# NyanCAD/CedarSim.jl

Measured on AMD Instinct MI355X. Metric: newton_iters_per_sec, higher is better.
Workload: dtype f64

## Files before the change

cedarsim.jl_amd/csrc/ch_engine.hip:

```cpp
#include <hip/hip_runtime.h>
#include <hip/hip_ext.h>

#include <algorithm>
#include <atomic>
#include <chrono>
#include <cmath>
#include <cstdio>
#include <cstring>
#include <map>
#include <memory>
#include <new>
#include <stdexcept>
#include <string>
#include <array>
#include <vector>

#include "../../include/cedarhip.h"
#include "ch_analysis.hpp"
#include "ch_bsim4.hpp"
#include "ch_device_mem.hpp"
#include "ch_env.hpp"
#include "ch_kernels.hpp"
#include "ch_persist.hpp"
#include "ch_sparse.hpp"
#include "ch_stepper_host.hpp"

using namespace chip;
using hclock = std::chrono::steady_clock;

struct ch_ctx {
  int device = 0;
  hipStream_t stream = nullptr;
  std::string err;
};

namespace {

struct Rng {
  uint64_t s;
  explicit Rng(uint64_t seed) : s(seed) {}
  uint64_t next() { uint64_t z = (s += 0x9E3779B97F4A7C15ull); z = (z ^ (z >> 30)) * 0xBF58476D1CE4E5B9ull; z = (z ^ (z >> 27)) * 0x94D049BB133111EBull; return z ^ (z >> 31); }
  double uniform() { return ((next() >> 11) + 0.5) * (1.0 / 9007199254740992.0); }
  double normal() { double u1 = uniform(), u2 = uniform(); return std::sqrt(-2.0 * std::log(u1)) * std::cos(6.283185307179586 * u2); }
};

}

struct ch_result {
  std::vector<double> times, values, final_state;
  std::vector<int32_t> pts;
  const double* dev_values = nullptr; int64_t dev_n = 0;
  ch_stats stats;
  int status = CH_OK;
  int n_obs = 0, S = 1;
};

struct PersistConsts;
struct ch_circuit;

struct Description {
  int n_nodes = 0; double temp = 27, gmin = 1e-12, scale = 1;
  std::vector<HDev> dev; std::vector<HSource> src; std::vector<std::vector<double>> model;
  std::vector<int> slot_kind, slot_a, slot_b, obs_kind, obs_index;
  std::vector<double> va_par;
  Analysis A;
};
struct Structure {
  DevBuf<int> d_comp_class, d_comp_uofs, d_comp_dofs, d_gl_ptr, d_dkind, d_dterm, d_dsrc, d_dhdev, d_obs_unk, d_unk_obs;
  DevBuf<unsigned long long> d_stamps; DevBuf<ClassMeta> d_classes; DevBuf<unsigned char> d_dmask;
  DevBuf<int> d_dvac, d_va_mod, d_va_pofs, d_va_cofs;
  int n_va_inst = 0; size_t vac_total = 0; std::vector<ClassMeta> h_cms;
  std::vector<int> obs_primary;
  std::vector<int> needed_src;
  std::vector<int> dev_src;
  int n_dev_src() const { return std::max<int>(1, (int)dev_src.size()); }
  int block_threads = 64, lu_variant = 16;
  bool wide_split = false; int wide_l = 0, wide_other = 0;
  size_t lds_doubles_fixed = 0, lds_extra_bytes = 0;
 private: friend struct ch_circuit;
  void class_blobs(const Description& D, std::vector<int>& blob) {
    h_cms.clear();
    int max_slots = 0;
    for (size_t ci = 0; ci < D.A.classes.size(); ++ci) {
      const CompClass& c = D.A.classes[ci];
      ClassMeta m; std::memset(&m, 0, sizeof(m));
      m.nc = c.nc; m.ndev = c.ndev; m.nonlinear = c.nonlinear ? 1 : 0;
      m.n_mat_src = (int)c.mat_src.size(); m.n_vec_src = (int)c.vec_src.size();
      while (blob.size() & 3) blob.push_back(0);
      m.blob_ofs = (int)blob.size();
      blob.insert(blob.end(), c.mat_ptr.begin(), c.mat_ptr.end());
      blob.insert(blob.end(), c.vec_ptr.begin(), c.vec_ptr.end());
      int rep = -1;
      for (int k = 0; k < D.A.n_comp; ++k) if (D.A.comp_class[k] == (int)ci) { rep = k; break; }
      int ns = 0;
      {
        std::vector<int> lanes;
        bool big = false;
        for (int d = 0; d < c.ndev; ++d) {
          const EDev& e = D.A.edev[D.A.comp_dofs[rep] + d];
          if (e.kind != K_VA) continue;
          if (va_gen::MODULES[D.dev[e.hdev].ipar[0]].n_params >= 64) big = true;
          bool first = true;
          for (int j = 0; j < e.nt; ++j) if (e.term[j] >= 0) { lanes.push_back((d << 4) | (first ? 8 : 0) | j); first = false; }
        }
        const bool split = big && !env_on(Env::VA_NOSPLIT);
        if (ci == 0) { wide_split = split; wide_l = (int)lanes.size(); wide_other = 0; }
        if (!split) { for (int v : lanes) { blob.push_back(v); ++ns; } }
        else {
          for (int v : lanes) { blob.push_back(v | (1 << 29)); ++ns; }
          while (ns & 63) { blob.push_back(-1); ++ns; }
          for (int v : lanes) { blob.push_back(v | (1 << 29) | (1 << 30)); ++ns; }
        }
      }
      for (int d = 0; d < c.ndev; ++d) if (D.A.edev[D.A.comp_dofs[rep] + d].kind == K_MOS) { blob.push_back(d << 4); ++ns; if (ci == 0) ++wide_other; }
      for (int d = 0; d < c.ndev; ++d) { const int kd = D.A.edev[D.A.comp_dofs[rep] + d].kind; if (kd != K_MOS && kd != K_VA) { blob.push_back(d << 4); ++ns; if (ci == 0) ++wide_other; } }
      m.nslots = ns;
      std::vector<uint16_t> h16(c.mat_src); h16.insert(h16.end(), c.vec_src.begin(), c.vec_src.end());
      if (h16.size() & 1) h16.push_back(0);
      for (size_t i = 0; i < h16.size(); i += 2) blob.push_back((int)((uint32_t)h16[i] | ((uint32_t)h16[i + 1] << 16)));
      if (((int)blob.size() - m.blob_ofs) & 1) blob.push_back(0);
      m.wl_ofs = (int)blob.size() - m.blob_ofs;
      if (c.nc <= 64 && !c.vec_ptr.empty()) {
        std::vector<std::array<int, 3>> items;
        for (int i = 0; i < c.nc; ++i) {
          const int start = c.vec_ptr[i], cnt = c.vec_ptr[i + 1] - start;
          items.push_back({cnt, m.n_mat_src + start, (int)(0x8000u | (uint32_t)i)});
        }
        for (int e = 0; e < c.nc * c.nc; ++e) {
          const int start = c.mat_ptr[e], cnt = c.mat_ptr[e + 1] - start;
          if (cnt == 0 && e / c.nc != e % c.nc) continue;
          items.push_back({cnt, start, e});
        }
        std::stable_sort(items.begin(), items.end(), [](const std::array<int, 3>& x, const std::array<int, 3>& y) { return x[0] > y[0]; });
        for (const auto& it : items) { blob.push_back(it[1]); blob.push_back((int)(((uint32_t)it[0] << 16) | (uint32_t)it[2])); ++m.n_work; }
      }
      while ((blob.size() - m.blob_ofs) & 3) blob.push_back(0);
      m.blob_ints = (int)blob.size() - m.blob_ofs;
      if (env_on(Env::DEBUG_BLOB)) std::fprintf(stderr, "[blob] class %zu: nc %d ndev %d slots %d mat_src %d vec_src %d work %d blob_ints %d\n", ci, m.nc, m.ndev, m.nslots, m.n_mat_src, m.n_vec_src, m.n_work, m.blob_ints);
      max_slots = std::max(max_slots, m.nslots);
      h_cms.push_back(m);
    }
    block_threads = std::min(256, std::max(64, ((max_slots + 63) / 64) * 64));
    lu_variant = D.A.max_nc <= 8 ? 8 : (D.A.max_nc <= 12 ? 12 : (D.A.max_nc <= 16 ? 16 : (D.A.max_nc <= 32 ? 32 : 0)));
    if (D.A.wide) lu_variant = D.A.max_nc <= 16 ? 16 : 0;
  }
  void source_lists(const Description& D, std::vector<int>& dkind, std::vector<int>& dterm, std::vector<int>& dhdev, std::vector<int>& dsrc) {
    dsrc.clear();
    dev_src.clear();
    { std::vector<int> slot_of(D.src.size(), -1);
      for (const EDev& e : D.A.edev) {
        dkind.push_back(e.kind); for (int k = 0; k < NTERM; ++k) dterm.push_back(e.term[k]); dhdev.push_back(e.hdev);
        int si = e.kind == K_VA ? D.dev[e.hdev].ipar[1] : 0;
        if (e.src >= 0) { if (slot_of[e.src] < 0) { slot_of[e.src] = (int)dev_src.size(); dev_src.push_back(e.src); } si = slot_of[e.src]; }
        dsrc.push_back(si);
      }
      std::vector<char> need(D.src.size(), 0);
      for (int si : dev_src) need[si] = 1;
      for (const KnownDef& kd : D.A.known) for (auto& tm : kd.terms) need[tm.first] = 1;
      needed_src.clear();
      for (size_t i = 0; i < D.src.size(); ++i) if (need[i]) needed_src.push_back((int)i); }
  }
  void va_offsets(const Description& D, std::vector<int>& dvac, std::vector<int>& vmod, std::vector<int>& vpofs, std::vector<int>& vcofs) {
    dvac.assign(D.A.edev.size(), 0);
    vac_total = 0;
    for (size_t i = 0; i < D.A.edev.size(); ++i) {
      const EDev& e = D.A.edev[i];
      if (e.kind != K_VA) continue;
      const int mod = D.dev[e.hdev].ipar[0];
      dvac[i] = (int)vac_total; vmod.push_back(mod); vpofs.push_back(D.dev[e.hdev].ipar[1]); vcofs.push_back((int)vac_total);
      vac_total += (size_t)va_gen::N_CACHE[mod];
    }
    n_va_inst = (int)vmod.size();
    if (vmod.empty()) { vmod.push_back(0); vpofs.push_back(0); vcofs.push_back(0); }
  }
  void masks_and_observables(const Description& D, std::vector<unsigned char>& dm, std::vector<int>& obs_unk, std::vector<int>& unk_obs) {
    dm.assign(D.A.n_unk, 0);
    for (int u = 0; u < D.A.n_unk; ++u) dm[u] = (D.A.diff_mask[u] ? 1 : 0) | (D.A.unk_mna[u] >= D.n_nodes ? 2 : 0) | (D.A.replica[u] ? 4 : 0);
    obs_unk.clear(); unk_obs.assign(D.A.n_unk, -1);
    obs_primary.clear();
    for (size_t o = 0; o < D.obs_kind.size(); ++o) {
      int u = -1;
      if (D.obs_kind[o] == 0) u = D.A.node_unknown[D.obs_index[o]];
      else { int b = D.dev[D.obs_index[o]].branch; u = b >= 0 ? D.A.branch_unknown[b] : -1; }
      obs_unk.push_back(u);
      int prim = (int)o;
      if (u >= 0) { if (unk_obs[u] < 0) unk_obs[u] = (int)o; else prim = unk_obs[u]; }
      obs_primary.push_back(prim);
    }
  }
  void size_lds(const Description& D) {
    lds_doubles_fixed = 0; lds_extra_bytes = 0;
    for (size_t ci = 0; ci < D.A.classes.size(); ++ci) {
      const CompClass& c = D.A.classes[ci];
      lds_doubles_fixed = std::max(lds_doubles_fixed, (size_t)c.ndev * D.A.stride() + (size_t)c.nc * (c.nc + 1) + (size_t)c.nc * c.nc + 12 * (size_t)c.nc);
      lds_extra_bytes = std::max(lds_extra_bytes, ((size_t)h_cms[ci].blob_ints + 64) * 4 + 16);
    }
  }
};
struct SampleTables {
  int S = 1; bool dirty = true;
  std::vector<std::vector<double>> slot_val;
  int Spar = 1, Ssrc = 1, Smos = 1, Sgmin = 1, Stemp = 1, Sva = 1;
  std::vector<double> h_src_dc, h_src_par;
  std::vector<int> mos_cls; int n_cls = 0, max_mc = 0; long vac_stride_ = 0;
  DevBuf<double> d_dpar, d_dmult, d_gmin, d_temp, d_mosp, d_vapar, d_vacache;
  DevBuf<int> d_dcls, d_moscls_inst, d_mc_ofs, d_mc_n, d_mc_list, d_dcls_local;
  DevBuf<BlockMeta> d_bmeta;
};
struct NewtonState {
  DevBuf<double> d_X, d_Q, d_rate, d_kv;
  DevBuf<unsigned char> d_perm, d_active;
  DevBuf<BlockOut> d_out; PinnedBuf<BlockOut> h_out;
  PinnedBuf<Summary> h_sum; PinnedBuf<double> h_stage;
  DevEvent ev0, ev1; bool host_reduce = true; size_t lds_bytes = 0;
  int path = 1;
  NewtonArgs base;
  mutable std::vector<double> all_src; std::vector<double> sv_buf, kv_buf;
};
struct SparsePath {
  SparsePlan plan[2];
  struct PlanDev { DevBuf<int> prow, pcol, a2lu, diag_pos, lvl_ptr, lvl_rows, ulvl_ptr, ulvl_rows, lrow_ptr, l_pos, l_k, l_upd_ptr, upd_dst, upd_src, urow_ptr, u_pos, u_col;
                   DevBuf<int> lu2a, la_pos, la_diag, lb_dst, lb_sptr, lb_l, lb_u, lb_d, fl_rows, bl_rows; DevBuf<double> LUv, Lv;
                   DevBuf<int> s3_blob, s3_ptr, s3_topa, s3_topr; DevBuf<double> s3_schur, s3_xT, s3_base, s3_sum; DevBuf<unsigned> s3_cnt; bool s3 = false; } plan_dev[2];
  DevBuf<int> dflag; DevBuf<double> part;
  DevBuf<double> hpart, hrow;
  DevBuf<int> rowptr, colidx, mat_gptr, mat_gsrc, vec_gptr, vec_gsrc, heavy_mat, heavy_vec, heavy_rows; int n_heavy_mat = 0, n_heavy_vec = 0, n_heavy_rows = 0;
  DevBuf<double> stage, Aval, Cval, F, Q, rhs, y, dx, xcur, xpred, hq, w, qn;
  std::vector<int> h_rowptr, h_colidx; PinnedBuf<double> h_red; PinnedBuf<int> h_flag;
  std::vector<double> rate_v; std::vector<int> status_v;
  DevBuf<int> act[3]; DevBuf<double> scale;
  PinnedBuf<int> h_act; PinnedBuf<double> h_scale;
};
struct DeviceStepper {
  DevBuf<int> d_pci; DevBuf<double> d_pcd, d_pbps, d_psave, d_ptimes, d_prows, d_wgrec, d_grprec; DevBuf<unsigned> d_pcnt; DevBuf<TranCtl> d_pctl; DevBuf<int> d_pwgc, d_pwgk; DevBuf<double> d_pdcent, d_ptrans;
  int n_cu = 0, mode = 0; bool aborted = false;
};
struct SmallSignal {
  DevBuf<double> d_dumpA, d_dumpF, d_dumpQ, d_dumpC, d_dumpG, d_dumpF0, d_omega, d_xac, d_psd, d_noise_pwr, d_noise_exp;
  DevBuf<int> d_noise_a, d_noise_b, d_acfail; DevBuf<BlockMeta> d_bmeta_all;
  double scale = 0.0;
};
struct TornCompanion {
  std::unique_ptr<ch_circuit> c; std::string note;
  bool is_torn = false, keep_slot0 = false;
  std::vector<int> dsrc_host;
  std::vector<double> h_dpar0, h_dmult0;
};

struct ch_circuit {
  Arena arena;
  ch_ctx* ctx = nullptr;
  Description desc; Structure stru; SampleTables tab; NewtonState nwt;
  SparsePath sp; DeviceStepper ps; SmallSignal ac; TornCompanion torn; LaunchStats stats;
  const bool host_profile = env_on(Env::HOST_PROFILE);
  const long time_every = std::max(1L, env_long(Env::TIME_EVERY, 8));

  std::string& err() { return ctx->err; }
  void set_err(const std::string& s) { ctx->err = s; }

  ~ch_circuit() {
    if (ctx && ctx->stream) (void)hipStreamSynchronize(ctx->stream);
    if (g_arena == &arena) g_arena = nullptr;
  }

  int upload_structure() {
    g_arena = &arena; hipStream_t st = ctx->stream;
    std::vector<int> blob, dkind, dterm, dhdev, dvac, vmod, vpofs, vcofs, obs_unk, unk_obs; std::vector<unsigned char> dm;
    std::vector<int>& dsrc = torn.dsrc_host;
    stru.class_blobs(desc, blob);
    stru.source_lists(desc, dkind, dterm, dhdev, dsrc);
    stru.va_offsets(desc, dvac, vmod, vpofs, vcofs);
    HIPCHK(stru.d_dvac.upload(dvac, st)); HIPCHK(stru.d_va_mod.upload(vmod, st)); HIPCHK(stru.d_va_pofs.upload(vpofs, st)); HIPCHK(stru.d_va_cofs.upload(vcofs, st));
    stru.masks_and_observables(desc, dm, obs_unk, unk_obs);
    HIPCHK(stru.d_unk_obs.upload(unk_obs, st));
    { std::vector<unsigned long long> z(8, 0ull); HIPCHK(stru.d_stamps.upload(z, st)); }
    HIPCHK(stru.d_classes.upload(stru.h_cms, st)); HIPCHK(stru.d_gl_ptr.upload(blob, st));
    HIPCHK(stru.d_comp_class.upload(desc.A.comp_class, st)); HIPCHK(stru.d_comp_uofs.upload(desc.A.comp_uofs, st)); HIPCHK(stru.d_comp_dofs.upload(desc.A.comp_dofs, st));
    HIPCHK(stru.d_dkind.upload(dkind, st)); HIPCHK(stru.d_dterm.upload(dterm, st)); HIPCHK(stru.d_dsrc.upload(dsrc, st)); HIPCHK(stru.d_dhdev.upload(dhdev, st));
    HIPCHK(stru.d_dmask.upload(dm, st)); HIPCHK(stru.d_obs_unk.upload(obs_unk, st));
    HIPCHK(nwt.h_sum.alloc(1, hipHostMallocMapped)); HIPCHK(nwt.ev0.create()); HIPCHK(nwt.ev1.create());
    stru.size_lds(desc);
    return CH_OK;
  }

  bool slot_set(int i) const { return !tab.slot_val[i].empty(); }

 private:
  int check_capacity() {
    size_t free_b = 0, total_b = 0;
    HIPCHK(hipMemGetInfo(&free_b, &total_b));
    const double need = 2.0 * NSLOT * (double)tab.S * (double)std::max(1, desc.A.n_unk) * sizeof(double) + 64.0 * (double)tab.S * (double)std::max(1, desc.A.n_comp);
    if (need > 0.9 * (double)total_b) { set_err("sample count does not fit the device: " + std::to_string(tab.S) + " samples of " + std::to_string(desc.A.n_unk) + " unknowns need " + std::to_string((long long)(need / 1048576.0)) + " MiB for the state rings"); return CH_ERR_NOMEM; }
    return CH_OK;
  }
  int sample_widths() {
    const int nslot = (int)desc.slot_kind.size();
    bool any_par = false, any_src = false, any_mos = false, any_gmin = false;
    for (int i = 0; i < nslot; ++i) if (slot_set(i)) {
      switch (desc.slot_kind[i]) {
        case CH_SLOT_DEV_PAR: if (desc.dev[desc.slot_a[i]].kind == CH_DEV_MOS) any_mos = true; else any_par = true; break;
        case CH_SLOT_DEV_MULT: any_par = true; break;
        case CH_SLOT_MODEL_PAR: case CH_SLOT_TEMP: any_mos = true; break;
        case CH_SLOT_SRC_DC: case CH_SLOT_SRC_PAR: any_src = true; break;
        case CH_SLOT_GMIN: any_gmin = true; break;
      }
    }
    tab.Spar = any_par ? tab.S : 1; tab.Ssrc = any_src ? tab.S : 1; tab.Smos = any_mos ? tab.S : 1; tab.Sgmin = any_gmin ? tab.S : 1;
    return CH_OK;
  }
  int param_tables() {
    hipStream_t st = ctx->stream; const int nslot = (int)desc.slot_kind.size();
    const int nh = (int)desc.dev.size(), nsrc = (int)desc.src.size();
    std::vector<double> hpar((size_t)nh * tab.Spar), hmult((size_t)nh * tab.Spar);
    for (int d = 0; d < nh; ++d) for (int s = 0; s < tab.Spar; ++s) { hpar[(size_t)d * tab.Spar + s] = desc.dev[d].par[0]; hmult[(size_t)d * tab.Spar + s] = desc.dev[d].mult; }
    tab.h_src_dc.assign((size_t)tab.Ssrc * nsrc, 0.0); tab.h_src_par.assign((size_t)tab.Ssrc * nsrc * CH_SRC_NPAR, 0.0);
    for (int s = 0; s < tab.Ssrc; ++s) for (int i = 0; i < nsrc; ++i) { tab.h_src_dc[(size_t)s * nsrc + i] = desc.src[i].dc; for (int k = 0; k < CH_SRC_NPAR; ++k) tab.h_src_par[((size_t)s * nsrc + i) * CH_SRC_NPAR + k] = desc.src[i].par[k]; }
    std::vector<double> hg(tab.Sgmin, desc.gmin);
    bool any_temp = false;
    for (int i = 0; i < nslot; ++i) if (slot_set(i) && desc.slot_kind[i] == CH_SLOT_TEMP) any_temp = true;
    tab.Stemp = any_temp ? tab.S : 1;
    std::vector<double> htemp(tab.Stemp, desc.temp);
    for (int i = 0; i < nslot; ++i) if (slot_set(i)) {
      const int a = desc.slot_a[i], b = desc.slot_b[i];
      for (int s = 0; s < tab.S; ++s) {
        const double v = tab.slot_val[i][s];
        switch (desc.slot_kind[i]) {
          case CH_SLOT_DEV_PAR: if (desc.dev[a].kind != CH_DEV_MOS && b == 0) hpar[(size_t)a * tab.Spar + s] = v; break;
          case CH_SLOT_DEV_MULT: hmult[(size_t)a * tab.Spar + s] = v; break;
          case CH_SLOT_SRC_DC: tab.h_src_dc[(size_t)s * nsrc + a] = v; if (desc.src[a].kind == CH_SRC_DC) tab.h_src_par[((size_t)s * nsrc + a) * CH_SRC_NPAR] = v; break;
          case CH_SLOT_SRC_PAR: tab.h_src_par[((size_t)s * nsrc + a) * CH_SRC_NPAR + b] = v; break;
          case CH_SLOT_GMIN: hg[s] = v; break;
          case CH_SLOT_TEMP: htemp[s] = v; break;
          default: break;
        }
      }
    }
    torn.h_dpar0.assign(nh, 0.0); torn.h_dmult0.assign(nh, 1.0);
    for (int i = 0; i < nh; ++i) { torn.h_dpar0[i] = hpar[(size_t)i * tab.Spar]; torn.h_dmult0[i] = hmult[(size_t)i * tab.Spar]; }
    HIPCHK(tab.d_dpar.upload(hpar, st)); HIPCHK(tab.d_dmult.upload(hmult, st)); HIPCHK(tab.d_gmin.upload(hg, st)); HIPCHK(tab.d_temp.upload(htemp, st));
    return CH_OK;
  }
  int va_setup() {
    hipStream_t st = ctx->stream; const int nslot = (int)desc.slot_kind.size();
    bool any_va = false;
    for (int i = 0; i < nslot; ++i) if (slot_set(i) && desc.slot_kind[i] == CH_SLOT_VA_PAR) any_va = true;
    tab.Sva = any_va ? tab.S : 1;
    const size_t nvp = std::max<size_t>(1, desc.va_par.size());
    std::vector<double> vp(nvp * tab.Sva, 0.0);
    for (int s = 0; s < tab.Sva; ++s) std::copy(desc.va_par.begin(), desc.va_par.end(), vp.begin() + (size_t)s * nvp);
    for (int i = 0; i < nslot; ++i) if (slot_set(i) && desc.slot_kind[i] == CH_SLOT_VA_PAR) for (int s = 0; s < tab.Sva; ++s) vp[(size_t)s * nvp + desc.slot_a[i]] = tab.slot_val[i][s];
    HIPCHK(tab.d_vapar.upload(vp, st));
    const int Svac = (tab.Sva > 1 || tab.Stemp > 1) ? tab.S : 1;
    HIPCHK(tab.d_vacache.alloc(std::max<size_t>(1, stru.vac_total * (size_t)Svac)));
    if (stru.n_va_inst > 0) {
      const long nthr = (long)stru.n_va_inst * Svac;
      hipLaunchKernelGGL(va_setup_kernel, dim3((unsigned)((nthr + 63) / 64)), dim3(64), 0, st, stru.n_va_inst, Svac, stru.d_va_mod.p, stru.d_va_pofs.p, stru.d_va_cofs.p,
                         tab.d_vapar.p, tab.Sva > 1 ? (long)nvp : 0L, tab.d_temp.p, tab.Stemp, tab.d_vacache.p, Svac > 1 ? (long)stru.vac_total : 0L);
      HIPCHK(hipGetLastError());
    }
    tab.vac_stride_ = Svac > 1 ? (long)stru.vac_total : 0L;
    return CH_OK;
  }
  int mos_classes() {
    hipStream_t st = ctx->stream; const int nslot = (int)desc.slot_kind.size();
    const int nmos = (int)desc.A.mos_hdev.size();
    tab.mos_cls.assign(nmos, 0);
    std::map<std::vector<double>, int> cls_of;
    std::vector<int> cls_rep;
    for (int m = 0; m < nmos; ++m) {
      const HDev& d = desc.dev[desc.A.mos_hdev[m]];
      std::vector<double> key;
      key.push_back(d.ipar[0]);
      for (int k = 0; k < 7; ++k) key.push_back(std::isnan(d.par[k]) ? -1e300 : d.par[k]);
      for (int i = 0; i < nslot; ++i) if (slot_set(i) && desc.slot_kind[i] == CH_SLOT_DEV_PAR && desc.slot_a[i] == desc.A.mos_hdev[m]) {
        key.push_back(1e6 + desc.slot_b[i]);
        key.insert(key.end(), tab.slot_val[i].begin(), tab.slot_val[i].end());
      }
      auto it = cls_of.find(key);
      if (it == cls_of.end()) { it = cls_of.insert({key, (int)cls_rep.size()}).first; cls_rep.push_back(m); }
      tab.mos_cls[m] = it->second;
    }
    tab.n_cls = (int)cls_rep.size();
    const long cols = (long)std::max(1, tab.n_cls) * tab.Smos;
    std::vector<double> table((size_t)B4I_COUNT * cols + 2, 0.0), col(B4I_COUNT);
    for (int c = 0; c < tab.n_cls; ++c) {
      const int hd = desc.A.mos_hdev[cls_rep[c]];
      for (int s = 0; s < tab.Smos; ++s) {
        std::vector<double> card = desc.model[desc.dev[hd].ipar[0]];
        double ip[CH_DEV_NPAR]; for (int k = 0; k < CH_DEV_NPAR; ++k) ip[k] = desc.dev[hd].par[k];
        double tc = desc.temp;
        for (int i = 0; i < nslot; ++i) if (slot_set(i)) {
          const double v = tab.slot_val[i][tab.Smos > 1 ? s : 0];
          if (desc.slot_kind[i] == CH_SLOT_MODEL_PAR && desc.slot_a[i] == desc.dev[hd].ipar[0]) card[desc.slot_b[i]] = v;
          else if (desc.slot_kind[i] == CH_SLOT_DEV_PAR && desc.slot_a[i] == hd) ip[desc.slot_b[i]] = v;
          else if (desc.slot_kind[i] == CH_SLOT_TEMP) tc = v;
        }
        ip[CH_MOS_W] *= desc.scale; ip[CH_MOS_L] *= desc.scale;
        int rc = b4_pack(card.data(), ip, tc, col.data());
        if (rc != CH_OK) { set_err(rc == CH_ERR_UNSUPPORTED ? "BSIM4 card selects a sub-model the engine does not implement (rdsmod/rgatemod/rbodymod/igcmod/igbmod/trnqsmod/geomod != 0, diomod != 1, mobmod > 2, capmod not 0/2)" : "invalid MOS geometry or model card"); return rc; }
        for (int k = 0; k < B4I_COUNT; ++k) table[((size_t)c * tab.Smos + s) * B4I_COUNT + k] = col[k];
      }
    }
    HIPCHK(tab.d_mosp.upload(table, st));
    std::vector<int> dcls;
    for (const EDev& e : desc.A.edev) dcls.push_back(e.mos >= 0 ? tab.mos_cls[e.mos] : 0);
    HIPCHK(tab.d_dcls.upload(dcls, st));
    return CH_OK;
  }
  int block_class_lists() {
    hipStream_t st = ctx->stream;
    std::vector<int> mc_ofs(desc.A.n_comp), mc_n(desc.A.n_comp), mc_list, dloc(desc.A.edev.size(), 0);
    tab.max_mc = 0;
    for (int k = 0; k < desc.A.n_comp; ++k) {
      mc_ofs[k] = (int)mc_list.size();
      std::vector<int> seen;
      for (int d = 0; d < desc.A.comp_ndev[k]; ++d) {
        const EDev& e = desc.A.edev[desc.A.comp_dofs[k] + d];
        if (e.kind == K_VA) { dloc[desc.A.comp_dofs[k] + d] = desc.dev[e.hdev].ipar[0]; continue; }
        if (e.mos < 0) continue;
        const int cl = tab.mos_cls[e.mos];
        int j = (int)(std::find(seen.begin(), seen.end(), cl) - seen.begin());
        if (j == (int)seen.size()) seen.push_back(cl);
        dloc[desc.A.comp_dofs[k] + d] = j;
      }
      mc_n[k] = (int)seen.size();
      mc_list.insert(mc_list.end(), seen.begin(), seen.end());
      tab.max_mc = std::max(tab.max_mc, mc_n[k]);
    }
    std::vector<BlockMeta> bmv(desc.A.n_comp);
    for (int k = 0; k < desc.A.n_comp; ++k) {
      BlockMeta& b = bmv[k]; std::memset(&b, 0, sizeof(b));
      b.uofs = desc.A.comp_uofs[k]; b.dofs = desc.A.comp_dofs[k]; b.mc_n = mc_n[k]; b.mc_ofs = mc_ofs[k]; b.cm = stru.h_cms[desc.A.comp_class[k]];
      for (int j = 0; j < mc_n[k] && j < 8; ++j) b.mc[j] = mc_list[mc_ofs[k] + j];
    }
    HIPCHK(tab.d_bmeta.upload(bmv, st));
    HIPCHK(tab.d_mc_ofs.upload(mc_ofs, st)); HIPCHK(tab.d_mc_n.upload(mc_n, st)); HIPCHK(tab.d_mc_list.upload(mc_list, st)); HIPCHK(tab.d_dcls_local.upload(dloc, st));
    HIPCHK(tab.d_moscls_inst.upload(tab.mos_cls, st));
    return CH_OK;
  }
  int alloc_rings() {
    hipStream_t st = ctx->stream;
    const size_t slot_elems = (size_t)tab.S * desc.A.n_unk;
    HIPCHK(nwt.d_X.alloc(slot_elems * NSLOT)); HIPCHK(nwt.d_Q.alloc(slot_elems * NSLOT));
    HIPCHK(hipMemsetAsync(nwt.d_X.p, 0, slot_elems * NSLOT * sizeof(double), st));
    HIPCHK(hipMemsetAsync(nwt.d_Q.p, 0, slot_elems * NSLOT * sizeof(double), st));
    HIPCHK(nwt.d_out.alloc((size_t)desc.A.n_comp * tab.S));
    { std::vector<double> ones((size_t)desc.A.n_comp * tab.S, 1.0); HIPCHK(nwt.d_rate.upload(ones, st)); }
    HIPCHK(nwt.d_perm.alloc((size_t)desc.A.n_comp * tab.S * 16)); HIPCHK(hipMemsetAsync(nwt.d_perm.p, 0, (size_t)desc.A.n_comp * tab.S * 16, st));
    nwt.host_reduce = (size_t)desc.A.n_comp * tab.S <= 4096 && !env_on(Env::DEVICE_REDUCE);
    if (nwt.host_reduce && nwt.h_out.n < (size_t)desc.A.n_comp * tab.S) {
      HIPCHK(nwt.h_out.alloc((size_t)desc.A.n_comp * tab.S, hipHostMallocMapped));
      std::memset(nwt.h_out, 0, (size_t)desc.A.n_comp * tab.S * sizeof(BlockOut));
    }
    HIPCHK(nwt.d_active.alloc((size_t)desc.A.n_comp * tab.S));
    const size_t need = (size_t)tab.Ssrc * (desc.A.known.size() + stru.n_dev_src());
    HIPCHK(nwt.d_kv.alloc(need));
    if (need > nwt.h_stage.n) HIPCHK(nwt.h_stage.alloc(need));
    return CH_OK;
  }
  int fill_base() {
    const long cols = (long)std::max(1, tab.n_cls) * tab.Smos; const size_t slot_elems = (size_t)tab.S * desc.A.n_unk;
    NewtonArgs& a = nwt.base;
    std::memset(&a, 0, sizeof(a));
    a.comp_class = stru.d_comp_class.p; a.comp_uofs = stru.d_comp_uofs.p; a.comp_dofs = stru.d_comp_dofs.p; a.classes = stru.d_classes.p;
    a.blob = stru.d_gl_ptr.p; a.dkind = stru.d_dkind.p; a.dterm = stru.d_dterm.p; a.dsrc = stru.d_dsrc.p; a.dcls = tab.d_dcls.p; a.dhdev = stru.d_dhdev.p;
    a.dpar = tab.d_dpar.p; a.dmult = tab.d_dmult.p; a.mosp = tab.d_mosp.p; a.mos_cols = cols; a.kv = nwt.d_kv.p; a.srcv = nwt.d_kv.p + (size_t)tab.Ssrc * desc.A.known.size(); a.dmask = stru.d_dmask.p;
    a.active = nullptr; a.gmin_s = tab.d_gmin.p; a.vapar = tab.d_vapar.p; a.va_stride = tab.Sva > 1 ? (long)std::max<size_t>(1, desc.va_par.size()) : 0; a.temp_s = tab.d_temp.p; a.Stemp = tab.Stemp;
    a.vacache = tab.d_vacache.p; a.vac_stride = tab.vac_stride_; a.dvac = stru.d_dvac.p;
    a.n_comp = desc.A.n_comp; a.S = tab.S; a.Spar = tab.Spar; a.Ssrc = tab.Ssrc; a.Smos = tab.Smos; a.Sgmin = tab.Sgmin; a.nk = (int)desc.A.known.size(); a.nsrc = stru.n_dev_src();
    a.n_unk = desc.A.n_unk; a.n_mos_cls = tab.n_cls;
    a.X = nwt.d_X.p; a.Qh = nwt.d_Q.p; a.slot_stride = (long)slot_elems; a.out = nwt.host_reduce ? nwt.h_out.p : nwt.d_out.p;
    a.unk_obs = stru.d_unk_obs.p; a.n_obs = (int)desc.obs_kind.size();
    a.bmeta = tab.d_bmeta.p; a.dcls_local = tab.d_dcls_local.p; a.comp_mc_ofs = tab.d_mc_ofs.p; a.comp_mc_n = tab.d_mc_n.p; a.mc_list = tab.d_mc_list.p; a.max_mc = tab.max_mc;
    a.summary = nwt.h_sum; a.rate = nwt.d_rate.p; a.perm = nwt.d_perm.p;
#ifdef CH_STAMPS
    a.stamps = stru.d_stamps.p;
#endif
    nwt.lds_bytes = (stru.lds_doubles_fixed + desc.A.known.size() + stru.n_dev_src() + (size_t)tab.max_mc * B4L_STRIDE) * sizeof(double) + stru.lds_extra_bytes;
    nwt.lds_bytes = std::max(nwt.lds_bytes, (size_t)9 * stru.block_threads * sizeof(double));
    nwt.path = (nwt.lds_bytes > 150 * 1024 || desc.A.max_nc > 64 || tab.max_mc > 64 || desc.A.force_sparse || env_on(Env::FORCE_SPARSE)) ? 2 : 1;
    return CH_OK;
  }
 public:
  int finalize_params() {
    if (!tab.dirty) return CH_OK;
    g_arena = &arena;
    for (int (ch_circuit::*step)() : {&ch_circuit::check_capacity, &ch_circuit::sample_widths, &ch_circuit::param_tables, &ch_circuit::va_setup,
                                      &ch_circuit::mos_classes, &ch_circuit::block_class_lists, &ch_circuit::alloc_rings, &ch_circuit::fill_base})
      { const int rc = (this->*step)(); if (rc != CH_OK) return rc; }
    if (nwt.path == 2) { const int rcs = build_sparse_structure(); if (rcs != CH_OK) return rcs; nwt.lds_bytes = 0; }
    HIPCHK(hipStreamSynchronize(ctx->stream));
    tab.dirty = false;
    return CH_OK;
  }

  void eval_sources(double t, int mode, std::vector<double>& sv, std::vector<double>& kv) const {
    const int nsrc = (int)desc.src.size(), nk = (int)desc.A.known.size(), nds = stru.n_dev_src();
    sv.assign((size_t)tab.Ssrc * nds, 0.0); kv.assign((size_t)tab.Ssrc * nk, 0.0);
    nwt.all_src.resize(std::max(1, nsrc));
    for (int s = 0; s < tab.Ssrc; ++s) {
      for (int i : stru.needed_src) nwt.all_src[i] = source_value(desc.src[i], &tab.h_src_par[((size_t)s * nsrc + i) * CH_SRC_NPAR], tab.h_src_dc[(size_t)s * nsrc + i], t, mode) + ac.scale * desc.src[i].ac;
      for (size_t j = 0; j < stru.dev_src.size(); ++j) sv[(size_t)s * nds + j] = nwt.all_src[stru.dev_src[j]];
      for (int k = 0; k < nk; ++k) { double v = 0; for (auto& tm : desc.A.known[k].terms) v += tm.second * nwt.all_src[tm.first]; kv[(size_t)s * nk + k] = v; }
    }
  }
  int set_sources(NewtonArgs& a, double t, int mode) {
    std::vector<double>& sv = nwt.sv_buf; std::vector<double>& kv = nwt.kv_buf;
    eval_sources(t, mode, sv, kv);
    if (tab.Ssrc == 1 && kv.size() + sv.size() <= (size_t)KV_INLINE) {
      a.inline_vals = 1;
      for (size_t i = 0; i < kv.size(); ++i) a.vals_inline[i] = kv[i];
      for (size_t i = 0; i < sv.size(); ++i) a.vals_inline[kv.size() + i] = sv[i];
      return CH_OK;
    }
    a.inline_vals = 0;
    std::memcpy(nwt.h_stage, kv.data(), kv.size() * sizeof(double));
    std::memcpy(nwt.h_stage + kv.size(), sv.data(), sv.size() * sizeof(double));
    HIPCHK(hipMemcpyAsync(nwt.d_kv.p, nwt.h_stage, (kv.size() + sv.size()) * sizeof(double), hipMemcpyHostToDevice, ctx->stream));
    return CH_OK;
  }

  int build_sparse_structure();
  SparseDev sparse_dev(int which, int sm = 0);
  int sparse_plan_from_current(int which, int sm = 0);
  void launch_lu_solve(int which, const int* wl, size_t n_work);
  int stage_list(int slot, const std::vector<int>& list);
  int run_sparse(NewtonArgs a, const unsigned char* host_active, Summary& out);
  int ac_ncomp() const { return nwt.path == 2 ? 1 : desc.A.n_comp; }
  int ac_ds() const { return nwt.path == 2 ? desc.A.n_unk : desc.A.max_nc; }
  int ac_comp_of(int u) const { return nwt.path == 2 ? 0 : (int)(std::upper_bound(desc.A.comp_uofs.begin(), desc.A.comp_uofs.end(), u) - desc.A.comp_uofs.begin()) - 1; }
  int ac_uofs(int comp) const { return nwt.path == 2 ? 0 : desc.A.comp_uofs[comp]; }
  int ac_nc(int comp) const { return nwt.path == 2 ? desc.A.n_unk : desc.A.comp_nc[comp]; }
  int ac_dofs(int comp) const { return nwt.path == 2 ? 0 : desc.A.comp_dofs[comp]; }
  int ac_ndev(int comp) const { return nwt.path == 2 ? (int)desc.A.edev.size() : desc.A.comp_ndev[comp]; }
  const BlockMeta* ac_bmeta();

  int poll_stream(const char* what) {
    hipError_t q = hipErrorNotReady;
    for (int spin = 0; spin < 200000 && q == hipErrorNotReady; ++spin) q = hipStreamQuery(ctx->stream);
    if (q == hipErrorNotReady) q = hipStreamSynchronize(ctx->stream);
    if (q != hipSuccess) { set_err(std::string(what) + hipGetErrorString(q)); return CH_ERR_DEVICE; }
    return CH_OK;
  }
  int run_newton(const NewtonArgs& a, const unsigned char* host_active, Summary& out) {
    if (nwt.path == 2) return run_sparse(a, host_active, out);
    hipStream_t st = ctx->stream;
    const int nblk = desc.A.n_comp * tab.S;
    const bool timed = time_every <= 1 || ((uint64_t)(stats.n_launch + 1) * 0x9E3779B97F4A7C15ull >> 33) % (uint64_t)time_every == 0;
    const auto tp0 = host_profile ? hclock::now() : hclock::time_point();
    hipEvent_t e0 = timed ? nwt.ev0.e : nullptr, e1 = timed ? nwt.ev1.e : nullptr;
    const dim3 g(nblk), b(stru.block_threads);
    static void (*const kernels[])(const NewtonArgs) = {newton_block_kernel<16, true>, newton_block_kernel<0, true>, newton_block_kernel<8>, newton_block_kernel<12>,
                                                        newton_block_kernel<16>, newton_block_kernel<32>, newton_block_kernel<0>};
    const int lu = stru.lu_variant, ki = desc.A.wide ? (lu == 16 ? 0 : 1) : lu == 8 ? 2 : lu == 12 ? 3 : lu == 16 ? 4 : lu == 32 ? 5 : 6;
    hipExtLaunchKernelGGL(kernels[ki], g, b, (uint32_t)nwt.lds_bytes, st, e0, e1, 0, a);
    if (!nwt.host_reduce) hipLaunchKernelGGL(reduce_blocks_kernel, dim3(1), dim3(256), 9 * 256 * sizeof(double), st, a);
    const auto tp1 = host_profile ? hclock::now() : hclock::time_point();
    { const int prc = poll_stream("newton kernel: "); if (prc != CH_OK) return prc; }
    HIPCHK(hipGetLastError());
    const auto tp2 = host_profile ? hclock::now() : hclock::time_point();
    if (timed) { float ms = 0; HIPCHK(hipEventElapsedTime(&ms, nwt.ev0, nwt.ev1)); stats.device_ms += ms; stats.n_timed += 1; }
    stats.n_launch += 1;
    if (!nwt.host_reduce) out = *nwt.h_sum;
    else {
      Summary r; std::memset(&r, 0, sizeof(r));
      for (int s = 0; s < tab.S; ++s) {
        double e2[3] = {0, 0, 0}; long nd = 0; int smx = 0;
        for (int k = 0; k < desc.A.n_comp; ++k) {
          const size_t b = (size_t)k * tab.S + s;
          if (host_active && !host_active[b]) continue;
          const BlockOut& o = nwt.h_out[b];
          e2[0] += o.e2k; e2[1] += o.e2km1; e2[2] += o.e2kp1; nd += o.ndiff;
          if (o.status != 0) ++r.n_fail;
          if (o.status == 2) ++r.n_singular;
          smx = std::max(smx, o.iters); r.sum_block_iters += o.iters; r.fnorm = std::max(r.fnorm, o.fnorm);
        }
        r.sum_iters += smx; r.max_iters = std::max(r.max_iters, smx);
        if (nd > 0) { r.errk = std::max(r.errk, a.ck * std::sqrt(e2[0] / nd)); r.errkm1 = std::max(r.errkm1, a.ckm1 * std::sqrt(e2[1] / nd)); r.errkp1 = std::max(r.errkp1, a.ckp1 * std::sqrt(e2[2] / nd)); }
      }
      out = r;
    }
    if (host_profile) {
      const auto tp3 = hclock::now();
      stats.prof_launch += std::chrono::duration<double>(tp1 - tp0).count(); stats.prof_wait += std::chrono::duration<double>(tp2 - tp1).count();
      stats.prof_reduce += std::chrono::duration<double>(tp3 - tp2).count();
    }
    return CH_OK;
  }

  int download_mna(int slot, double t, int mode, double* x_out) {
    std::vector<double> xs((size_t)tab.S * desc.A.n_unk);
    HIPCHK(hipMemcpy(xs.data(), nwt.d_X.p + (size_t)slot * tab.S * desc.A.n_unk, xs.size() * sizeof(double), hipMemcpyDeviceToHost));
    std::vector<double> sv, kv; eval_sources(t, mode, sv, kv);
    const int nk = (int)desc.A.known.size();
    for (int s = 0; s < tab.S; ++s) {
      double* xo = x_out + (size_t)s * desc.A.n_mna;
      for (int n = 1; n <= desc.n_nodes; ++n) xo[n - 1] = desc.A.node_unknown[n] >= 0 ? xs[(size_t)s * desc.A.n_unk + desc.A.node_unknown[n]] : kv[(size_t)(tab.Ssrc > 1 ? s : 0) * nk + desc.A.node_known[n]];
      for (int b = 0; b < desc.A.n_branch; ++b) xo[desc.n_nodes + b] = desc.A.branch_unknown[b] >= 0 ? xs[(size_t)s * desc.A.n_unk + desc.A.branch_unknown[b]] : CH_NAN;
    }
    return CH_OK;
  }
  int upload_from_mna(int slot, const double* x_mna) {
    std::vector<double> xs((size_t)tab.S * desc.A.n_unk);
    for (int s = 0; s < tab.S; ++s) for (int u = 0; u < desc.A.n_unk; ++u) xs[(size_t)s * desc.A.n_unk + u] = x_mna[(size_t)s * desc.A.n_mna + desc.A.unk_mna[u]];
    HIPCHK(hipMemcpy(nwt.d_X.p + (size_t)slot * tab.S * desc.A.n_unk, xs.data(), xs.size() * sizeof(double), hipMemcpyHostToDevice));
    return CH_OK;
  }

  int dc_solve(const ch_dc_opts& o, int slot, std::vector<int>* status_out, ch_stats* stt) {
    const int mode = o.tran_mode ? 2 : 0;
    const int nblk = desc.A.n_comp * tab.S;
    int rc = CH_OK;
    std::vector<unsigned char> active(nblk, 1);
    std::vector<double> xs((size_t)tab.S * desc.A.n_unk), xm(desc.A.n_mna);
    std::vector<BlockOut> bo(nblk);
    NewtonArgs a = nwt.base;
    a.mode = MODE_DC; a.maxit = std::max(1, o.maxiters); a.dc_abstol = o.abstol; a.dv_max = o.dv_max; a.gshunt = 0.0;
    a.abstol = 1e-6; a.reltol = 1e-3; a.newton_tol = 0.1;
    a.hist_slot[0] = slot; a.cand_slot = slot; a.active = nwt.d_active.p;
    rc = set_sources(a, 0.0, mode);
    if (rc != CH_OK) return rc;
    std::vector<Rng> rngs; for (int s = 0; s < tab.S; ++s) rngs.emplace_back(o.seed + (uint64_t)s);
    auto block_of_unknown = [&](int u) { int c = (int)(std::upper_bound(desc.A.comp_uofs.begin(), desc.A.comp_uofs.end(), u) - desc.A.comp_uofs.begin()) - 1; return c; };
    int n_active = nblk;
    std::vector<unsigned char> donor_ok(nblk, 0);
    const int nrest = std::max(1, o.n_restarts);
    for (int r = 0; r < nrest + 1 && n_active > 0; ++r) {
      const bool homotopy = (r == nrest);
      HIPCHK(hipMemcpy(xs.data(), nwt.d_X.p + (size_t)slot * tab.S * desc.A.n_unk, xs.size() * sizeof(double), hipMemcpyDeviceToHost));
      for (int s = 0; s < tab.S; ++s) {
        bool any = false;
        for (int c = 0; c < desc.A.n_comp; ++c) if (active[(size_t)c * tab.S + s]) any = true;
        if (!any) continue;
        if (!homotopy) {
          if (r == 0 && o.x0) for (int i = 0; i < desc.A.n_mna; ++i) xm[i] = o.x0[(size_t)s * desc.A.n_mna + i];
          else for (int i = 0; i < desc.A.n_mna; ++i) xm[i] = 1e-7 * rngs[s].normal();
        } else std::fill(xm.begin(), xm.end(), 0.0);
        for (int u = 0; u < desc.A.n_unk; ++u) if (active[(size_t)block_of_unknown(u) * tab.S + s]) xs[(size_t)s * desc.A.n_unk + u] = xm[desc.A.unk_mna[u]];
      }
      if (r == 1 && tab.S > 1) {
        for (int c = 0; c < desc.A.n_comp; ++c) {
          int donor = -1;
          for (int s = 0; s < tab.S && donor < 0; ++s) if (!active[(size_t)c * tab.S + s] && donor_ok[(size_t)c * tab.S + s]) donor = s;
          if (donor < 0) continue;
          for (int s = 0; s < tab.S; ++s) if (active[(size_t)c * tab.S + s])
            for (int u = desc.A.comp_uofs[c]; u < desc.A.comp_uofs[c] + desc.A.comp_nc[c]; ++u) xs[(size_t)s * desc.A.n_unk + u] = xs[(size_t)donor * desc.A.n_unk + u];
        }
      }
      HIPCHK(hipMemcpy(nwt.d_X.p + (size_t)slot * tab.S * desc.A.n_unk, xs.data(), xs.size() * sizeof(double), hipMemcpyHostToDevice));
      HIPCHK(hipMemcpy(nwt.d_active.p, active.data(), nblk, hipMemcpyHostToDevice));
      Summary sm;
      if (!homotopy) {
        rc = run_newton(a, active.data(), sm);
        if (rc != CH_OK) return rc;
      } else {
        for (double g = 1e-2; g >= 1e-13 * 0.99; g *= 0.1) { a.gshunt = g; rc = run_newton(a, active.data(), sm); if (rc != CH_OK) return rc; }
        a.gshunt = 0.0;
        rc = run_newton(a, active.data(), sm);
        if (rc != CH_OK) return rc;
      }
      if (stt) { stt->n_block_iters += sm.sum_block_iters; stt->nnonliniter += sm.sum_iters; stt->nf += sm.sum_iters; stt->njacs += sm.sum_iters; stt->nfactors += sm.sum_iters; stt->nsolve += sm.sum_iters; }
      if (nwt.path == 2) { for (int b = 0; b < nblk; ++b) bo[b].status = sp.status_v[b % tab.S]; }
      else if (nwt.host_reduce) std::memcpy(bo.data(), nwt.h_out, nblk * sizeof(BlockOut)); else HIPCHK(hipMemcpy(bo.data(), nwt.d_out.p, nblk * sizeof(BlockOut), hipMemcpyDeviceToHost));
      n_active = 0;
      for (int b = 0; b < nblk; ++b) if (active[b]) { if (bo[b].status == 0) { active[b] = 0; donor_ok[b] = 1; } else ++n_active; }
      if (n_active > 0 && stt) { stt->nrestarts++; stt->nnonlinconvfail++; }
    }
    if (status_out) { status_out->assign(tab.S, CH_OK); for (int b = 0; b < nblk; ++b) if (active[b]) (*status_out)[b % tab.S] = bo[b].status == 2 ? CH_ERR_SINGULAR : CH_ERR_MAXITERS; }
    if (n_active > 0) { set_err("DC operating point analysis failed for " + std::to_string(n_active) + " block(s)"); return CH_ERR_MAXITERS; }
    return CH_OK;
  }

  bool persist_eligible(std::string& why, bool own_steps);
  int persist_bpw(long nblk) const;
  bool persist_own_steps(const ch_tran_opts& o) const;
  size_t persist_wave_doubles(bool wg_consts) const;
  bool persist_blob(const std::vector<int>& kn, const std::vector<int>& ds, std::vector<int>& bi, std::vector<double>& bd, std::vector<int>& need) const;
  size_t persist_va_arena(int bpw, size_t& lds) const;
  int persist_collect(ch_result& R, const TranCtl& cs, bool own_steps, bool single_batch, const std::vector<double>& htimes, const std::vector<double>& hpts,
                      const std::vector<double>& hrows, int status, hclock::time_point tstart);
  bool persist_consts(bool wg_consts, int n_wg, int bpw, double t0, double t1, PersistConsts& pc);
  int tran_persistent(double t0, double t1, const ch_tran_opts& o, ch_result& R, const std::vector<double>& bps, int kmax, double dtmin, double dtmax,
                      int max_steps, int nmaxit, hclock::time_point tstart, bool& used, const ch_dc_opts* dcm = nullptr, long long* dc_iters = nullptr,
                      const std::vector<double>* bpc = nullptr);
  int dc_border(const ch_dc_opts& o, long long* iters);
  int tran_torn(double t0, double t1, const ch_tran_opts& o, ch_result& R, bool& used);


  int check_tran_opts(double t0, double t1, const ch_tran_opts& o) {
    if (!std::isfinite(t0) || !std::isfinite(t1) || !(t1 > t0)) { set_err("tspan must be finite and increasing"); return CH_ERR_INVALID; }
    if (!(o.abstol >= 0) || !(o.reltol >= 0) || !std::isfinite(o.abstol) || !std::isfinite(o.reltol) || o.abstol + o.reltol == 0) { set_err("abstol and reltol must be finite, non-negative and not both zero"); return CH_ERR_INVALID; }
    if (!(o.dtmin >= 0) || !(o.dtmax >= 0) || !(o.dt0 >= 0) || !std::isfinite(o.dtmin) || !std::isfinite(o.dtmax) || !std::isfinite(o.dt0)) { set_err("dtmin, dtmax and dt0 must be finite and non-negative (0 = automatic)"); return CH_ERR_INVALID; }
    if (o.n_saveat < 0 || (o.n_saveat > 0 && !o.saveat)) { set_err("saveat: n_saveat points announced, none given"); return CH_ERR_INVALID; }
    for (int i = 0; i < o.n_saveat; ++i)
      if (!std::isfinite(o.saveat[i]) || (i > 0 && o.saveat[i] < o.saveat[i - 1])) { set_err("saveat must be finite and non-decreasing"); return CH_ERR_INVALID; }
    if (o.stepper < CH_STEPPER_AUTO || o.stepper > CH_STEPPER_DEVICE) { set_err("stepper must be CH_STEPPER_AUTO, _HOST or _DEVICE"); return CH_ERR_INVALID; }
    if (o.step_control != CH_STEPS_AUTO && o.step_control != CH_STEPS_SHARED) { set_err("step_control must be CH_STEPS_AUTO or CH_STEPS_SHARED"); return CH_ERR_INVALID; }
    return CH_OK;
  }
  int try_device_stepper(double t0, double t1, const ch_tran_opts& o, ch_result& R, const std::vector<double>& bps, const std::vector<double>& bpc, int kmax,
                         double dtmin, double dtmax, int max_steps, int nmaxit, hclock::time_point tstart, bool& done) {
    done = true;
    const int want = resolve_stepper(o.stepper, env_get(Env::STEPPER));
    if (want != CH_STEPPER_HOST) {
      std::string why;
      if (persist_eligible(why, persist_own_steps(o))) {
        bool used = false;
        ps.aborted = false;
        const int rc = tran_persistent(t0, t1, o, R, bps, kmax, dtmin, dtmax, max_steps, nmaxit, tstart, used, nullptr, nullptr, &bpc);
        if (used && ps.aborted && want != CH_STEPPER_DEVICE) {
          const std::string msg = err();
          ctx->err.clear();
          if (torn.is_torn) { set_err(msg); return CH_ERR_UNSUPPORTED; }
          ch_tran_opts o3 = o; o3.stepper = CH_STEPPER_HOST;
          return tran_solve(t0, t1, o3, R);
        }
        if (used) return rc;
        why = err();
      }
      if (want == CH_STEPPER_DEVICE || torn.is_torn) { set_err("device-resident stepper not available for this circuit: " + why); return CH_ERR_UNSUPPORTED; }
      if (env_on(Env::DEBUG_STEPPER)) std::fprintf(stderr, "[stepper] host stepper because: %s\n", why.c_str());
    }
    if (torn.is_torn) { set_err("the torn form of a circuit runs on the device-resident stepper only"); return CH_ERR_UNSUPPORTED; }
    done = false;
    return CH_OK;
  }

  struct RowStore {
    static constexpr int CH = 512;
    std::vector<double*> chunks; size_t row_doubles = 1;
    ~RowStore() { for (double* p : chunks) (void)hipFree(p); }
    hipError_t row_ptr(long row, double** out) {
      while ((size_t)(row / CH) >= chunks.size()) { double* p = nullptr; const hipError_t e = hipMalloc((void**)&p, std::max<size_t>(1, (size_t)CH * row_doubles) * sizeof(double)); if (e != hipSuccess) return e; chunks.push_back(p); }
      *out = chunks[row / CH] + (size_t)(row % CH) * row_doubles;
      return hipSuccess;
    }
  };
  int save_row(ch_result& R, RowStore& rows, double ts, const int* slots, const double* w, int nw) {
    double* dst = nullptr;
    HIPCHK(rows.row_ptr((long)R.times.size(), &dst));
    const int n_obs = R.n_obs;
    if (n_obs > 0) {
      ObsArgs oa; oa.X = nwt.d_X.p; oa.slot_stride = (long)tab.S * desc.A.n_unk; oa.nw = nw; oa.n_unk = desc.A.n_unk; oa.S = tab.S; oa.n_obs = n_obs; oa.obs_unk = stru.d_obs_unk.p;
      for (int j = 0; j < nw; ++j) { oa.slots[j] = slots[j]; oa.w[j] = w[j]; }
      oa.dst = dst;
      const int n = n_obs * tab.S;
      hipLaunchKernelGGL(save_obs_kernel, dim3((n + 255) / 256), dim3(256), 0, ctx->stream, oa);
    }
    R.times.push_back(ts); R.pts.push_back(0);
    return CH_OK;
  }

  int tran_solve(double t0, double t1, const ch_tran_opts& o, ch_result& R) {
    { const int vrc = check_tran_opts(t0, t1, o); if (vrc != CH_OK) return vrc; }
    if (torn.c && !torn.is_torn && tab.S == 1 && !env_on(Env::NO_TEAR) && resolve_stepper(o.stepper, env_get(Env::STEPPER), false) != CH_STEPPER_HOST) {
      bool used = false;
      const int rc = tran_torn(t0, t1, o, R, used);
      if (used || rc != CH_OK) return rc;
    }
    auto tstart = hclock::now();
    R.times.clear(); R.pts.clear(); R.values.clear(); R.final_state.clear();
    std::memset(&R.stats, 0, sizeof(R.stats));
    R.S = tab.S; R.n_obs = (int)desc.obs_kind.size();
    stats.reset();
    int rc = finalize_params();
    if (rc != CH_OK) return rc;
    hipStream_t st = ctx->stream;
    const int kmax = std::min(5, std::max(1, o.max_order));
    const double span = t1 - t0;
    const double dtmax = o.dtmax > 0 ? o.dtmax : span / 10.0, dtmin = o.dtmin > 0 ? o.dtmin : 1e-15 * span;
    const int max_steps = o.max_steps > 0 ? o.max_steps : 100000 , nmaxit = o.newton_maxiters > 0 ? o.newton_maxiters : 10;
    const int n_obs = R.n_obs;

    if (o.skip_dc) {
      if (o.dc.x0) { rc = upload_from_mna(0, o.dc.x0); if (rc != CH_OK) return rc; }
      else if (!torn.keep_slot0) HIPCHK(hipMemsetAsync(nwt.d_X.p, 0, (size_t)tab.S * desc.A.n_unk * sizeof(double), st));
    } else {
      rc = dc_solve(o.dc, 0, nullptr, &R.stats);
      if (rc != CH_OK) return rc;
    }
    R.stats.dc_seconds = std::chrono::duration<double>(hclock::now() - tstart).count();
    {
      NewtonArgs a = nwt.base; a.mode = MODE_EVAL; a.maxit = 1; a.hist_slot[0] = 0; a.cand_slot = 0; a.abstol = o.abstol; a.reltol = o.reltol;
      rc = set_sources(a, t0, 1); if (rc != CH_OK) return rc;
      Summary sm; rc = run_newton(a, nullptr, sm); if (rc != CH_OK) return rc;
      R.stats.nf += tab.S;
    }
    stats.end_of_dc(R.stats.n_block_iters);

    std::vector<double> bps, bpc;
    {
      const int nsrc = (int)desc.src.size();
      std::vector<std::pair<double, double>> pts;
      for (int s = 0; s < tab.Ssrc; ++s) for (int i = 0; i < nsrc; ++i) source_breakpoint_codes(desc.src[i], &tab.h_src_par[((size_t)s * nsrc + i) * CH_SRC_NPAR], t0, t1, pts);
      merge_breakpoints(pts, t1, bps, bpc);
    }
    if (nwt.d_perm.p) HIPCHK(hipMemsetAsync(nwt.d_perm.p, 0, (size_t)desc.A.n_comp * tab.S * 16, ctx->stream));

    { bool done = false;
      rc = try_device_stepper(t0, t1, o, R, bps, bpc, kmax, dtmin, dtmax, max_steps, nmaxit, tstart, done);
      if (done) return rc; }

    StepControl sc(t0, t1, o.dt0, dtmin, dtmax, kmax, bps, bpc);
    RowStore rows; rows.row_doubles = (size_t)n_obs * tab.S;
    int isave = 0;
    { const double one = 1.0; const int s0 = sc.order[0];
      if (o.n_saveat == 0) { rc = save_row(R, rows, t0, &s0, &one, 1); if (rc) return rc; }
      else while (isave < o.n_saveat && o.saveat[isave] <= t0) { rc = save_row(R, rows, o.saveat[isave], &s0, &one, 1); if (rc) return rc; ++isave; } }

    int status = CH_OK;
    NewtonArgs a = nwt.base;
    a.mode = MODE_TRAN; a.maxit = nmaxit; a.abstol = o.abstol; a.reltol = o.reltol; a.newton_tol = 0.1;
    for (int step = 0; step < max_steps && sc.t < t1;) {
      status = sc.plan();
      if (status != CH_OK) break;
      const StepCoeffs& c = sc.c;
      a.k = c.k; a.npred = c.npred; a.nkm1 = c.nkm1; a.nkp1 = c.nkp1; a.ck = c.ck; a.ckm1 = c.ckm1; a.ckp1 = c.ckp1; a.cand_slot = c.cand_slot;
      std::memcpy(a.alpha, c.alpha, sizeof(a.alpha)); std::memcpy(a.wpred, c.wpred, sizeof(a.wpred)); std::memcpy(a.wkm1, c.wkm1, sizeof(a.wkm1)); std::memcpy(a.wkp1, c.wkp1, sizeof(a.wkp1));
      std::memcpy(a.hist_slot, c.hist_slot, sizeof(a.hist_slot));
      rc = set_sources(a, sc.source_time(), 1); if (rc != CH_OK) { status = rc; break; }
      a.reset_rate = sc.reset_rate ? 1 : 0;
      a.obs_row = nullptr;
      if (o.n_saveat == 0 && n_obs > 0 && rows.row_ptr((long)R.times.size(), &a.obs_row) != hipSuccess) { set_err("host stepper: out of device memory for the saved rows"); status = CH_ERR_DEVICE; break; }
      Summary sm;
      rc = run_newton(a, nullptr, sm); if (rc != CH_OK) { status = rc; break; }
      R.stats.n_step_attempts++;
      R.stats.n_block_iters += sm.sum_block_iters; R.stats.nnonliniter += sm.sum_iters; R.stats.nf += sm.sum_iters; R.stats.njacs += sm.sum_iters; R.stats.nfactors += sm.sum_iters; R.stats.nsolve += sm.sum_iters;
      if (sm.n_fail > 0) { R.stats.nnonlinconvfail++; sc.on_convergence_failure(); continue; }
      const double errk = sc.lte ? sm.errk : 0.0;
      if (errk > 1.0) { R.stats.nreject++; sc.on_error_test_failure(errk); continue; }
      R.stats.naccept++; ++step;
      sc.on_accept();
      if (o.n_saveat > 0) {
        while (isave < o.n_saveat && o.saveat[isave] <= sc.tn * (1 + 1e-15)) {
          double ww[9]; const int m = sc.dense_weights(o.saveat[isave], ww);
          rc = save_row(R, rows, o.saveat[isave], sc.order, ww + 1, m); if (rc) break;
          ++isave;
        }
      } else if (n_obs > 0) { R.times.push_back(sc.tn); R.pts.push_back(sc.dense_points()); }
      else { const double one = 1.0; rc = save_row(R, rows, sc.tn, sc.order, &one, 1); if (rc == CH_OK) R.pts.back() = sc.dense_points(); }
      if (rc != CH_OK) { status = rc; break; }
      sc.select_next(errk, sm.errkm1, sm.errkp1);
    }
    if (status == CH_OK && sc.t < t1) status = CH_ERR_MAXSTEPS;
    (void)hipStreamSynchronize(st);
    const size_t nt = R.times.size();
    R.values.assign((size_t)n_obs * nt * tab.S, 0.0);
    std::vector<double> buf((size_t)RowStore::CH * n_obs * tab.S);
    for (size_t cidx = 0; cidx < rows.chunks.size(); ++cidx) {
      const size_t nr = std::min<size_t>(RowStore::CH, nt - cidx * RowStore::CH);
      if (n_obs == 0 || nr == 0) continue;
      (void)hipMemcpy(buf.data(), rows.chunks[cidx], nr * n_obs * tab.S * sizeof(double), hipMemcpyDeviceToHost);
      rows_to_obs_major(buf.data(), nr, cidx * RowStore::CH, nt, n_obs, tab.S, R.values.data());
    }
    return finish_tran(R, sc.order[0], sc.t, status, tstart);
  }

  int finish_tran(ch_result& R, int newest_slot, double t, int status, hclock::time_point tstart) {
    const int n_obs = R.n_obs;
    const size_t nt = R.times.size();
    {
      for (int ob = 0; ob < n_obs; ++ob) if (stru.obs_primary[ob] != ob)
        std::memcpy(&R.values[(size_t)ob * nt * tab.S], &R.values[(size_t)stru.obs_primary[ob] * nt * tab.S], nt * tab.S * sizeof(double));
      const int nk = (int)desc.A.known.size();
      std::vector<double> sv, kv;
      for (int ob = 0; ob < n_obs; ++ob) {
        if (desc.obs_kind[ob] == 0 && desc.A.node_unknown[desc.obs_index[ob]] < 0) {
          const int kn = desc.A.node_known[desc.obs_index[ob]];
          for (size_t it = 0; it < nt; ++it) { eval_sources(R.times[it], 1, sv, kv); for (int s = 0; s < tab.S; ++s) R.values[((size_t)ob * nt + it) * tab.S + s] = kv[(size_t)(tab.Ssrc > 1 ? s : 0) * nk + kn]; }
        } else if (desc.obs_kind[ob] == 1) {
          const int b = desc.dev[desc.obs_index[ob]].branch;
          if (b < 0 || desc.A.branch_unknown[b] < 0) for (size_t it = 0; it < nt; ++it) for (int s = 0; s < tab.S; ++s) R.values[((size_t)ob * nt + it) * tab.S + s] = CH_NAN;
        }
      }
    }
    R.final_state.assign((size_t)tab.S * desc.A.n_mna, 0.0);
    download_mna(newest_slot, t, 1, R.final_state.data());
#ifdef CH_STAMPS
    { unsigned long long hs[8]; (void)hipMemcpy(hs, stru.d_stamps.p, sizeof(hs), hipMemcpyDeviceToHost);
      std::fprintf(stderr, "[stamps] cycles summed over blocks: prologue %llu eval %llu gather %llu solve %llu epilogue %llu arrival %llu pre-LU %llu LU %llu ; launches %ld blocks %d\n", hs[0], hs[1], hs[2], hs[3], hs[4], hs[5], hs[6], hs[7], stats.n_launch, desc.A.n_comp * tab.S); }
#endif
    R.status = status;
    R.stats.wall_seconds = std::chrono::duration<double>(hclock::now() - tstart).count();
    if (host_profile) { std::fprintf(stderr, "[host profile] wall %.3f ms; in run_newton: launch %.3f ms, wait %.3f ms, events+reduce %.3f ms; launches %ld\n", 1e3 * R.stats.wall_seconds, 1e3 * stats.prof_launch, 1e3 * stats.prof_wait, 1e3 * stats.prof_reduce, stats.n_launch); stats.prof_launch = stats.prof_wait = stats.prof_reduce = 0; }
    stats.fill(R.stats);
    R.stats.n_kernel_launches = stats.n_launch + stats.persist_launches;
    R.stats.n_step_attempts += stats.persist_attempts; R.stats.barrier_seconds = stats.persist_barrier_s;
    R.stats.stepper = stats.persist_launches > 0 ? CH_STEPPER_DEVICE : CH_STEPPER_HOST;
    R.stats.stepper_mode = stats.persist_launches > 0 ? ps.mode : 0;
    R.stats.step_block_iters = R.stats.n_block_iters - stats.dc_block_iters;
    if (status != CH_OK && err().empty()) set_err(status == CH_ERR_DTMIN ? "step size underflow (DtLessThanMin)" : "transient did not reach t1");
    return status;
  }
};
struct CallScope { ArenaScope arena; explicit CallScope(ch_circuit* c) : arena(&c->arena) { c->ctx->err.clear(); (void)hipSetDevice(c->ctx->device); } };

#include "ch_engine_sparse.hpp"
#include "ch_engine_persist.hpp"


static void set_err_nothrow(ch_ctx* ctx, const char* what, const char* detail) noexcept {
  if (!ctx) return;
  try { ctx->err = what; if (detail && *detail) { ctx->err += ": "; ctx->err += detail; } }
  catch (...) { ctx->err.clear(); }
}
template <class F>
static int guard_rc(ch_ctx* ctx, F&& body) noexcept {
  try { return body(); }
  catch (const std::bad_alloc&) { set_err_nothrow(ctx, "out of host memory inside the engine call", ""); return CH_ERR_NOMEM; }
  catch (const std::length_error& e) { set_err_nothrow(ctx, "a host container would exceed its maximum size (sample count x circuit size too large)", e.what()); return CH_ERR_NOMEM; }
  catch (const std::exception& e) { set_err_nothrow(ctx, "internal error (C++ exception caught at the C-ABI)", e.what()); return CH_ERR_INTERNAL; }
  catch (...) { set_err_nothrow(ctx, "internal error (unknown C++ exception caught at the C-ABI)", ""); return CH_ERR_INTERNAL; }
}

extern "C" {

void ch_dc_opts_default(ch_dc_opts* o) { std::memset(o, 0, sizeof(*o)); o->abstol = 1e-10; o->maxiters = 200; o->n_restarts = 10; o->seed = 10; o->tran_mode = 0; o->dv_max = 2.0; o->x0 = nullptr; }
void ch_tran_opts_default(ch_tran_opts* o) { std::memset(o, 0, sizeof(*o)); o->abstol = 1e-6; o->reltol = 1e-3; o->max_order = 5; o->newton_maxiters = 10; ch_dc_opts_default(&o->dc); }

static hipError_t raise_lds_ceilings() {
  const int lds_cu = 160 * 1024;
  const void* fns[] = {(const void*)newton_block_kernel<8>, (const void*)newton_block_kernel<12>, (const void*)newton_block_kernel<16>,
                       (const void*)newton_block_kernel<32>, (const void*)newton_block_kernel<0>, (const void*)newton_block_kernel<16, true>,
                       (const void*)newton_block_kernel<0, true>, (const void*)ac_block_kernel<64>};
  for (const void* f : fns) {
    hipFuncAttributes fa;
    hipError_t e = hipFuncGetAttributes(&fa, f);
    if (e != hipSuccess) return e;
    const int cap = (lds_cu - (int)fa.sharedSizeBytes) & ~255;
    e = hipFuncSetAttribute(f, hipFuncAttributeMaxDynamicSharedMemorySize, cap);
    if (e != hipSuccess) return e;
  }
  return hipSuccess;
}

static ch_ctx* ch_create_impl(int device_id, char* err, size_t errlen) {
  auto fail = [&](const std::string& m) -> ch_ctx* { if (err && errlen) { std::snprintf(err, errlen, "%s", m.c_str()); } return nullptr; };
  int n = 0;
  hipError_t e = hipGetDeviceCount(&n);
  if (e != hipSuccess || n == 0) return fail(std::string("cedarhip needs a HIP device (gfx950); none available: ") + (e != hipSuccess ? hipGetErrorString(e) : "device count 0"));
  if (device_id < 0 || device_id >= n) return fail("invalid device id");
  if ((e = hipSetDevice(device_id)) != hipSuccess) return fail(hipGetErrorString(e));
  if ((e = raise_lds_ceilings()) != hipSuccess) return fail(std::string("hipFuncSetAttribute(MaxDynamicSharedMemorySize): ") + hipGetErrorString(e));
  ch_ctx* c = new ch_ctx();
  c->device = device_id;
  if ((e = hipStreamCreateWithFlags(&c->stream, hipStreamNonBlocking)) != hipSuccess) { delete c; return fail(hipGetErrorString(e)); }
  return c;
}
void ch_destroy(ch_ctx* c) { if (!c) return; if (c->stream) (void)hipStreamDestroy(c->stream); delete c; }
const char* ch_last_error(ch_ctx* c) { return c ? c->err.c_str() : "null context"; }

static ch_circuit* ch_circuit_build_impl(ch_ctx* ctx, const ch_desc* d, bool tear = false) {
  if (!ctx || !d) return nullptr;
  ctx->err.clear();
  (void)hipSetDevice(ctx->device);
  std::unique_ptr<ch_circuit> owner(new ch_circuit());
  ch_circuit* c = owner.get();
  c->ctx = ctx;
  ArenaScope arena_scope(&c->arena);
  c->desc.n_nodes = d->n_nodes; c->desc.temp = d->temp; c->desc.gmin = d->gmin; c->desc.scale = d->scale;
  for (int i = 0; i < d->n_src; ++i) {
    HSource s; s.kind = d->src_kind[i]; s.dc = d->src_dc[i];
    for (int k = 0; k < CH_SRC_NPAR; ++k) s.par[k] = d->src_par[i * CH_SRC_NPAR + k];
    if (d->src_pwl_ofs) for (int k = d->src_pwl_ofs[i]; k < d->src_pwl_ofs[i + 1]; ++k) { s.ts.push_back(d->pwl_t[k]); s.ys.push_back(d->pwl_y[k]); }
    s.ac = d->src_ac ? std::fabs(d->src_ac[i]) : 0.0;
    c->desc.src.push_back(s);
  }
  for (int i = 0; i < d->n_model; ++i) c->desc.model.emplace_back(d->model_par + (size_t)i * CH_B4_NPAR, d->model_par + (size_t)(i + 1) * CH_B4_NPAR);
  auto bad = [&](const char* m) -> ch_circuit* { ctx->err = m; return nullptr; };
  for (int i = 0; i < d->n_dev; ++i) {
    HDev v; v.kind = d->dev_kind[i]; v.branch = -1; v.eliminated = false;
    for (int k = 0; k < CH_DEV_NNODE; ++k) { v.node[k] = d->dev_node[i * CH_DEV_NNODE + k]; if (v.node[k] < 0 || v.node[k] > d->n_nodes) return bad("device node id out of range"); }
    for (int k = 0; k < CH_DEV_NIPAR; ++k) v.ipar[k] = d->dev_ipar[i * CH_DEV_NIPAR + k];
    for (int k = 0; k < CH_DEV_NPAR; ++k) v.par[k] = d->dev_par[i * CH_DEV_NPAR + k];
    v.mult = d->dev_mult[i];
    if (v.mult < 0) return bad("Cannot construct a ParallelInstances with non-positive multiplier");
    if ((v.kind == CH_DEV_V || v.kind == CH_DEV_I) && (v.ipar[0] < 0 || v.ipar[0] >= d->n_src)) return bad("source index out of range");
    if (v.kind == CH_DEV_MOS && (v.ipar[0] < 0 || v.ipar[0] >= d->n_model)) return bad("model index out of range");
    if (v.kind < CH_DEV_R || v.kind > CH_DEV_VA) return bad("unknown device kind");
    if (v.kind == CH_DEV_VA) {
      if (v.ipar[0] < 0 || v.ipar[0] >= va_gen::N_MODULES) return bad("Verilog-A module id out of range (is the module compiled into this library?)");
      const va_gen::ModuleInfo& mi = va_gen::MODULES[v.ipar[0]];
      if (v.ipar[1] < 0 || (int64_t)v.ipar[1] + 2 * mi.n_params > d->n_va_par || !d->va_par) return bad("Verilog-A parameter block out of range");
      v.va_nt = mi.n_nodes; v.va_qmask = mi.q_mask;
    }
    c->desc.dev.push_back(v);
  }
  if (d->va_par && d->n_va_par > 0) c->desc.va_par.assign(d->va_par, d->va_par + d->n_va_par);
  for (int i = 0; i < d->n_slot; ++i) { c->desc.slot_kind.push_back(d->slot_kind[i]); c->desc.slot_a.push_back(d->slot_a[i]); c->desc.slot_b.push_back(d->slot_b[i]); }
  for (int i = 0; i < d->n_obs; ++i) { c->desc.obs_kind.push_back(d->obs_kind[i]); c->desc.obs_index.push_back(d->obs_index[i]); }
  c->tab.slot_val.assign(c->desc.slot_kind.size(), {});
  std::vector<char> protect(c->desc.dev.size(), 0), swept(c->desc.src.size(), 0);
  for (size_t o = 0; o < c->desc.obs_kind.size(); ++o) if (c->desc.obs_kind[o] == 1) { if (c->desc.obs_index[o] < 0 || c->desc.obs_index[o] >= (int)c->desc.dev.size()) return bad("observable device index out of range"); protect[c->desc.obs_index[o]] = 1; }
  for (size_t i = 0; i < c->desc.slot_kind.size(); ++i) {
    const int k = c->desc.slot_kind[i], sa = c->desc.slot_a[i], sb = c->desc.slot_b[i];
    bool ok = true;
    switch (k) {
      case CH_SLOT_DEV_PAR: ok = sa >= 0 && sa < (int)c->desc.dev.size() && sb >= 0 && sb < CH_DEV_NPAR; break;
      case CH_SLOT_DEV_MULT: ok = sa >= 0 && sa < (int)c->desc.dev.size(); break;
      case CH_SLOT_MODEL_PAR: ok = sa >= 0 && sa < (int)c->desc.model.size() && sb >= 0 && sb < CH_B4_NPAR; break;
      case CH_SLOT_SRC_DC: ok = sa >= 0 && sa < (int)c->desc.src.size(); break;
      case CH_SLOT_SRC_PAR: ok = sa >= 0 && sa < (int)c->desc.src.size() && sb >= 0 && sb < CH_SRC_NPAR; break;
      case CH_SLOT_TEMP: case CH_SLOT_GMIN: break;
      case CH_SLOT_VA_PAR: ok = sa >= 0 && (size_t)sa < c->desc.va_par.size(); break;
      default: ok = false;
    }
    if (!ok) return bad("parameter slot refers to a device, model, source or field that does not exist");
    if (k == CH_SLOT_SRC_DC || k == CH_SLOT_SRC_PAR) swept[sa] = 1;
  }
  for (size_t i = 0; i < c->desc.dev.size(); ++i) if (c->desc.dev[i].kind == CH_DEV_V && c->desc.src[c->desc.dev[i].ipar[0]].ac != 0.0) { protect[i] = 1; swept[c->desc.dev[i].ipar[0]] = 1; }
  int rc = analyse(c->desc.n_nodes, c->desc.dev, c->desc.src, protect, swept, c->desc.A, tear);
  if (rc != CH_OK) { ctx->err = c->desc.A.err; return nullptr; }
  c->torn.is_torn = tear;
  rc = c->upload_structure();
  if (rc != CH_OK) return nullptr;
  if (!tear && c->desc.A.max_nc > 64 && !env_on(Env::NO_TEAR)) {
    c->torn.c.reset(ch_circuit_build_impl(ctx, d, true));
    c->torn.note = c->torn.c ? "torn companion built" : ctx->err;
    ctx->err.clear();
  }
  return owner.release();
}
void ch_circuit_free(ch_circuit* c) { delete c; }

int ch_circuit_info(ch_circuit* c, ch_info* o) {
  if (!c || !o) return CH_ERR_INVALID;
  std::memset(o, 0, sizeof(*o));
  const Analysis& A = c->desc.A;
  o->n_nodes = c->desc.n_nodes; o->n_branches = A.n_branch; o->n_mna = A.n_mna; o->n_unknowns = A.n_unk; o->n_known = (int)A.known.size() - 1;
  o->n_alias = A.n_alias; o->n_components = A.n_comp; o->max_component = A.max_nc; o->n_classes = (int)A.classes.size();
  o->n_mos = (int)A.mos_hdev.size(); o->n_mos_classes = c->tab.n_cls; o->path = c->nwt.path; o->n_samples = c->tab.S;
  o->nnz_jac = (int64_t)c->sp.h_colidx.size(); o->nnz_lu = c->sp.plan[1].valid ? c->sp.plan[1].nnz_lu : (c->sp.plan[0].valid ? c->sp.plan[0].nnz_lu : 0);
  return CH_OK;
}
int ch_circuit_maps(ch_circuit* c, int32_t* node_unknown, int32_t* node_known, int32_t* branch_unknown) {
  if (!c) return CH_ERR_INVALID;
  for (int n = 0; n <= c->desc.n_nodes; ++n) { if (node_unknown) node_unknown[n] = c->desc.A.node_unknown[n]; if (node_known) node_known[n] = c->desc.A.node_known[n]; }
  for (int b = 0; b < c->desc.A.n_branch; ++b) if (branch_unknown) branch_unknown[b] = c->desc.A.branch_unknown[b];
  return CH_OK;
}

static int ch_set_samples_impl(ch_circuit* c, int32_t n) {
  if (!c) return CH_ERR_INVALID;
  if (n < 1) { c->set_err("ch_set_samples: at least one sample"); return CH_ERR_INVALID; }
  c->tab.S = n;
  for (auto& v : c->tab.slot_val) v.clear();
  c->tab.dirty = true;
  if (c->torn.c) return ch_set_samples_impl(c->torn.c.get(), n);
  return CH_OK;
}
static int ch_set_params_impl(ch_circuit* c, int32_t lo, int32_t hi, int32_t n_slots, const int32_t* ids, const double* values) {
  if (!c) return CH_ERR_INVALID;
  if (lo < 0 || hi > c->tab.S || lo >= hi || n_slots < 0 || (n_slots > 0 && (!ids || !values))) { c->set_err("ch_set_params: sample range outside [0, n_samples) or missing arrays"); return CH_ERR_INVALID; }
  for (int i = 0; i < n_slots; ++i) {
    const int id = ids[i];
    if (id < 0 || id >= (int)c->desc.slot_kind.size()) { c->set_err("slot id out of range"); return CH_ERR_INVALID; }
    auto& v = c->tab.slot_val[id];
    if (v.empty()) {
      double base = 0; const int a = c->desc.slot_a[id], b = c->desc.slot_b[id];
      switch (c->desc.slot_kind[id]) {
        case CH_SLOT_DEV_PAR: base = c->desc.dev[a].par[b]; break;
        case CH_SLOT_DEV_MULT: base = c->desc.dev[a].mult; break;
        case CH_SLOT_MODEL_PAR: base = c->desc.model[a][b]; break;
        case CH_SLOT_SRC_DC: base = c->desc.src[a].dc; break;
        case CH_SLOT_SRC_PAR: base = c->desc.src[a].par[b]; break;
        case CH_SLOT_TEMP: base = c->desc.temp; break;
        case CH_SLOT_GMIN: base = c->desc.gmin; break;
        case CH_SLOT_VA_PAR: base = c->desc.va_par[a]; break;
      }
      v.assign(c->tab.S, base);
    }
    for (int s = lo; s < hi; ++s) v[s] = values[(size_t)i * (hi - lo) + (s - lo)];
  }
  c->tab.dirty = true;
  if (c->torn.c) return ch_set_params_impl(c->torn.c.get(), lo, hi, n_slots, ids, values);
  return CH_OK;
}

static int ch_dc_impl(ch_circuit* c, const ch_dc_opts* o, double* x_out, int32_t* status_out, ch_stats* stats) {
  if (!c || !o) return CH_ERR_INVALID;
  CallScope call(c);
  auto t0 = hclock::now();
  ch_stats st; std::memset(&st, 0, sizeof(st));
  c->stats.reset();
  int rc = c->finalize_params();
  if (rc != CH_OK) return rc;
  std::vector<int> status;
  rc = c->dc_solve(*o, 0, &status, &st);
  if (x_out) { int r2 = c->download_mna(0, 0.0, o->tran_mode ? 2 : 0, x_out); if (r2 != CH_OK) return r2; }
  if (status_out) for (int s = 0; s < c->tab.S; ++s) status_out[s] = status.empty() ? rc : status[s];
  st.wall_seconds = st.dc_seconds = std::chrono::duration<double>(hclock::now() - t0).count();
  c->stats.end_of_dc(st.n_block_iters); c->stats.fill(st); st.n_kernel_launches = c->stats.n_launch;
  if (stats) *stats = st;
  return rc;
}

static int ch_tran_impl(ch_circuit* c, double t0, double t1, const ch_tran_opts* o, ch_result** out) {
  if (!c || !o || !out) return CH_ERR_INVALID;
  CallScope call(c);
  std::unique_ptr<ch_result> R(new ch_result());
  int rc = c->tran_solve(t0, t1, *o, *R);
  R->status = rc;
  *out = R.release();
  return rc;
}
int64_t ch_result_n_times(const ch_result* r) { return r ? (int64_t)r->times.size() : 0; }
const double* ch_result_times(const ch_result* r) { return r ? r->times.data() : nullptr; }
const int32_t* ch_result_dense_points(const ch_result* r) { return (r && r->pts.size() == r->times.size()) ? r->pts.data() : nullptr; }
int ch_result_device_values(const ch_result* r, const double** ptr, int64_t* n_doubles) {
  if (!r || !ptr || !n_doubles) return CH_ERR_INVALID;
  *ptr = r->dev_values; *n_doubles = r->dev_n;
  return r->dev_values ? CH_OK : CH_ERR_UNSUPPORTED;
}
const double* ch_result_values(const ch_result* r) { return r ? r->values.data() : nullptr; }
const double* ch_result_final_state(const ch_result* r) { return r ? r->final_state.data() : nullptr; }
int ch_result_stats(const ch_result* r, ch_stats* s) { if (!r || !s) return CH_ERR_INVALID; *s = r->stats; return CH_OK; }
int ch_result_status(const ch_result* r) { return r ? r->status : CH_ERR_INVALID; }
void ch_result_free(ch_result* r) { delete r; }

static int ch_eval_impl(ch_circuit* c, int32_t sample, const double* x_mna, double t, double alpha0, int32_t mode, double* F_out, double* Q_out, double* J_out) {
  if (!c || !x_mna || sample < 0 || sample >= c->tab.S) return CH_ERR_INVALID;
  CallScope call(c);
  int rc = c->finalize_params();
  if (rc != CH_OK) return rc;
  const Analysis& A = c->desc.A;
  const int S = c->tab.S, nblk = A.n_comp * S, ds = A.max_nc;
  std::vector<double> xs((size_t)S * A.n_unk, 0.0);
  for (int u = 0; u < A.n_unk; ++u) xs[(size_t)sample * A.n_unk + u] = x_mna[A.unk_mna[u]];
  if (hipMemcpy(c->nwt.d_X.p, xs.data(), xs.size() * sizeof(double), hipMemcpyHostToDevice) != hipSuccess) return CH_ERR_DEVICE;
  std::vector<unsigned char> act(nblk, 0);
  for (int k = 0; k < A.n_comp; ++k) act[(size_t)k * S + sample] = 1;
  if (hipMemcpy(c->nwt.d_active.p, act.data(), nblk, hipMemcpyHostToDevice) != hipSuccess) return CH_ERR_DEVICE;
  if (c->ac.d_dumpA.alloc((size_t)nblk * ds * ds) != hipSuccess || c->ac.d_dumpF.alloc((size_t)nblk * ds) != hipSuccess || c->ac.d_dumpQ.alloc((size_t)nblk * ds) != hipSuccess) return CH_ERR_DEVICE;
  NewtonArgs a = c->nwt.base;
  rc = c->set_sources(a, t, mode == 0 ? 0 : 1);
  if (rc != CH_OK) return rc;
  a.mode = MODE_EVAL; a.maxit = 1; a.alpha[0] = alpha0; a.hist_slot[0] = 0; a.cand_slot = 1; a.active = c->nwt.d_active.p; a.abstol = 1e-6; a.reltol = 1e-3;
  a.dumpA = c->ac.d_dumpA.p; a.dumpF = c->ac.d_dumpF.p; a.dumpQ = c->ac.d_dumpQ.p; a.dumpC = nullptr; a.dump_stride = ds;
  Summary sm;
  rc = c->run_newton(a, act.data(), sm);
  if (rc != CH_OK) return rc;
  const int n = A.n_mna;
  std::vector<char> has(n, 0);
  if (J_out) std::fill(J_out, J_out + (size_t)n * n, 0.0);
  if (F_out) std::fill(F_out, F_out + n, 0.0);
  if (Q_out) std::fill(Q_out, Q_out + n, 0.0);
  if (c->nwt.path == 2) {
    const size_t nnz = c->sp.h_colidx.size();
    std::vector<double> av(nnz), fv(A.n_unk), qv(A.n_unk);
    (void)hipMemcpy(av.data(), c->sp.Aval.p + (size_t)sample * nnz, nnz * sizeof(double), hipMemcpyDeviceToHost);
    (void)hipMemcpy(fv.data(), c->sp.F.p + (size_t)sample * A.n_unk, fv.size() * sizeof(double), hipMemcpyDeviceToHost);
    (void)hipMemcpy(qv.data(), c->sp.Q.p + (size_t)sample * A.n_unk, qv.size() * sizeof(double), hipMemcpyDeviceToHost);
    for (int u = 0; u < A.n_unk; ++u) {
      const int ri = A.unk_mna[u]; has[ri] = 1;
      if (F_out) F_out[ri] = fv[u];
      if (Q_out) Q_out[ri] = qv[u];
      if (J_out) for (int p = c->sp.h_rowptr[u]; p < c->sp.h_rowptr[u + 1]; ++p) J_out[(size_t)ri * n + A.unk_mna[c->sp.h_colidx[p]]] = av[p];
    }
  } else {
  std::vector<double> hA((size_t)nblk * ds * ds), hF((size_t)nblk * ds), hQ((size_t)nblk * ds);
  (void)hipMemcpy(hA.data(), c->ac.d_dumpA.p, hA.size() * sizeof(double), hipMemcpyDeviceToHost);
  (void)hipMemcpy(hF.data(), c->ac.d_dumpF.p, hF.size() * sizeof(double), hipMemcpyDeviceToHost);
  (void)hipMemcpy(hQ.data(), c->ac.d_dumpQ.p, hQ.size() * sizeof(double), hipMemcpyDeviceToHost);
  for (int k = 0; k < A.n_comp; ++k) {
    const int blk = k * S + sample, nc = A.comp_nc[k], uo = A.comp_uofs[k];
    for (int i = 0; i < nc; ++i) {
      const int ri = A.unk_mna[uo + i];
      has[ri] = 1;
      if (F_out) F_out[ri] = hF[(size_t)blk * ds + i];
      if (Q_out) Q_out[ri] = hQ[(size_t)blk * ds + i];
      if (J_out) for (int j = 0; j < nc; ++j) J_out[(size_t)ri * n + A.unk_mna[uo + j]] = hA[(size_t)blk * ds * ds + (size_t)i * nc + j];
    }
  }
  }
  if (J_out) for (int i = 0; i < n; ++i) if (!has[i]) J_out[(size_t)i * n + i] = 1.0;
  return CH_OK;
}

#include "ch_engine_ac.hpp"


static int mos_eval_impl(ch_circuit* c, int32_t sample, const double* v, double* out, bool quad) {
  if (!c || !v || !out || sample < 0 || sample >= c->tab.S) return CH_ERR_INVALID;
  CallScope call(c);
  int rc = c->finalize_params();
  if (rc != CH_OK) return rc;
  const int nm = (int)c->desc.A.mos_hdev.size();
  if (nm == 0) return CH_OK;
  double *dv = nullptr, *dout = nullptr;
  if (hipMalloc((void**)&dv, (size_t)nm * 4 * sizeof(double)) != hipSuccess || hipMalloc((void**)&dout, (size_t)nm * 40 * sizeof(double)) != hipSuccess) return CH_ERR_DEVICE;
  (void)hipMemcpy(dv, v, (size_t)nm * 4 * sizeof(double), hipMemcpyHostToDevice);
  std::vector<double> hg(c->tab.Sgmin);
  (void)hipMemcpy(hg.data(), c->tab.d_gmin.p, hg.size() * sizeof(double), hipMemcpyDeviceToHost);
  const double gm = hg[c->tab.Sgmin > 1 ? sample : 0];
  hipLaunchKernelGGL(quad ? mos_eval_quad_kernel : mos_eval_kernel, dim3(((quad ? 4 : 1) * nm + 63) / 64), dim3(64), 0, c->ctx->stream, (const double*)c->tab.d_mosp.p, c->nwt.base.mos_cols, (const int*)c->tab.d_moscls_inst.p, c->tab.Smos, (int)sample, nm, (const double*)dv, gm, dout);
  hipError_t e = hipStreamSynchronize(c->ctx->stream);
  if (e == hipSuccess) e = hipMemcpy(out, dout, (size_t)nm * 40 * sizeof(double), hipMemcpyDeviceToHost);
  (void)hipFree(dv); (void)hipFree(dout);
  if (e != hipSuccess) { c->set_err(hipGetErrorString(e)); return CH_ERR_DEVICE; }
  return CH_OK;
}
int ch_mos_eval(ch_circuit* c, int32_t sample, const double* v, double* out) { return guard_rc(c ? c->ctx : nullptr, [&] { return mos_eval_impl(c, sample, v, out, false); }); }
int ch_mos_eval_quad(ch_circuit* c, int32_t sample, const double* v, double* out) { return guard_rc(c ? c->ctx : nullptr, [&] { return mos_eval_impl(c, sample, v, out, true); }); }

static const char* const k_b4_names[] = {
#define P(n, d) #n,
#define B(n, d) #n, "l" #n, "w" #n, "p" #n,
#define I(n)
#include "../../include/cedarhip_bsim4_params.def"
};
static const char* const k_b4_ignored[] = {
#define P(n, d)
#define B(n, d)
#define I(n) #n,
#include "../../include/cedarhip_bsim4_params.def"
    nullptr};
int32_t ch_bsim4_npar(void) { return CH_B4_NPAR; }
const char* ch_bsim4_param_name(int32_t i) { return (i >= 0 && i < CH_B4_NPAR) ? k_b4_names[i] : nullptr; }
int32_t ch_bsim4_param_ignored(const char* name) {
  if (!name) return 0;
  for (int i = 0; k_b4_ignored[i]; ++i) if (std::strcmp(k_b4_ignored[i], name) == 0) return 1;
  return 0;
}
#include "ch_engine_diag.hpp"
int32_t ch_va_n_modules(void) { return va_gen::N_MODULES; }
int32_t ch_va_find(const char* name) {
  if (!name) return -1;
  for (int i = 0; i < va_gen::N_MODULES; ++i) if (std::strcmp(va_gen::MODULES[i].name, name) == 0) return i;
  return -1;
}
const char* ch_va_module_name(int32_t id) { return (id >= 0 && id < va_gen::N_MODULES) ? va_gen::MODULES[id].name : nullptr; }
int32_t ch_va_module_info(int32_t id, int32_t* n_ports, int32_t* n_nodes, int32_t* n_params) {
  if (id < 0 || id >= va_gen::N_MODULES) return CH_ERR_INVALID;
  const va_gen::ModuleInfo& mi = va_gen::MODULES[id];
  if (n_ports) *n_ports = mi.n_ports; if (n_nodes) *n_nodes = mi.n_nodes; if (n_params) *n_params = mi.n_params;
  return CH_OK;
}
const char* ch_va_node_name(int32_t id, int32_t k) { return (id >= 0 && id < va_gen::N_MODULES && k >= 0 && k < va_gen::MODULES[id].n_nodes) ? va_gen::MODULES[id].node_names[k] : nullptr; }
const char* ch_va_param_name(int32_t id, int32_t k) { return (id >= 0 && id < va_gen::N_MODULES && k >= 0 && k < va_gen::MODULES[id].n_params) ? va_gen::MODULES[id].param_names[k] : nullptr; }
int32_t ch_va_n_opvars(int32_t id) { return (id >= 0 && id < va_gen::N_MODULES) ? va_gen::N_OPVARS[id] : 0; }
const char* ch_va_opvar_name(int32_t id, int32_t k) { return (id >= 0 && id < va_gen::N_MODULES && k >= 0 && k < va_gen::N_OPVARS[id]) ? va_gen::OPNAMES[id][k] : nullptr; }
ch_ctx* ch_create(int device_id, char* err, size_t errlen) {
  try { return ch_create_impl(device_id, err, errlen); }
  catch (const std::exception& e) { if (err && errlen) std::snprintf(err, errlen, "ch_create: %s", e.what()); }
  catch (...) { if (err && errlen) std::snprintf(err, errlen, "ch_create: unknown C++ exception"); }
  return nullptr;
}
ch_circuit* ch_circuit_build(ch_ctx* ctx, const ch_desc* d) {
  ch_circuit* c = nullptr;
  const int rc = guard_rc(ctx, [&] { c = ch_circuit_build_impl(ctx, d); return c ? CH_OK : CH_ERR_INVALID; });
  return rc == CH_OK ? c : nullptr;
}
int ch_set_samples(ch_circuit* c, int32_t n) { return guard_rc(c ? c->ctx : nullptr, [&] { return ch_set_samples_impl(c, n); }); }
int ch_set_params(ch_circuit* c, int32_t lo, int32_t hi, int32_t n_slots, const int32_t* ids, const double* values) {
  return guard_rc(c ? c->ctx : nullptr, [&] { return ch_set_params_impl(c, lo, hi, n_slots, ids, values); });
}
int ch_dc(ch_circuit* c, const ch_dc_opts* o, double* x_out, int32_t* status_out, ch_stats* stats) {
  return guard_rc(c ? c->ctx : nullptr, [&] { return ch_dc_impl(c, o, x_out, status_out, stats); });
}
int ch_tran(ch_circuit* c, double t0, double t1, const ch_tran_opts* o, ch_result** out) {
  if (out) *out = nullptr;
  return guard_rc(c ? c->ctx : nullptr, [&] { return ch_tran_impl(c, t0, t1, o, out); });
}
int ch_eval(ch_circuit* c, int32_t sample, const double* x_mna, double t, double alpha0, int32_t mode, double* F_out, double* Q_out, double* J_out) {
  return guard_rc(c ? c->ctx : nullptr, [&] { return ch_eval_impl(c, sample, x_mna, t, alpha0, mode, F_out, Q_out, J_out); });
}
int ch_ac(ch_circuit* c, const ch_dc_opts* o, int32_t n_freq, const double* freqs_hz, double* x_ac_out, ch_stats* stats) {
  return guard_rc(c ? c->ctx : nullptr, [&] { return ch_ac_impl(c, o, n_freq, freqs_hz, x_ac_out, stats); });
}
int ch_noise(ch_circuit* c, const ch_dc_opts* o, int32_t out_kind, int32_t out_index, int32_t n_freq, const double* freqs_hz, double* psd_out, ch_stats* stats) {
  return guard_rc(c ? c->ctx : nullptr, [&] { return ch_noise_impl(c, o, out_kind, out_index, n_freq, freqs_hz, psd_out, stats); });
}
int ch_bench_triad(ch_ctx* ctx, int64_t n, int32_t iters, double* gbps_out) { return guard_rc(ctx, [&] { return ch_bench_triad_impl(ctx, n, iters, gbps_out); }); }
int ch_bench_fp64(ch_ctx* ctx, int32_t iters, double* tflops_out) { return guard_rc(ctx, [&] { return ch_bench_fp64_impl(ctx, iters, tflops_out); }); }
int ch_debug_poison_lds(ch_ctx* ctx) { return guard_rc(ctx, [&] { return ch_debug_poison_lds_impl(ctx); }); }
int ch_debug_math(ch_ctx* ctx, int32_t which, int32_t n, const double* x, double* y) { return guard_rc(ctx, [&] { return ch_debug_math_impl(ctx, which, n, x, y); }); }
int ch_va_eval(ch_ctx* ctx, int32_t id, const double* par, const double* v, double temperature_k, double gmin, double* st_out) {
  return guard_rc(ctx, [&] { return ch_va_eval_impl(ctx, id, par, v, temperature_k, gmin, st_out); });
}
int ch_va_opvars(ch_ctx* ctx, int32_t id, const double* par, const double* v, double temperature_k, double gmin, double* op_out) {
  return guard_rc(ctx, [&] { return ch_va_opvars_impl(ctx, id, par, v, temperature_k, gmin, op_out); });
}
const char* ch_version(void) { return "cedarhip 0.3 (gfx950; fused block Newton, device-resident step controller)"; }

}
```

cedarsim.jl_amd/csrc/ch_engine_persist.hpp:

```cpp
#pragma once

constexpr size_t P_MAX_ENTRIES = 64, P_MAX_PWL = 2048;
inline bool ch_circuit::persist_eligible(std::string& why, bool own_steps) {
  auto no = [&](const char* m) { why = m; return false; };
  if (nwt.path != 1) return no("the circuit takes the sparse path");
  if (desc.A.n_comp < 1) return no("the circuit has no unknowns");
  if (!(stru.lu_variant == 8 || stru.lu_variant == 12 || stru.lu_variant == 16)) return no("a Jacobian block has more than 16 unknowns");
  if (desc.A.wide) {
    if (desc.A.classes.size() != 1) return no("compiled Verilog-A devices in blocks of several classes");
    if (desc.A.nb > 0) return no("compiled Verilog-A devices in a bordered form");
    if (stru.wide_split ? (stru.wide_l + stru.wide_other > 32) : (stru.h_cms[0].nslots > 64)) return no("a block's compiled devices need more evaluation lanes than a wave pair offers");
    if (own_steps && tab.S == 1 && desc.A.n_comp > 1) return no("per-block steps of one circuit with compiled Verilog-A devices");
  } else if (stru.block_threads != 64) return no("a block needs more than one wavefront of device slots");
  if (tab.max_mc > 8) return no("more than 8 MOSFET classes in a block");
  if (tab.Ssrc != 1) return no("per-sample source parameters");
  const bool wg_consts = own_steps && tab.S == 1 && desc.A.n_comp > 1;
  if (!wg_consts && (stru.needed_src.size() > (size_t)P_MAXSRC || desc.A.known.size() + (size_t)stru.n_dev_src() > P_MAX_ENTRIES)) return no("more than 64 sources / known-node and source values per attempt");
  if (!(tab.S == 1 || desc.A.n_comp == 1)) return no("several blocks per sample in a multi-sample batch");
  if (desc.A.nb > 0 && (tab.S != 1 || desc.A.border_dev.size() > 8)) return no("bordered form: one sample and at most 8 devices on the border alone");
  for (const ClassMeta& m : stru.h_cms) if ((!desc.A.wide && m.nslots > 64) || m.nc > stru.lu_variant || m.n_work <= 0) return no("a block class does not fit the one-wave register path");
  if (ps.n_cu == 0) { hipDeviceProp_t prop; if (hipGetDeviceProperties(&prop, ctx->device) != hipSuccess) return no("hipGetDeviceProperties failed"); ps.n_cu = prop.multiProcessorCount; }
  const long nblk = (long)desc.A.n_comp * tab.S;
  const int bpw = persist_bpw(nblk);
  if (nblk > (long)bpw * ps.n_cu && !own_steps) return no("more blocks than resident wavefronts (4 per CU)");
  if (!own_steps && (nblk + bpw - 1) / bpw > 256) return no("more than 256 workgroups in a grid-wide reduction");
  size_t npwl = 0; for (int i : stru.needed_src) npwl += desc.src[i].ts.size();
  if (!wg_consts && npwl > P_MAX_PWL) return no("piecewise-linear tables above 2048 points");
  return true;
}
inline int ch_circuit::persist_bpw(long nblk) const {
  if (ps.n_cu > 0 && desc.A.wide && stru.wide_split && nblk <= 2L * ps.n_cu) return 2;
  return PW;
}
inline bool ch_circuit::persist_own_steps(const ch_tran_opts& o) const {
  return ((desc.A.n_comp == 1 && tab.S > 1) || (tab.S == 1 && desc.A.n_comp > 1 && desc.A.nb == 0 && !desc.A.wide)) && o.n_saveat > 0 && o.step_control != CH_STEPS_SHARED && !env_on(Env::LOCKSTEP);
}
inline size_t ch_circuit::persist_wave_doubles(bool wg_consts) const {
  const size_t n_ent = wg_consts ? (size_t)P_MAXSRC : desc.A.known.size() + stru.n_dev_src();
  return stru.lds_doubles_fixed + 16 * (size_t)desc.A.max_nc + 10 + 48 + P_MAXSRC + n_ent + (size_t)tab.max_mc * B4L_STRIDE + (stru.lds_extra_bytes + 7) / 8 + 2;
}
inline bool ch_circuit::persist_blob(const std::vector<int>& kn, const std::vector<int>& ds, std::vector<int>& bi, std::vector<double>& bd, std::vector<int>& need) const {
  const int nsrc = (int)desc.src.size();
  std::vector<char> nd(std::max(1, nsrc), 0);
  for (int k : kn) for (auto& tm : desc.A.known[k].terms) nd[tm.first] = 1;
  for (int j : ds) if (j < (int)stru.dev_src.size()) nd[stru.dev_src[j]] = 1;
  need.clear();
  for (int i = 0; i < nsrc; ++i) if (nd[i]) need.push_back(i);
  std::vector<int> pos(std::max(1, nsrc), -1);
  for (size_t i = 0; i < need.size(); ++i) pos[need[i]] = (int)i;
  std::vector<double> pt, py;
  bi = {(int)need.size(), (int)(kn.size() + ds.size()), 0, (int)kn.size()};
  for (int i : need) { bi.push_back(desc.src[i].kind); bi.push_back((int)pt.size()); bi.push_back((int)desc.src[i].ts.size()); pt.insert(pt.end(), desc.src[i].ts.begin(), desc.src[i].ts.end()); py.insert(py.end(), desc.src[i].ys.begin(), desc.src[i].ys.end()); }
  bi[2] = (int)pt.size();
  std::vector<int> eptr(1, 0), eidx; std::vector<double> ecoef;
  for (int k : kn) { for (auto& tm : desc.A.known[k].terms) { eidx.push_back(pos[tm.first]); ecoef.push_back(tm.second); } eptr.push_back((int)eidx.size()); }
  for (int j : ds) { if (j < (int)stru.dev_src.size()) { eidx.push_back(pos[stru.dev_src[j]]); ecoef.push_back(1.0); } eptr.push_back((int)eidx.size()); }
  bi.insert(bi.end(), eptr.begin(), eptr.end()); bi.insert(bi.end(), eidx.begin(), eidx.end());
  bd.clear();
  for (int i : need) for (int k = 0; k < CH_SRC_NPAR; ++k) bd.push_back(tab.h_src_par[(size_t)i * CH_SRC_NPAR + k]);
  bd.insert(bd.end(), ecoef.begin(), ecoef.end()); bd.insert(bd.end(), pt.begin(), pt.end()); bd.insert(bd.end(), py.begin(), py.end());
  for (size_t q = 4; q < bi.size(); ++q) if (bi[q] < 0) return false;
  return need.size() <= (size_t)P_MAXSRC && kn.size() + ds.size() <= P_MAX_ENTRIES && pt.size() <= P_MAX_PWL;
}

inline const void* persist_kernel(bool wide, int mode, int nc, bool pair) {
  struct Row { bool wide; int mode, nc; bool pair; const void* fn; };
  static const Row rows[] = {
    {true, PM_OWN, 16, true, (const void*)tran_persistent_kernel<16, true, PM_OWN, true>}, {true, PM_OWN, 16, false, (const void*)tran_persistent_kernel<16, false, PM_OWN, true>},
    {true, PM_LOCKSTEP, 16, true, (const void*)tran_persistent_kernel<16, true, PM_LOCKSTEP, true>}, {true, PM_LOCKSTEP, 16, false, (const void*)tran_persistent_kernel<16, false, PM_LOCKSTEP, true>},
    {false, PM_BORDER, 16, true, (const void*)tran_persistent_kernel<16, true, PM_BORDER>}, {false, PM_BORDER, 16, false, (const void*)tran_persistent_kernel<16, false, PM_BORDER>},
    {false, PM_OWN, 12, true, (const void*)tran_persistent_kernel<12, true, PM_OWN>}, {false, PM_OWN, 12, false, (const void*)tran_persistent_kernel<12, false, PM_OWN>},
    {false, PM_OWN, 16, true, (const void*)tran_persistent_kernel<16, true, PM_OWN>}, {false, PM_OWN, 16, false, (const void*)tran_persistent_kernel<16, false, PM_OWN>},
    {false, PM_LOCKSTEP, 12, true, (const void*)tran_persistent_kernel<12, true>}, {false, PM_LOCKSTEP, 12, false, (const void*)tran_persistent_kernel<12, false>},
    {false, PM_LOCKSTEP, 16, true, (const void*)tran_persistent_kernel<16, true>}, {false, PM_LOCKSTEP, 16, false, (const void*)tran_persistent_kernel<16, false>},
  };
  for (const Row& r : rows) if (r.wide == wide && r.mode == mode && r.nc == nc && r.pair == pair) return r.fn;
  return nullptr;
}

struct PersistConsts {
  std::vector<int> ci; std::vector<double> cd; size_t max_ci = 0, max_cd = 0;
  std::vector<int> wgc, wgk;
  std::vector<double> bps_all;
};
inline bool ch_circuit::persist_consts(bool wg_consts, int n_wg, int bpw, double t0, double t1, PersistConsts& pc) {
  const int nblk = desc.A.n_comp * tab.S, nk = (int)desc.A.known.size(), nds = stru.n_dev_src();
  if (!wg_consts) {
    std::vector<int> kn(nk), ds(nds), need;
    std::iota(kn.begin(), kn.end(), 0); std::iota(ds.begin(), ds.end(), 0);
    if (!persist_blob(kn, ds, pc.ci, pc.cd, need)) { set_err("device-resident stepper: the source tables exceed the kernel's limits"); return false; }
    pc.max_ci = pc.ci.size(); pc.max_cd = pc.cd.size();
  } else {
    pc.wgk.assign((size_t)n_wg * P_MAXSRC, -1);
    for (int w = 0; w < n_wg; ++w) {
      std::vector<char> uk(nk, 0), ud(nds, 0);
      for (int b = w * bpw; b < std::min(nblk, (w + 1) * bpw); ++b)
        for (int i = 0; i < desc.A.comp_ndev[b]; ++i) {
          const EDev& e = desc.A.edev[desc.A.comp_dofs[b] + i];
          for (int k = 0; k < NTERM; ++k) if (e.term[k] < 0) uk[-e.term[k] - 1] = 1;
          if (e.src >= 0) ud[torn.dsrc_host[desc.A.comp_dofs[b] + i]] = 1;
        }
      std::vector<int> kn, ds, need, bi; std::vector<double> bd;
      for (int k = 0; k < nk; ++k) if (uk[k]) kn.push_back(k);
      for (int j = 0; j < nds; ++j) if (ud[j]) ds.push_back(j);
      if (ds.empty()) ds.push_back(0);
      if (!persist_blob(kn, ds, bi, bd, need)) { set_err("device-resident stepper: a workgroup's blocks reference more than 64 sources / known nodes"); return false; }
      for (size_t q = 0; q < kn.size(); ++q) pc.wgk[(size_t)w * P_MAXSRC + q] = kn[q];
      for (size_t q = 0; q < ds.size(); ++q) pc.wgk[(size_t)w * P_MAXSRC + kn.size() + q] = ds[q];
      std::vector<double> wb, wc;
      { std::vector<std::pair<double, double>> pts;
        for (int i : need) source_breakpoint_codes(desc.src[i], &tab.h_src_par[(size_t)i * CH_SRC_NPAR], t0, t1, pts);
        merge_breakpoints(pts, t1, wb, wc); }
      pc.wgc.insert(pc.wgc.end(), {(int)pc.ci.size(), (int)pc.cd.size(), (int)bi.size(), (int)bd.size(), (int)pc.bps_all.size(), (int)wb.size()});
      pc.ci.insert(pc.ci.end(), bi.begin(), bi.end()); pc.cd.insert(pc.cd.end(), bd.begin(), bd.end());
      pc.bps_all.insert(pc.bps_all.end(), wb.begin(), wb.end());
      pc.bps_all.insert(pc.bps_all.end(), wc.begin(), wc.end());
      pc.max_ci = std::max(pc.max_ci, bi.size()); pc.max_cd = std::max(pc.max_cd, bd.size());
    }
  }
  return true;
}

inline size_t ch_circuit::persist_va_arena(int bpw, size_t& lds) const {
  size_t va_arena = 0;
  if (desc.A.wide && !env_on(Env::VA_NO_LDS)) {
    size_t worst = 0;
    for (int cpt = 0; cpt < desc.A.n_comp; ++cpt) {
      size_t need = 0;
      for (int i = 0; i < desc.A.comp_ndev[cpt]; ++i) {
        const EDev& e = desc.A.edev[desc.A.comp_dofs[cpt] + i];
        if (e.kind != K_VA) continue;
        const int mod = desc.dev[e.hdev].ipar[0];
        need += (size_t)((va_gen::param_doubles(mod) + 1) & ~1) + (size_t)((va_gen::cache_doubles(mod) + 1) & ~1);
      }
      worst = std::max(worst, need);
    }
    const size_t room = lds < 148 * 1024 ? (148 * 1024 - lds) / sizeof(double) : 0;
    va_arena = std::min(worst * (size_t)bpw, room);
    lds += va_arena * sizeof(double);
    if (env_on(Env::DEBUG_STEPPER)) std::fprintf(stderr, "[stepper] compiled devices: %zu doubles per block, LDS arena %zu doubles, workgroup LDS %zu bytes\n", worst, va_arena, lds);
  }
  return va_arena;
}

inline int ch_circuit::persist_collect(ch_result& R, const TranCtl& cs, bool own_steps, bool single_batch, const std::vector<double>& htimes,
                                       const std::vector<double>& hpts, const std::vector<double>& hrows, int status, hclock::time_point tstart) {
  hipStream_t st = ctx->stream;
  const int n_obs = R.n_obs;
  stats.persist_attempts = cs.n_attempts;
  stats.persist_barrier_s = (double)cs.t_cycles_barrier * 1e-8;
#ifdef CH_STAMPS
  { static const char* nm[12] = {"set-up", "coefficients", "sources", "predictor", "eval", "gather", "rows+norm", "LU+solves", "update", "candidate", "grid-reduce", "controller"};
    std::fprintf(stderr, "[pstamps] attempts %lld; cycles per attempt (wave 0 of workgroup 0):", cs.n_attempts);
    for (int q = 0; q < 12; ++q) std::fprintf(stderr, " %s %.0f", nm[q], (double)cs.stamps[q] / (double)std::max<long long>(1, cs.n_attempts));
    std::fprintf(stderr, "\n"); }
#endif
  R.stats.naccept += cs.naccept; R.stats.nreject += cs.nreject; R.stats.nnonlinconvfail += cs.nconvfail;
  const long long arr_iters = (own_steps && tab.S == 1) ? cs.max_iters : cs.sum_iters;
  R.stats.n_block_iters += cs.sum_block_iters; R.stats.nnonliniter += arr_iters; R.stats.nf += arr_iters; R.stats.njacs += arr_iters;
  R.stats.nfactors += arr_iters; R.stats.nsolve += arr_iters;
  const size_t nt = htimes.size();
  R.times = htimes;
  R.pts.assign(nt, 0);
  if (own_steps == false) for (size_t r = 0; r < nt; ++r) R.pts[r] = (int32_t)hpts[r];
  R.values.assign((size_t)n_obs * nt * tab.S, 0.0);
  if (single_batch) {
    const size_t n = (size_t)n_obs * nt * tab.S;
    if (n > 0) {
      HIPCHK(ps.d_ptrans.alloc(n));
      hipLaunchKernelGGL(transpose_rows_kernel, dim3((unsigned)std::min<size_t>(65535, (n + 255) / 256)), dim3(256), 0, st, (const double*)ps.d_prows.p, ps.d_ptrans.p, (long)nt, (long)n_obs, tab.S);
      HIPCHK(hipGetLastError());
      HIPCHK(hipMemcpyAsync(R.values.data(), ps.d_ptrans.p, n * sizeof(double), hipMemcpyDeviceToHost, st));
      HIPCHK(hipStreamSynchronize(st));
      bool plain = true;
      for (int ob = 0; ob < n_obs && plain; ++ob) {
        if (stru.obs_primary[ob] != ob) plain = false;
        else if (desc.obs_kind[ob] == 0 && desc.A.node_unknown[desc.obs_index[ob]] < 0) plain = false;
        else if (desc.obs_kind[ob] == 1) { const int br = desc.dev[desc.obs_index[ob]].branch; if (br < 0 || desc.A.branch_unknown[br] < 0) plain = false; }
      }
      if (plain) { R.dev_values = ps.d_ptrans.p; R.dev_n = (int64_t)n; }
    }
  } else
  rows_to_obs_major(hrows.data(), nt, 0, nt, n_obs, tab.S, R.values.data());
  return finish_tran(R, 0, cs.t, status, tstart);
}

inline int ch_circuit::tran_persistent(double t0, double t1, const ch_tran_opts& o, ch_result& R, const std::vector<double>& bps, int kmax, double dtmin, double dtmax,
                                       int max_steps, int nmaxit, hclock::time_point tstart, bool& used, const ch_dc_opts* dcm, long long* dc_iters,
                                       const std::vector<double>* bpc) {
  used = false;
  hipStream_t st = ctx->stream;
  g_arena = &arena;
  const int n_obs = R.n_obs;
  const int nblk = desc.A.n_comp * tab.S, bpw = persist_bpw(nblk), n_wg = (nblk + bpw - 1) / bpw;
  const bool own_steps = persist_own_steps(o);
  const bool wg_consts = own_steps && tab.S == 1 && desc.A.n_comp > 1;
  const int nk = (int)desc.A.known.size(), nds = stru.n_dev_src();
  PersistConsts pc;
  if (!persist_consts(wg_consts, n_wg, bpw, t0, t1, pc)) return CH_OK;
  const size_t max_ci = pc.max_ci, max_cd = pc.max_cd;
  const size_t wave_d = persist_wave_doubles(wg_consts);
  size_t lds = (max_cd + (max_ci + 1) / 2 + PW * P_NREC + P_NREC + 4 + P_SCR + PW * wave_d) * sizeof(double);
  const size_t va_arena = persist_va_arena(bpw, lds);
  const bool pair = desc.A.wide ? stru.wide_split
                           : (desc.A.classes.size() == 1 && stru.h_cms[0].nslots <= 32 && !env_on(Env::PERSIST_NOPAIR));
  if (lds > 150 * 1024) { set_err("device-resident stepper: the workgroup's LDS footprint exceeds 150 KB"); return CH_OK; }
  const size_t row_d = std::max<size_t>(1, (size_t)n_obs * tab.S);
  long long max_rows;
  if (o.n_saveat > 0) max_rows = (long long)o.n_saveat + 1;
  else max_rows = std::min<long long>((long long)max_steps + 2, std::max<long long>(1024, std::min<long long>(1 << 20, (long long)((256u << 20) / (row_d * sizeof(double))))));
  if (o.n_saveat == 0 && env_on(Env::PERSIST_MAXROWS)) max_rows = std::max(2L, env_long(Env::PERSIST_MAXROWS, 0));
  if (dcm) max_rows = 2;
  HIPCHK(ps.d_pci.upload(pc.ci, st)); HIPCHK(ps.d_pcd.upload(pc.cd, st)); {
    std::vector<double> bpu = wg_consts ? pc.bps_all : bps;
    if (!wg_consts) for (size_t b = 0; b < bps.size(); ++b) bpu.push_back(bpc ? (*bpc)[b] : -1.0);
    HIPCHK(ps.d_pbps.upload(bpu, st));
  }
  if (wg_consts) { HIPCHK(ps.d_pwgc.upload(pc.wgc, st)); HIPCHK(ps.d_pwgk.upload(pc.wgk, st)); }
  { std::vector<double> sv(o.saveat, o.saveat + std::max(0, o.n_saveat)); if (sv.empty()) sv.push_back(0.0); HIPCHK(ps.d_psave.upload(sv, st)); }
  HIPCHK(ps.d_ptimes.alloc((size_t)2 * max_rows));  HIPCHK(ps.d_prows.alloc((size_t)max_rows * row_d));
  HIPCHK(ps.d_wgrec.alloc((size_t)2 * n_wg * 16)); HIPCHK(ps.d_grprec.alloc(2 * 8 * 16));  HIPCHK(ps.d_pcnt.alloc(10 * 32)); HIPCHK(ps.d_pctl.alloc(2));
  PersistArgs pa; std::memset(&pa, 0, sizeof(pa));
  pa.a = nwt.base;
  pa.a.mode = MODE_TRAN; pa.a.maxit = nmaxit; pa.a.abstol = o.abstol; pa.a.reltol = o.reltol; pa.a.newton_tol = 0.1; pa.a.active = nullptr; pa.a.gshunt = 0.0;
  pa.bpw = bpw; pa.wide_l = stru.wide_l; pa.wide_other = stru.wide_other; pa.va_arena = (int)va_arena;
  pa.nblk = nblk; pa.n_wg = n_wg; pa.red_max = (tab.S > 1 || own_steps) ? 1 : 0; pa.wave_doubles = (int)wave_d;
  pa.t1 = t1; pa.dtmin = dtmin; pa.dtmax = dtmax; pa.first_frac = FIRST_STEP_FRAC; pa.kmax = kmax; pa.max_steps = max_steps;
  pa.bps = ps.d_pbps.p; pa.nbp = (int)bps.size(); pa.saveat = ps.d_psave.p; pa.n_saveat = o.n_saveat;
  pa.ci = ps.d_pci.p; pa.cd = ps.d_pcd.p; pa.n_ci = (int)max_ci; pa.n_cd = (int)max_cd;
  pa.wgc = wg_consts ? ps.d_pwgc.p : nullptr; pa.wgk = wg_consts ? ps.d_pwgk.p : nullptr;
  pa.out_times = ps.d_ptimes.p; pa.out_rows = ps.d_prows.p; pa.max_rows = max_rows; pa.n_obs = n_obs;
  pa.ctl = ps.d_pctl.p; pa.wg_rec = ps.d_wgrec.p; pa.grp_rec = ps.d_grprec.p; pa.counters = ps.d_pcnt.p;
  pa.spin_ticks = 200000000LL;
  if (env_on(Env::SPIN_TICKS)) pa.spin_ticks = std::max(1L, env_long(Env::SPIN_TICKS, 0));
  pa.indep = own_steps ? 1 : 0;
  ps.mode = desc.A.nb > 0 ? CH_MODE_BORDERED : (own_steps ? CH_MODE_OWN_STEPS : CH_MODE_LOCKSTEP);
  if (dcm) {
    if (desc.A.nb == 0 || wg_consts) { set_err("internal: operating point on the device stepper is for the bordered form"); return CH_ERR_INTERNAL; }
    std::vector<double> sv, kv, ent;
    eval_sources(0.0, dcm->tran_mode ? 2 : 0, sv, kv);
    ent.assign(kv.begin(), kv.begin() + nk); ent.insert(ent.end(), sv.begin(), sv.begin() + nds);
    HIPCHK(ps.d_pdcent.upload(ent, st));
    pa.dc_mode = 1; pa.dc_maxit = std::max(1, dcm->maxiters); pa.dc_abstol = dcm->abstol; pa.dc_entries = ps.d_pdcent.p;
    pa.dv_max = (!desc.A.mos_hdev.empty() || desc.A.wide) ? dcm->dv_max : 0.0;
  }
  pa.nb = desc.A.nb; pa.n_glob = desc.A.n_glob; pa.n_bdev = (int)desc.A.border_dev.size();
  for (int q = 0; q < pa.n_bdev; ++q) {
    const Analysis::BorderDev& bd = desc.A.border_dev[q];
    pa.bd_kind[q] = bd.kind; pa.bd_ta[q] = bd.ta; pa.bd_tb[q] = bd.tb;
    pa.bd_val[q] = bd.kind == K_R ? torn.h_dmult0[bd.hdev] / torn.h_dpar0[bd.hdev] : torn.h_dmult0[bd.hdev] * torn.h_dpar0[bd.hdev];
  }
  const bool coop = !pa.indep;
  pa.pair_dbg = (int)env_long(Env::PAIR_DBG, 0);
  TranCtl cs; std::memset(&cs, 0, sizeof(cs));
  cs.t = t0; cs.h = start_step(o.dt0, t0, t1, dtmin, dtmax, bps[0]); cs.k = 1; cs.nhist = 1; cs.reset_rate = 1; cs.tslot[0] = t0;
  const void* fn = persist_kernel(desc.A.wide, desc.A.wide ? (own_steps ? PM_OWN : PM_LOCKSTEP) : desc.A.nb > 0 ? PM_BORDER : (own_steps ? PM_OWN : PM_LOCKSTEP),
                                  (desc.A.wide || desc.A.nb > 0 || stru.lu_variant > 12) ? 16 : 12, pair);
  if (!fn) { set_err("internal: no device-stepper kernel for this form"); return CH_ERR_INTERNAL; }
  {
    hipFuncAttributes fa;
    HIPCHK(hipFuncGetAttributes(&fa, fn));
    if (lds + fa.sharedSizeBytes > 160 * 1024) { set_err("device-resident stepper: LDS footprint"); return CH_OK; }
    HIPCHK(hipFuncSetAttribute(fn, hipFuncAttributeMaxDynamicSharedMemorySize, (int)((160 * 1024 - (int)fa.sharedSizeBytes) & ~255)));
  }
  std::vector<double> hrows, htimes, hpts;
  bool single_batch = false;
  std::vector<std::vector<double>> row_store;
  int resume = 0, status = CH_OK;
  for (;;) {
    HIPCHK(hipMemcpyAsync(ps.d_pctl.p, &cs, sizeof(cs), hipMemcpyHostToDevice, st));
    HIPCHK(hipMemcpyAsync(ps.d_pctl.p + 1, &cs, sizeof(cs), hipMemcpyHostToDevice, st));
    HIPCHK(hipMemsetAsync(ps.d_pcnt.p, 0, 10 * 32 * sizeof(unsigned), st));
    HIPCHK(hipMemsetAsync(ps.d_ptimes.p + max_rows, 0, (size_t)max_rows * sizeof(double), st));
    if (pa.indep) HIPCHK(hipMemsetAsync(ps.d_prows.p, 0xff, (size_t)max_rows * row_d * sizeof(double), st));
    HIPCHK(hipMemsetAsync(ps.d_wgrec.p, 0, (size_t)2 * n_wg * 16 * sizeof(double), st)); HIPCHK(hipMemsetAsync(ps.d_grprec.p, 0, 2 * 8 * 16 * sizeof(double), st));
    pa.resume = resume;
    void* kargs[] = {(void*)&pa};
    HIPCHK(hipEventRecord(nwt.ev0, st));
    const hipError_t le = coop ? hipLaunchCooperativeKernel(fn, dim3(n_wg), dim3(PW * 64), kargs, (unsigned)lds, st)
                               : hipLaunchKernel(fn, dim3(n_wg), dim3(PW * 64), kargs, lds, st);
    if (le != hipSuccess) {
      (void)hipGetLastError();
      if (resume == 0) { set_err(std::string("cooperative launch refused: ") + hipGetErrorString(le)); return CH_OK; }
      set_err(std::string("device-resident stepper: relaunch failed: ") + hipGetErrorString(le)); used = true; return CH_ERR_DEVICE;
    }
    HIPCHK(hipEventRecord(nwt.ev1, st));
    used = true;
    { const hipError_t se = hipStreamSynchronize(st); if (se != hipSuccess) { set_err(std::string("device-resident stepper: ") + hipGetErrorString(se)); return CH_ERR_DEVICE; } }
    { float ms = 0; HIPCHK(hipEventElapsedTime(&ms, nwt.ev0, nwt.ev1)); stats.persist_ms += ms; stats.persist_launches += 1; }
    HIPCHK(hipMemcpy(&cs, ps.d_pctl.p + (pa.indep ? 1 : 0), sizeof(cs), hipMemcpyDeviceToHost));
    const size_t nr = (size_t)cs.nsaved;
    const size_t base_t = htimes.size();
    single_batch = resume == 0 && cs.exit_reason != PX_ROWS_FULL && !dcm;
    htimes.resize(base_t + nr); hpts.resize(base_t + nr);
    if (!single_batch) hrows.resize((base_t + nr) * row_d);
    if (nr > 0) {
      HIPCHK(hipMemcpy(htimes.data() + base_t, ps.d_ptimes.p, nr * sizeof(double), hipMemcpyDeviceToHost));
      HIPCHK(hipMemcpy(hpts.data() + base_t, ps.d_ptimes.p + max_rows, nr * sizeof(double), hipMemcpyDeviceToHost));
      if (!single_batch) HIPCHK(hipMemcpy(hrows.data() + base_t * row_d, ps.d_prows.p, nr * row_d * sizeof(double), hipMemcpyDeviceToHost));
    }
    if (cs.exit_reason == PX_ROWS_FULL) { cs.nsaved = 0; resume = 1; continue; }
    if (cs.exit_reason == PX_ABORT) {
      ps.aborted = true;
      unsigned code = 0; (void)hipMemcpy(&code, ps.d_pcnt.p + 9 * 32, sizeof(code), hipMemcpyDeviceToHost);
      set_err("device-resident stepper: a wait exceeded its bound (site " + std::to_string(code & 255u) + ", sequence " + std::to_string(code >> 8) +
              ", attempts " + std::to_string((long long)cs.n_attempts) + "; workgroups not co-resident?)");
      status = CH_ERR_DEVICE;
    }
    else status = cs.status;
    break;
  }
  if (dcm) {
    if (dc_iters) *dc_iters = cs.sum_iters;
    if (cs.exit_reason == PX_ABORT && status == CH_OK) status = CH_ERR_DEVICE;
    return status;
  }
  return persist_collect(R, cs, own_steps, single_batch, htimes, hpts, hrows, status, tstart);
}

inline int ch_circuit::dc_border(const ch_dc_opts& o, long long* iters) {
  const auto td0 = hclock::now();
  auto lap = [&](const char* what) { if (env_on(Env::DEBUG_TORN)) std::fprintf(stderr, "[torn] dc_border %s at %.3f ms\n", what, 1e3 * std::chrono::duration<double>(hclock::now() - td0).count()); };
  int rc = finalize_params();
  if (rc != CH_OK) return rc;
  lap("finalized");
  std::string why;
  if (!torn.is_torn || !persist_eligible(why, false)) { set_err("bordered operating point: " + why); return CH_ERR_UNSUPPORTED; }
  std::vector<double> xm((size_t)tab.S * desc.A.n_mna, 0.0);
  if (o.x0) std::copy(o.x0, o.x0 + xm.size(), xm.begin());
  else { Rng rng(o.seed); for (double& v : xm) v = 1e-7 * rng.normal(); }
  lap("start vector");
  rc = upload_from_mna(0, xm.data());
  if (rc != CH_OK) return rc;
  lap("uploaded");
  ch_tran_opts to; std::memset(&to, 0, sizeof(to));
  to.abstol = 1e-6; to.reltol = 1e-3; to.max_order = 1;
  ch_result tmp; tmp.S = tab.S; tmp.n_obs = (int)desc.obs_kind.size();
  const std::vector<double> one_bp{1.0};
  const double save_ms = stats.persist_ms; const long save_l = stats.persist_launches;
  bool used = false;
  const auto tq0 = hclock::now();
  rc = tran_persistent(0.0, 1.0, to, tmp, one_bp, 1, 1e-15, 0.1, 10, 10, hclock::now(), used, &o, iters);
  if (env_on(Env::DEBUG_TORN)) std::fprintf(stderr, "[torn] dc_border: kernel %.3f ms, call %.3f ms\n", stats.persist_ms - save_ms, 1e3 * std::chrono::duration<double>(hclock::now() - tq0).count());
  stats.persist_ms = save_ms; stats.persist_launches = save_l;
  if (!used && rc == CH_OK) return CH_ERR_UNSUPPORTED;
  return rc;
}

inline int ch_circuit::tran_torn(double t0, double t1, const ch_tran_opts& o, ch_result& R, bool& used) {
  used = false;
  auto tstart = hclock::now();
  int rc = finalize_params();
  if (rc != CH_OK) return rc;
  std::vector<double> x_mna((size_t)tab.S * desc.A.n_mna, 0.0);
  ch_stats dcst; std::memset(&dcst, 0, sizeof(dcst));
  stats.reset();
  ch_circuit* tc = torn.c.get();
  bool dc_on_torn = false;
  if (o.skip_dc) { if (o.dc.x0) std::copy(o.dc.x0, o.dc.x0 + x_mna.size(), x_mna.begin()); }
  else {
    if (!env_on(Env::TORN_DC_SPARSE)) {
      long long it = 0;
      ArenaScope sc(&tc->arena);
      const int r = tc->dc_border(o.dc, &it);
      if (r == CH_OK) { dc_on_torn = true; dcst.nnonliniter = it; dcst.nf = dcst.njacs = dcst.nfactors = dcst.nsolve = it; dcst.n_block_iters = it * tc->desc.A.n_comp; }
      else { torn.note = "bordered operating point: " + err(); ctx->err.clear(); }
      if (env_on(Env::DEBUG_TORN)) std::fprintf(stderr, "[torn] operating point on the device stepper: rc %d, %lld iterations, %.3f ms%s%s\n", r, it,
                                                           1e3 * std::chrono::duration<double>(hclock::now() - tstart).count(), r == CH_OK ? "" : " -> sparse path: ", r == CH_OK ? "" : torn.note.c_str());
    }
    if (!dc_on_torn) {
      rc = dc_solve(o.dc, 0, nullptr, &dcst);
      if (rc != CH_OK) { used = true; return rc; }
      rc = download_mna(0, t0, 1, x_mna.data());
      if (rc != CH_OK) return rc;
    }
  }
  const double dc_s = std::chrono::duration<double>(hclock::now() - tstart).count();
  const long dc_l = stats.n_launch;
  ch_tran_opts o2 = o; o2.skip_dc = 1; o2.dc.x0 = dc_on_torn ? nullptr : x_mna.data(); o2.stepper = CH_STEPPER_DEVICE;
  { ArenaScope sc(&tc->arena); tc->torn.keep_slot0 = dc_on_torn; rc = tc->tran_solve(t0, t1, o2, R); tc->torn.keep_slot0 = false; }
  if (rc == CH_ERR_UNSUPPORTED || (rc == CH_ERR_DEVICE && tc->ps.aborted)) { torn.note = err(); ctx->err.clear(); return CH_OK; }
  used = true;
  R.stats.dc_seconds = dc_s; R.stats.wall_seconds += dc_s; R.stats.n_kernel_launches += dc_l;
  R.stats.nf += dcst.nf; R.stats.njacs += dcst.njacs; R.stats.nfactors += dcst.nfactors; R.stats.nsolve += dcst.nsolve;
  R.stats.nnonliniter += dcst.nnonliniter; R.stats.nrestarts += dcst.nrestarts; R.stats.n_block_iters += dcst.n_block_iters;
  return rc;
}
```

cedarsim.jl_amd/csrc/ch_stepper_host.hpp:

```cpp
#pragma once

#include <algorithm>
#include <cmath>
#include <cstring>
#include <utility>
#include <vector>

#include "ch_analysis.hpp"
#include "ch_env.hpp"

namespace chip {

inline double pwl_at_time(const double* ts, const double* ys, int n, double t) {
  if (n == 0) return 0.0;
  int i = (int)(std::lower_bound(ts, ts + n, t) - ts) + 1;
  if (i <= n && ts[i - 1] == t) ++i;
  if (i <= 1) return ys[0];
  if (i > n) return ys[n - 1];
  if (ys[i - 2] == ys[i - 1]) return ys[i - 1];
  if (ts[i - 1] == ts[i - 2]) return 0.5 * (ys[i - 2] + ys[i - 1]);
  return ys[i - 2] + (t - ts[i - 2]) * ((ys[i - 1] - ys[i - 2]) / (ts[i - 1] - ts[i - 2]));
}
inline double sind(double deg) { return std::sin(std::fmod(deg, 360.0) * (3.14159265358979323846 / 180.0)); }
inline double source_value(const HSource& s, const double* par, double dc, double t, int mode) {
  if (mode == 0) return dc;
  if (mode == 2) t = 0.0;
  switch (s.kind) {
    case CH_SRC_DC: return par[0];
    case CH_SRC_PWL: return pwl_at_time(s.ts.data(), s.ys.data(), (int)s.ts.size(), t);
    case CH_SRC_PULSE: {
      const double td = par[2], tr = par[3], tf = par[4], pw = par[5], per = par[6];
      const double ts[4] = {td, td + tr, td + tr + pw, td + tr + pw + tf}, ys[4] = {par[0], par[1], par[1], par[0]};
      return pwl_at_time(ts, ys, 4, std::isfinite(per) ? std::fmod(t, per) : t);
    }
    case CH_SRC_SIN: {
      const double vo = par[0], va = par[1], f = par[2], td = par[3], th = par[4], ph = par[5], nc = par[6];
      if (td < t && t < nc / f) return vo + va * std::exp(-(t - td) * th) * sind(360.0 * f * (t - td) + ph);
      return vo + va * sind(ph);
    }
  }
  return 0.0;
}
inline void source_breakpoints(const HSource& s, const double* par, double t0, double t1, std::vector<double>& out) {
  if (s.kind == CH_SRC_PWL) { for (double t : s.ts) if (t > t0 && t < t1) out.push_back(t); }
  else if (s.kind == CH_SRC_PULSE) {
    const double td = par[2], tr = par[3], tf = par[4], pw = par[5], per = par[6];
    const double c[4] = {td, td + tr, td + tr + pw, td + tr + pw + tf};
    if (!std::isfinite(per) || per <= 0) { for (double t : c) if (t > t0 && t < t1) out.push_back(t); }
    else {
      long k0 = std::max(0L, (long)std::floor(t0 / per) - 1);
      for (long k = k0; k * per < t1 && (k - k0) < 10000000; ++k) {
        for (double tc : c) { double t = tc + k * per; if (t > t0 && t < t1) out.push_back(t); }
        if (k >= 1 && k * per > t0 && k * per < t1) out.push_back(k * per);
      }
    }
  } else if (s.kind == CH_SRC_SIN) {
    const double te = par[6] / par[2];
    if (par[3] > t0 && par[3] < t1) out.push_back(par[3]);
    if (std::isfinite(te) && te > t0 && te < t1) out.push_back(te);
  }
}

inline bool source_jumps_at(const HSource& s, const double* par, double t) {
  double amp = 0.0;
  if (s.kind == CH_SRC_PWL) for (double y : s.ys) amp = std::max(amp, std::fabs(y));
  else if (s.kind == CH_SRC_PULSE) amp = std::max(std::fabs(par[0]), std::fabs(par[1]));
  else if (s.kind == CH_SRC_SIN) amp = std::fabs(par[0]) + std::fabs(par[1]);
  const double a = source_value(s, par, 0.0, std::nextafter(t, -INFINITY), 1), b = source_value(s, par, 0.0, t, 1);
  return std::fabs(a - b) > 1e-9 * amp;
}

inline void source_breakpoint_codes(const HSource& s, const double* par, double t0, double t1, std::vector<std::pair<double, double>>& out) {
  const bool restart_all = env_on(Env::BP_RESTART_ALL);
  std::vector<double> own;
  source_breakpoints(s, par, t0, t1, own);
  std::sort(own.begin(), own.end());
  for (size_t j = 0; j < own.size(); ++j) {
    const double seg = (j + 1 < own.size() ? own[j + 1] : t1) - own[j];
    out.emplace_back(own[j], (restart_all || source_jumps_at(s, par, own[j])) ? -1.0 : seg);
  }
}
inline void merge_breakpoints(std::vector<std::pair<double, double>>& pts, double t1, std::vector<double>& bps, std::vector<double>& bpc) {
  pts.emplace_back(t1, -1.0);
  std::sort(pts.begin(), pts.end());
  bps.clear(); bpc.clear();
  for (const auto& pt : pts) {
    if (!bps.empty() && bps.back() == pt.first) { bpc.back() = (bpc.back() < 0 || pt.second < 0) ? -1.0 : std::min(bpc.back(), pt.second); continue; }
    bps.push_back(pt.first); bpc.push_back(pt.second);
  }
}

inline void bdf_coeffs(const double* tau, int k, double* alpha) {
  double a0 = 0;
  for (int m = 1; m <= k; ++m) a0 += 1.0 / (tau[0] - tau[m]);
  alpha[0] = a0;
  for (int j = 1; j <= k; ++j) {
    double num = 1, den = 1;
    for (int m = 1; m <= k; ++m) if (m != j) num *= (tau[0] - tau[m]);
    for (int m = 0; m <= k; ++m) if (m != j) den *= (tau[j] - tau[m]);
    alpha[j] = num / den;
  }
}
inline void extrap_weights(const double* tau, int np, double* w) {
  for (int j = 1; j <= np; ++j) { double v = 1; for (int i = 1; i <= np; ++i) if (i != j) v *= (tau[0] - tau[i]) / (tau[j] - tau[i]); w[j] = v; }
}

constexpr int NSLOT = 8;
constexpr double FIRST_STEP_FRAC = 1e-3;

inline double first_step(double h, double t, double next_bp, double dtmin) {
  return std::max(10 * dtmin, std::min(h, (next_bp - t) / 50.0) * FIRST_STEP_FRAC);
}
inline double start_step(double dt0, double t0, double t1, double dtmin, double dtmax, double first_bp) {
  const double span = t1 - t0;
  const double h = dt0 > 0 ? dt0 : std::min(dtmax, 1e-3 * span);
  return first_step(h, t0, first_bp, dtmin);
}

inline int resolve_stepper(int opt, const char* ev, bool device_known = true) {
  if (opt != CH_STEPPER_AUTO || !ev) return opt;
  if (std::strcmp(ev, "host") == 0) return CH_STEPPER_HOST;
  return (device_known && std::strcmp(ev, "device") == 0) ? CH_STEPPER_DEVICE : CH_STEPPER_AUTO;
}

inline void rows_to_obs_major(const double* rows_in, size_t rows, size_t row0, size_t nt, int n_obs, int S, double* values) {
  for (size_t r = 0; r < rows; ++r) for (int ob = 0; ob < n_obs; ++ob)
    std::copy(rows_in + (r * n_obs + ob) * S, rows_in + (r * n_obs + ob + 1) * S, values + ((size_t)ob * nt + row0 + r) * S);
}

struct LaunchStats {
  double device_ms = 0; long n_launch = 0, n_timed = 0;
  double prof_launch = 0, prof_wait = 0, prof_reduce = 0;
  double persist_ms = 0; long persist_launches = 0; long long persist_attempts = 0; double persist_barrier_s = 0;
  double dc_device_ms = 0; long dc_launches = 0, dc_timed = 0; long long dc_block_iters = 0;
  void reset() { *this = LaunchStats(); }
  void end_of_dc(long long block_iters) { dc_device_ms = device_ms; dc_launches = n_launch; dc_timed = n_timed; dc_block_iters = block_iters; }
  static double scaled_seconds(double ms, long launches, long timed) { return timed > 0 ? ms * 1e-3 * (double)launches / (double)timed : 0.0; }
  void fill(ch_stats& s) const {
    s.device_seconds = scaled_seconds(device_ms, n_launch, n_timed) + persist_ms * 1e-3;
    const bool dev = persist_launches > 0;
    s.step_kernel_launches = dev ? persist_launches : n_launch - dc_launches;
    s.step_kernel_seconds = dev ? persist_ms * 1e-3 : scaled_seconds(device_ms - dc_device_ms, n_launch - dc_launches, n_timed - dc_timed);
  }
};

struct StepCoeffs {
  int k = 0, npred = 0, nkm1 = 0, nkp1 = 0;
  double alpha[8] = {0}, wpred[8] = {0}, wkm1[8] = {0}, wkp1[8] = {0};
  double ck = 0, ckm1 = 0, ckp1 = 0;
  int hist_slot[8] = {0}, cand_slot = 0;
};

struct StepControl {
  const double t1, dtmin, dtmax; const int kmax;
  const std::vector<double>& bps; const std::vector<double>& bpc;
  double t, h;
  int k = 1, nhist = 1, steps_at_order = 0;
  bool reset_rate = true;
  size_t ibp = 0;
  int order[NSLOT]; double htime[NSLOT] = {0};
  double tn = 0, hh = 0, tb_code = -1.0;
  bool hit_bp = false, lte = false, try_up = false;
  int kk = 1, np = 1, nh = 1;
  StepCoeffs c;

  StepControl(double t0, double t1_, double dt0, double dtmin_, double dtmax_, int kmax_, const std::vector<double>& bps_, const std::vector<double>& bpc_)
      : t1(t1_), dtmin(dtmin_), dtmax(dtmax_), kmax(kmax_), bps(bps_), bpc(bpc_), t(t0), h(start_step(dt0, t0, t1_, dtmin_, dtmax_, bps_[0])) {
    for (int i = 0; i < NSLOT; ++i) order[i] = i;
    htime[0] = t0;
  }
  bool tb_jump() const { return tb_code < 0; }
  int dense_points() const { return std::min(kk, nh) + 1; }

  int plan() {
    while (ibp < bps.size() && bps[ibp] <= t * (1 + 1e-15) + 1e-300) ++ibp;
    const double tb = ibp < bps.size() ? bps[ibp] : t1;
    tb_code = ibp < bps.size() ? bpc[ibp] : -1.0;
    hit_bp = false;
    tn = t + h;
    if (tn >= tb - 1e-3 * h) { tn = tb; hit_bp = true; }
    hh = tn - t;
    if (hh < dtmin) return CH_ERR_DTMIN;
    nh = nhist; kk = std::min(k, nh); np = std::min(kk + 1, nh);
    double tau[9];
    tau[0] = tn; for (int j = 0; j < nh && j < 7; ++j) tau[j + 1] = htime[j];
    extrap_weights(tau, np, c.wpred); c.npred = np;
    bdf_coeffs(tau, kk, c.alpha); c.k = kk;
    lte = np >= kk + 1;
    c.ck = lte ? hh / (tn - tau[kk + 1]) : 0.0;
    c.nkm1 = 0; c.nkp1 = 0; c.ckm1 = 0; c.ckp1 = 0;
    try_up = lte && kk < kmax && nh >= kk + 2 && steps_at_order + 1 >= kk + 1;
    if (lte && kk > 1) { extrap_weights(tau, kk, c.wkm1); c.nkm1 = kk; c.ckm1 = hh / (tn - tau[kk]); }
    if (try_up) { extrap_weights(tau, kk + 2, c.wkp1); c.nkp1 = kk + 2; c.ckp1 = hh / (tn - tau[kk + 2]); }
    for (int j = 0; j < 7; ++j) c.hist_slot[j] = order[std::min(j, nh - 1)];
    c.cand_slot = order[NSLOT - 1];
    return CH_OK;
  }
  double source_time() const { return hit_bp ? std::nextafter(tn, -INFINITY) : tn; }

  void on_convergence_failure() {
    reset_rate = true;
    h = hh * 0.25; k = 1; steps_at_order = 0;
    if (nhist > 2) nhist = 2;
  }
  void on_error_test_failure(double errk) {
    const double fac = 0.9 * std::pow(2.0 * errk + 1e-4, -1.0 / (kk + 1));
    h = hh * std::min(0.9, std::max(0.25, fac));
    steps_at_order = 0;
  }
  void on_accept() {
    reset_rate = false;
    int cand = order[NSLOT - 1];
    for (int j = NSLOT - 1; j > 0; --j) { order[j] = order[j - 1]; htime[j] = htime[j - 1]; }
    order[0] = cand; htime[0] = tn; nhist = std::min(nhist + 1, kmax + 2);
  }
  int dense_weights(double ts, double* ww) const {
    double tt[9]; const int m = dense_points();
    tt[0] = ts; for (int j = 0; j < m; ++j) tt[j + 1] = htime[j];
    extrap_weights(tt, m, ww);
    return m;
  }
  void select_next(double errk, double errkm1, double errkp1) {
    const double fac_k = std::pow(2.0 * errk + 1e-4, -1.0 / (kk + 1));
    double best = fac_k; int knew = kk;
    if (lte) {
      ++steps_at_order;
      if (kk > 1) { const double f = std::pow(2.0 * errkm1 + 1e-4, -1.0 / kk); if (f > best) { best = f; knew = kk - 1; } }
      if (try_up) { const double f = std::pow(2.0 * errkp1 + 1e-4, -1.0 / (kk + 2)); if (f > 1.1 * best) { best = f; knew = kk + 1; } }
    } else knew = 1;
    if (knew != kk) steps_at_order = 0;
    k = knew;
    if (best > 1.0 && best < 1.2) best = 1.0;
    h = std::min(dtmax, hh * std::min(kk == 1 ? 10.0 : 2.0, std::max(0.5, best)));
    t = tn;
    if (hit_bp && t < t1 && !tb_jump()) {
      reset_rate = true;
      h = std::max(dtmin * 10, std::min(h, tb_code / 10.0));
    }
    if (hit_bp && t < t1 && tb_jump()) {
      nhist = 1; k = 1; steps_at_order = 0; reset_rate = true;
      double nb = t1;
      for (size_t b = ibp; b < bps.size(); ++b) if (bps[b] > t * (1 + 1e-15)) { nb = bps[b]; break; }
      h = first_step(h, t, nb, dtmin);
    }
  }
};

}
```

Before: 52370.

## Cache start vectors, stage persistent-stepper uploads, and overlap host prep with DC kernel

Caches the random DC start vector per seed in pinned memory and uploads it asynchronously instead of regenerating it and doing synchronous copies. The persistent-stepper's many small device buffers are consolidated into a single staged pinned/device region, and control readback uses async copies into pinned memory. Host-side breakpoint and blob preparation can run while the first DC Newton kernel executes. A phase-timing profiler and a precomputed unknown-to-block map are added. The aim is fewer host-device round trips and synchronous waits per solve, at the cost of cached state that must stay consistent across calls.

```diff
diff --git a/cedarsim.jl_amd/csrc/ch_engine.hip b/cedarsim.jl_amd/csrc/ch_engine.hip
--- a/cedarsim.jl_amd/csrc/ch_engine.hip
+++ b/cedarsim.jl_amd/csrc/ch_engine.hip
@@ -7,6 +7,7 @@
 #include <cmath>
 #include <cstdio>
 #include <cstring>
+#include <functional>
 #include <map>
 #include <memory>
 #include <new>
@@ -33,18 +34,6 @@
   hipStream_t stream = nullptr;
   std::string err;
 };
-
-namespace {
-
-struct Rng {
-  uint64_t s;
-  explicit Rng(uint64_t seed) : s(seed) {}
-  uint64_t next() { uint64_t z = (s += 0x9E3779B97F4A7C15ull); z = (z ^ (z >> 30)) * 0xBF58476D1CE4E5B9ull; z = (z ^ (z >> 27)) * 0x94D049BB133111EBull; return z ^ (z >> 31); }
-  double uniform() { return ((next() >> 11) + 0.5) * (1.0 / 9007199254740992.0); }
-  double normal() { double u1 = uniform(), u2 = uniform(); return std::sqrt(-2.0 * std::log(u1)) * std::cos(6.283185307179586 * u2); }
-};
-
-}
 
 struct ch_result {
   std::vector<double> times, values, final_state;
@@ -74,6 +63,7 @@
   std::vector<int> needed_src;
   std::vector<int> dev_src;
   int n_dev_src() const { return std::max<int>(1, (int)dev_src.size()); }
+  std::vector<int> unk_block;
   int block_threads = 64, lu_variant = 16;
   bool wide_split = false; int wide_l = 0, wide_other = 0;
   size_t lds_doubles_fixed = 0, lds_extra_bytes = 0;
@@ -216,6 +206,7 @@
   int path = 1;
   NewtonArgs base;
   mutable std::vector<double> all_src; std::vector<double> sv_buf, kv_buf;
+  StartVectorCache start; PinnedBuf<double> h_x0; bool h_x0_current = false;
 };
 struct SparsePath {
   SparsePlan plan[2];
@@ -231,8 +222,21 @@
   DevBuf<int> act[3]; DevBuf<double> scale;
   PinnedBuf<int> h_act; PinnedBuf<double> h_scale;
 };
+struct PersistPrep {
+  bool ready = false;
+  PersistArgs pa; TranCtl cs; const void* fn = nullptr; size_t lds = 0, row_d = 1, zero_bytes = 0; long long max_rows = 0;
+  int n_wg = 0; bool coop = true, own_steps = false;
+};
 struct DeviceStepper {
-  DevBuf<int> d_pci; DevBuf<double> d_pcd, d_pbps, d_psave, d_ptimes, d_prows, d_wgrec, d_grprec; DevBuf<unsigned> d_pcnt; DevBuf<TranCtl> d_pctl; DevBuf<int> d_pwgc, d_pwgk; DevBuf<double> d_pdcent, d_ptrans;
+  DevBuf<double> d_ptimes, d_prows, d_ptrans;
+  StageLayout lay;
+  PinnedBuf<unsigned char> h_stage;
+  DevBuf<unsigned char> d_stage;
+  DevBuf<unsigned char> d_zero;
+  PinnedBuf<unsigned char> h_ret;
+  size_t h_ret_bytes = 0;
+  const void* attr_fn = nullptr; size_t attr_static_lds = 0;
+  PersistPrep prep;
   int n_cu = 0, mode = 0; bool aborted = false;
 };
 struct SmallSignal {
@@ -252,6 +256,7 @@
   ch_ctx* ctx = nullptr;
   Description desc; Structure stru; SampleTables tab; NewtonState nwt;
   SparsePath sp; DeviceStepper ps; SmallSignal ac; TornCompanion torn; LaunchStats stats;
+  HostSplit hsplit;
   const bool host_profile = env_on(Env::HOST_PROFILE);
   const long time_every = std::max(1L, env_long(Env::TIME_EVERY, 8));
 
@@ -280,6 +285,8 @@
     HIPCHK(stru.d_dmask.upload(dm, st)); HIPCHK(stru.d_obs_unk.upload(obs_unk, st));
     HIPCHK(nwt.h_sum.alloc(1, hipHostMallocMapped)); HIPCHK(nwt.ev0.create()); HIPCHK(nwt.ev1.create());
     stru.size_lds(desc);
+    stru.unk_block.resize(desc.A.n_unk);
+    for (int u = 0; u < desc.A.n_unk; ++u) stru.unk_block[u] = (int)(std::upper_bound(desc.A.comp_uofs.begin(), desc.A.comp_uofs.end(), u) - desc.A.comp_uofs.begin()) - 1;
     return CH_OK;
   }
 
@@ -535,29 +542,45 @@
   int ac_ndev(int comp) const { return nwt.path == 2 ? (int)desc.A.edev.size() : desc.A.comp_ndev[comp]; }
   const BlockMeta* ac_bmeta();
 
+  hipError_t sync_wait() { ++hsplit.waits; return hipStreamSynchronize(ctx->stream); }
+  hipError_t copy_wait(void* dst, const void* src, size_t bytes, hipMemcpyKind kind) { ++hsplit.waits; return hipMemcpy(dst, src, bytes, kind); }
   int poll_stream(const char* what) {
+    ++hsplit.waits;
     hipError_t q = hipErrorNotReady;
     for (int spin = 0; spin < 200000 && q == hipErrorNotReady; ++spin) q = hipStreamQuery(ctx->stream);
     if (q == hipErrorNotReady) q = hipStreamSynchronize(ctx->stream);
     if (q != hipSuccess) { set_err(std::string(what) + hipGetErrorString(q)); return CH_ERR_DEVICE; }
     return CH_OK;
   }
-  int run_newton(const NewtonArgs& a, const unsigned char* host_active, Summary& out) {
-    if (nwt.path == 2) return run_sparse(a, host_active, out);
+  void launch_newton(const NewtonArgs& a, hipEvent_t e0, hipEvent_t e1) {
+    hipStream_t st = ctx->stream;
+    const dim3 g(desc.A.n_comp * tab.S), b(stru.block_threads);
+    static void (*const kernels[])(const NewtonArgs) = {newton_block_kernel<16, true>, newton_block_kernel<0, true>, newton_block_kernel<8>, newton_block_kernel<12>,
+                                                        newton_block_kernel<16>, newton_block_kernel<32>, newton_block_kernel<0>};
+    const int lu = stru.lu_variant, ki = desc.A.wide ? (lu == 16 ? 0 : 1) : lu == 8 ? 2 : lu == 12 ? 3 : lu == 16 ? 4 : lu == 32 ? 5 : 6;
+    hipExtLaunchKernelGGL(kernels[ki], g, b, (uint32_t)nwt.lds_bytes, st, e0, e1, 0, a);
+    if (!nwt.host_reduce) hipLaunchKernelGGL(reduce_blocks_kernel, dim3(1), dim3(256), 9 * 256 * sizeof(double), st, a);
+  }
+  int enqueue_newton(const NewtonArgs& a) {
+    launch_newton(a, nullptr, nullptr);
+    HIPCHK(hipGetLastError());
+    stats.n_launch += 1;
+    return CH_OK;
+  }
+  int run_newton(const NewtonArgs& a, const unsigned char* host_active, Summary& out, const std::function<int()>* overlap = nullptr) {
+    if (nwt.path == 2) { const int orc = overlap ? (*overlap)() : CH_OK; const int rrc = run_sparse(a, host_active, out); return orc != CH_OK ? orc : rrc; }
     hipStream_t st = ctx->stream;
     const int nblk = desc.A.n_comp * tab.S;
     const bool timed = time_every <= 1 || ((uint64_t)(stats.n_launch + 1) * 0x9E3779B97F4A7C15ull >> 33) % (uint64_t)time_every == 0;
     const auto tp0 = host_profile ? hclock::now() : hclock::time_point();
     hipEvent_t e0 = timed ? nwt.ev0.e : nullptr, e1 = timed ? nwt.ev1.e : nullptr;
-    const dim3 g(nblk), b(stru.block_threads);
-    static void (*const kernels[])(const NewtonArgs) = {newton_block_kernel<16, true>, newton_block_kernel<0, true>, newton_block_kernel<8>, newton_block_kernel<12>,
-                                                        newton_block_kernel<16>, newton_block_kernel<32>, newton_block_kernel<0>};
-    const int lu = stru.lu_variant, ki = desc.A.wide ? (lu == 16 ? 0 : 1) : lu == 8 ? 2 : lu == 12 ? 3 : lu == 16 ? 4 : lu == 32 ? 5 : 6;
-    hipExtLaunchKernelGGL(kernels[ki], g, b, (uint32_t)nwt.lds_bytes, st, e0, e1, 0, a);
-    if (!nwt.host_reduce) hipLaunchKernelGGL(reduce_blocks_kernel, dim3(1), dim3(256), 9 * 256 * sizeof(double), st, a);
+    launch_newton(a, e0, e1);
     const auto tp1 = host_profile ? hclock::now() : hclock::time_point();
+    const int orc = overlap ? (*overlap)() : CH_OK;
+    const auto tp1b = host_profile ? hclock::now() : hclock::time_point();
     { const int prc = poll_stream("newton kernel: "); if (prc != CH_OK) return prc; }
     HIPCHK(hipGetLastError());
+    if (orc != CH_OK) return orc;
     const auto tp2 = host_profile ? hclock::now() : hclock::time_point();
     if (timed) { float ms = 0; HIPCHK(hipEventElapsedTime(&ms, nwt.ev0, nwt.ev1)); stats.device_ms += ms; stats.n_timed += 1; }
     stats.n_launch += 1;
@@ -582,7 +605,7 @@
     }
     if (host_profile) {
       const auto tp3 = hclock::now();
-      stats.prof_launch += std::chrono::duration<double>(tp1 - tp0).count(); stats.prof_wait += std::chrono::duration<double>(tp2 - tp1).count();
+      stats.prof_launch += std::chrono::duration<double>(tp1 - tp0).count(); stats.prof_wait += std::chrono::duration<double>(tp2 - tp1b).count();
       stats.prof_reduce += std::chrono::duration<double>(tp3 - tp2).count();
     }
     return CH_OK;
@@ -590,7 +613,11 @@
 
   int download_mna(int slot, double t, int mode, double* x_out) {
     std::vector<double> xs((size_t)tab.S * desc.A.n_unk);
-    HIPCHK(hipMemcpy(xs.data(), nwt.d_X.p + (size_t)slot * tab.S * desc.A.n_unk, xs.size() * sizeof(double), hipMemcpyDeviceToHost));
+    HIPCHK(copy_wait(xs.data(), nwt.d_X.p + (size_t)slot * tab.S * desc.A.n_unk, xs.size() * sizeof(double), hipMemcpyDeviceToHost));
+    unknowns_to_mna(xs.data(), t, mode, x_out);
+    return CH_OK;
+  }
+  void unknowns_to_mna(const double* xs, double t, int mode, double* x_out) const {
     std::vector<double> sv, kv; eval_sources(t, mode, sv, kv);
     const int nk = (int)desc.A.known.size();
     for (int s = 0; s < tab.S; ++s) {
@@ -598,7 +625,6 @@
       for (int n = 1; n <= desc.n_nodes; ++n) xo[n - 1] = desc.A.node_unknown[n] >= 0 ? xs[(size_t)s * desc.A.n_unk + desc.A.node_unknown[n]] : kv[(size_t)(tab.Ssrc > 1 ? s : 0) * nk + desc.A.node_known[n]];
       for (int b = 0; b < desc.A.n_branch; ++b) xo[desc.n_nodes + b] = desc.A.branch_unknown[b] >= 0 ? xs[(size_t)s * desc.A.n_unk + desc.A.branch_unknown[b]] : CH_NAN;
     }
-    return CH_OK;
   }
   int upload_from_mna(int slot, const double* x_mna) {
     std::vector<double> xs((size_t)tab.S * desc.A.n_unk);
@@ -607,7 +633,9 @@
     return CH_OK;
   }
 
-  int dc_solve(const ch_dc_opts& o, int slot, std::vector<int>* status_out, ch_stats* stt) {
+  int dc_solve(const ch_dc_opts& o, int slot, std::vector<int>* status_out, ch_stats* stt, const std::function<int()>* overlap = nullptr) {
+    PhaseClock pcl(host_profile ? &hsplit : nullptr);
+    hipStream_t st = ctx->stream;
     const int mode = o.tran_mode ? 2 : 0;
     const int nblk = desc.A.n_comp * tab.S;
     int rc = CH_OK;
@@ -620,38 +648,62 @@
     a.hist_slot[0] = slot; a.cand_slot = slot; a.active = nwt.d_active.p;
     rc = set_sources(a, 0.0, mode);
     if (rc != CH_OK) return rc;
-    std::vector<Rng> rngs; for (int s = 0; s < tab.S; ++s) rngs.emplace_back(o.seed + (uint64_t)s);
-    auto block_of_unknown = [&](int u) { int c = (int)(std::upper_bound(desc.A.comp_uofs.begin(), desc.A.comp_uofs.end(), u) - desc.A.comp_uofs.begin()) - 1; return c; };
+    std::vector<Rng> rngs;
+    if (!o.x0) {
+      if (!nwt.start.lookup(o.seed, desc.A.n_mna, tab.S)) nwt.h_x0_current = false;
+      rngs = nwt.start.after;
+    } else for (int s = 0; s < tab.S; ++s) rngs.emplace_back(o.seed + (uint64_t)s);
+    double* const dX = nwt.d_X.p + (size_t)slot * tab.S * desc.A.n_unk;
     int n_active = nblk;
     std::vector<unsigned char> donor_ok(nblk, 0);
     const int nrest = std::max(1, o.n_restarts);
     for (int r = 0; r < nrest + 1 && n_active > 0; ++r) {
       const bool homotopy = (r == nrest);
-      HIPCHK(hipMemcpy(xs.data(), nwt.d_X.p + (size_t)slot * tab.S * desc.A.n_unk, xs.size() * sizeof(double), hipMemcpyDeviceToHost));
-      for (int s = 0; s < tab.S; ++s) {
-        bool any = false;
-        for (int c = 0; c < desc.A.n_comp; ++c) if (active[(size_t)c * tab.S + s]) any = true;
-        if (!any) continue;
-        if (!homotopy) {
-          if (r == 0 && o.x0) for (int i = 0; i < desc.A.n_mna; ++i) xm[i] = o.x0[(size_t)s * desc.A.n_mna + i];
-          else for (int i = 0; i < desc.A.n_mna; ++i) xm[i] = 1e-7 * rngs[s].normal();
-        } else std::fill(xm.begin(), xm.end(), 0.0);
-        for (int u = 0; u < desc.A.n_unk; ++u) if (active[(size_t)block_of_unknown(u) * tab.S + s]) xs[(size_t)s * desc.A.n_unk + u] = xm[desc.A.unk_mna[u]];
+      if (r == 0 && !o.x0) {
+        const size_t nx = xs.size();
+        if (nwt.h_x0.n < nx) { HIPCHK(nwt.h_x0.alloc(std::max<size_t>(1, nx))); nwt.h_x0_current = false; }
+        if (!nwt.h_x0_current) {
+          for (int s = 0; s < tab.S; ++s) for (int u = 0; u < desc.A.n_unk; ++u) nwt.h_x0[(size_t)s * desc.A.n_unk + u] = nwt.start.x[(size_t)s * desc.A.n_mna + desc.A.unk_mna[u]];
+          nwt.h_x0_current = true;
+        }
+        pcl.to(HP_DC_START);
+        hipError_t ue = nx > 0 ? hipMemcpyAsync(dX, nwt.h_x0.p, nx * sizeof(double), hipMemcpyHostToDevice, st) : hipSuccess;
+        if (ue == hipSuccess) ue = hipMemsetAsync(nwt.d_active.p, 1, nblk, st);
+        if (ue != hipSuccess) { (void)sync_wait(); set_err(std::string("operating point: start vector upload: ") + hipGetErrorString(ue)); return CH_ERR_DEVICE; }
+        pcl.to(HP_DC_COPIES);
+      } else {
+        if (r > 0) HIPCHK(copy_wait(xs.data(), dX, xs.size() * sizeof(double), hipMemcpyDeviceToHost));
+        pcl.to(HP_DC_COPIES);
+        for (int s = 0; s < tab.S; ++s) {
+          bool any = false;
+          for (int c = 0; c < desc.A.n_comp; ++c) if (active[(size_t)c * tab.S + s]) any = true;
+          if (!any) continue;
+          if (!homotopy) {
+            if (r == 0 && o.x0) for (int i = 0; i < desc.A.n_mna; ++i) xm[i] = o.x0[(size_t)s * desc.A.n_mna + i];
+            else for (int i = 0; i < desc.A.n_mna; ++i) xm[i] = 1e-7 * rngs[s].normal();
+          } else std::fill(xm.begin(), xm.end(), 0.0);
+          for (int u = 0; u < desc.A.n_unk; ++u) if (active[(size_t)stru.unk_block[u] * tab.S + s]) xs[(size_t)s * desc.A.n_unk + u] = xm[desc.A.unk_mna[u]];
+        }
+        if (r == 1 && tab.S > 1) {
+          for (int c = 0; c < desc.A.n_comp; ++c) {
+            int donor = -1;
+            for (int s = 0; s < tab.S && donor < 0; ++s) if (!active[(size_t)c * tab.S + s] && donor_ok[(size_t)c * tab.S + s]) donor = s;
+            if (donor < 0) continue;
+            for (int s = 0; s < tab.S; ++s) if (active[(size_t)c * tab.S + s])
+              for (int u = desc.A.comp_uofs[c]; u < desc.A.comp_uofs[c] + desc.A.comp_nc[c]; ++u) xs[(size_t)s * desc.A.n_unk + u] = xs[(size_t)donor * desc.A.n_unk + u];
+          }
+        }
+        pcl.to(HP_DC_START);
+        HIPCHK(copy_wait(dX, xs.data(), xs.size() * sizeof(double), hipMemcpyHostToDevice));
+        HIPCHK(copy_wait(nwt.d_active.p, active.data(), nblk, hipMemcpyHostToDevice));
+        pcl.to(HP_DC_COPIES);
       }
-      if (r == 1 && tab.S > 1) {
-        for (int c = 0; c < desc.A.n_comp; ++c) {
-          int donor = -1;
-          for (int s = 0; s < tab.S && donor < 0; ++s) if (!active[(size_t)c * tab.S + s] && donor_ok[(size_t)c * tab.S + s]) donor = s;
-          if (donor < 0) continue;
-          for (int s = 0; s < tab.S; ++s) if (active[(size_t)c * tab.S + s])
-            for (int u = desc.A.comp_uofs[c]; u < desc.A.comp_uofs[c] + desc.A.comp_nc[c]; ++u) xs[(size_t)s * desc.A.n_unk + u] = xs[(size_t)donor * desc.A.n_unk + u];
-        }
-      }
-      HIPCHK(hipMemcpy(nwt.d_X.p + (size_t)slot * tab.S * desc.A.n_unk, xs.data(), xs.size() * sizeof(double), hipMemcpyHostToDevice));
-      HIPCHK(hipMemcpy(nwt.d_active.p, active.data(), nblk, hipMemcpyHostToDevice));
       Summary sm;
       if (!homotopy) {
-        rc = run_newton(a, active.data(), sm);
+        const double ov0 = hsplit.s[HP_BP_BLOB] + hsplit.s[HP_UPLOADS];
+        rc = run_newton(a, active.data(), sm, r == 0 ? overlap : nullptr);
+        pcl.to(HP_DC_WAIT);
+        hsplit.s[HP_DC_WAIT] -= hsplit.s[HP_BP_BLOB] + hsplit.s[HP_UPLOADS] - ov0;
         if (rc != CH_OK) return rc;
       } else {
         for (double g = 1e-2; g >= 1e-13 * 0.99; g *= 0.1) { a.gshunt = g; rc = run_newton(a, active.data(), sm); if (rc != CH_OK) return rc; }
@@ -661,7 +713,7 @@
       }
       if (stt) { stt->n_block_iters += sm.sum_block_iters; stt->nnonliniter += sm.sum_iters; stt->nf += sm.sum_iters; stt->njacs += sm.sum_iters; stt->nfactors += sm.sum_iters; stt->nsolve += sm.sum_iters; }
       if (nwt.path == 2) { for (int b = 0; b < nblk; ++b) bo[b].status = sp.status_v[b % tab.S]; }
-      else if (nwt.host_reduce) std::memcpy(bo.data(), nwt.h_out, nblk * sizeof(BlockOut)); else HIPCHK(hipMemcpy(bo.data(), nwt.d_out.p, nblk * sizeof(BlockOut), hipMemcpyDeviceToHost));
+      else if (nwt.host_reduce) std::memcpy(bo.data(), nwt.h_out, nblk * sizeof(BlockOut)); else HIPCHK(copy_wait(bo.data(), nwt.d_out.p, nblk * sizeof(BlockOut), hipMemcpyDeviceToHost));
       n_active = 0;
       for (int b = 0; b < nblk; ++b) if (active[b]) { if (bo[b].status == 0) { active[b] = 0; donor_ok[b] = 1; } else ++n_active; }
       if (n_active > 0 && stt) { stt->nrestarts++; stt->nnonlinconvfail++; }
@@ -677,8 +729,12 @@
   size_t persist_wave_doubles(bool wg_consts) const;
   bool persist_blob(const std::vector<int>& kn, const std::vector<int>& ds, std::vector<int>& bi, std::vector<double>& bd, std::vector<int>& need) const;
   size_t persist_va_arena(int bpw, size_t& lds) const;
-  int persist_collect(ch_result& R, const TranCtl& cs, bool own_steps, bool single_batch, const std::vector<double>& htimes, const std::vector<double>& hpts,
+  int persist_collect(ch_result& R, const TranCtl& cs, bool own_steps, bool single_batch, size_t nr, const std::vector<double>& htimes, const std::vector<double>& hpts,
                       const std::vector<double>& hrows, int status, hclock::time_point tstart);
+  size_t persist_ret_head() const;
+  int persist_zero(const PersistPrep& P);
+  int persist_prepare(double t0, double t1, const ch_tran_opts& o, int n_obs, const std::vector<double>& bps, const std::vector<double>* bpc, int kmax, double dtmin,
+                      double dtmax, int max_steps, int nmaxit, const ch_dc_opts* dcm);
   bool persist_consts(bool wg_consts, int n_wg, int bpw, double t0, double t1, PersistConsts& pc);
   int tran_persistent(double t0, double t1, const ch_tran_opts& o, ch_result& R, const std::vector<double>& bps, int kmax, double dtmin, double dtmax,
                       int max_steps, int nmaxit, hclock::time_point tstart, bool& used, const ch_dc_opts* dcm = nullptr, long long* dc_iters = nullptr,
@@ -771,22 +827,8 @@
     const double dtmax = o.dtmax > 0 ? o.dtmax : span / 10.0, dtmin = o.dtmin > 0 ? o.dtmin : 1e-15 * span;
     const int max_steps = o.max_steps > 0 ? o.max_steps : 100000 , nmaxit = o.newton_maxiters > 0 ? o.newton_maxiters : 10;
     const int n_obs = R.n_obs;
-
-    if (o.skip_dc) {
-      if (o.dc.x0) { rc = upload_from_mna(0, o.dc.x0); if (rc != CH_OK) return rc; }
-      else if (!torn.keep_slot0) HIPCHK(hipMemsetAsync(nwt.d_X.p, 0, (size_t)tab.S * desc.A.n_unk * sizeof(double), st));
-    } else {
-      rc = dc_solve(o.dc, 0, nullptr, &R.stats);
-      if (rc != CH_OK) return rc;
-    }
-    R.stats.dc_seconds = std::chrono::duration<double>(hclock::now() - tstart).count();
-    {
-      NewtonArgs a = nwt.base; a.mode = MODE_EVAL; a.maxit = 1; a.hist_slot[0] = 0; a.cand_slot = 0; a.abstol = o.abstol; a.reltol = o.reltol;
-      rc = set_sources(a, t0, 1); if (rc != CH_OK) return rc;
-      Summary sm; rc = run_newton(a, nullptr, sm); if (rc != CH_OK) return rc;
-      R.stats.nf += tab.S;
-    }
-    stats.end_of_dc(R.stats.n_block_iters);
+    PhaseClock pcl(host_profile ? &hsplit : nullptr);
+    ps.prep.ready = false;
 
     std::vector<double> bps, bpc;
     {
@@ -795,10 +837,39 @@
       for (int s = 0; s < tab.Ssrc; ++s) for (int i = 0; i < nsrc; ++i) source_breakpoint_codes(desc.src[i], &tab.h_src_par[((size_t)s * nsrc + i) * CH_SRC_NPAR], t0, t1, pts);
       merge_breakpoints(pts, t1, bps, bpc);
     }
+    pcl.to(HP_BP_BLOB);
+
+    std::function<int()> prepare;
+    if (!o.skip_dc && nwt.path == 1 && resolve_stepper(o.stepper, env_get(Env::STEPPER)) != CH_STEPPER_HOST) {
+      std::string why;
+      if (persist_eligible(why, persist_own_steps(o)))
+        prepare = [&]() { return persist_prepare(t0, t1, o, n_obs, bps, &bpc, kmax, dtmin, dtmax, max_steps, nmaxit, nullptr); };
+    }
+    if (o.skip_dc) {
+      if (o.dc.x0) { rc = upload_from_mna(0, o.dc.x0); if (rc != CH_OK) return rc; }
+      else if (!torn.keep_slot0) HIPCHK(hipMemsetAsync(nwt.d_X.p, 0, (size_t)tab.S * desc.A.n_unk * sizeof(double), st));
+    } else {
+      rc = dc_solve(o.dc, 0, nullptr, &R.stats, prepare ? &prepare : nullptr);
+      if (rc != CH_OK) { ps.prep.ready = false; return rc; }
+    }
+    R.stats.dc_seconds = std::chrono::duration<double>(hclock::now() - tstart).count();
+    pcl.skip();
+    {
+      NewtonArgs a = nwt.base; a.mode = MODE_EVAL; a.maxit = 1; a.hist_slot[0] = 0; a.cand_slot = 0; a.abstol = o.abstol; a.reltol = o.reltol;
+      rc = set_sources(a, t0, 1); if (rc != CH_OK) { ps.prep.ready = false; return rc; }
+      if (ps.prep.ready) rc = enqueue_newton(a);
+      else { Summary sm; rc = run_newton(a, nullptr, sm); }
+      if (rc != CH_OK) { ps.prep.ready = false; (void)sync_wait(); return rc; }
+      R.stats.nf += tab.S;
+    }
+    pcl.to(HP_T0_EVAL);
+    stats.end_of_dc(R.stats.n_block_iters);
+
     if (nwt.d_perm.p) HIPCHK(hipMemsetAsync(nwt.d_perm.p, 0, (size_t)desc.A.n_comp * tab.S * 16, ctx->stream));
 
     { bool done = false;
       rc = try_device_stepper(t0, t1, o, R, bps, bpc, kmax, dtmin, dtmax, max_steps, nmaxit, tstart, done);
+      ps.prep.ready = false;
       if (done) return rc; }
 
     StepControl sc(t0, t1, o.dt0, dtmin, dtmax, kmax, bps, bpc);
@@ -856,7 +927,8 @@
     return finish_tran(R, sc.order[0], sc.t, status, tstart);
   }
 
-  int finish_tran(ch_result& R, int newest_slot, double t, int status, hclock::time_point tstart) {
+  int finish_tran(ch_result& R, int newest_slot, double t, int status, hclock::time_point tstart, const double* xs_final = nullptr) {
+    PhaseClock pcl(host_profile ? &hsplit : nullptr);
     const int n_obs = R.n_obs;
     const size_t nt = R.times.size();
     {
@@ -874,15 +946,23 @@
         }
       }
     }
+    pcl.to(HP_COLLECT);
     R.final_state.assign((size_t)tab.S * desc.A.n_mna, 0.0);
-    download_mna(newest_slot, t, 1, R.final_state.data());
+    if (xs_final) unknowns_to_mna(xs_final, t, 1, R.final_state.data());
+    else download_mna(newest_slot, t, 1, R.final_state.data());
+    pcl.to(HP_FINAL_STATE);
 #ifdef CH_STAMPS
     { unsigned long long hs[8]; (void)hipMemcpy(hs, stru.d_stamps.p, sizeof(hs), hipMemcpyDeviceToHost);
       std::fprintf(stderr, "[stamps] cycles summed over blocks: prologue %llu eval %llu gather %llu solve %llu epilogue %llu arrival %llu pre-LU %llu LU %llu ; launches %ld blocks %d\n", hs[0], hs[1], hs[2], hs[3], hs[4], hs[5], hs[6], hs[7], stats.n_launch, desc.A.n_comp * tab.S); }
 #endif
     R.status = status;
     R.stats.wall_seconds = std::chrono::duration<double>(hclock::now() - tstart).count();
-    if (host_profile) { std::fprintf(stderr, "[host profile] wall %.3f ms; in run_newton: launch %.3f ms, wait %.3f ms, events+reduce %.3f ms; launches %ld\n", 1e3 * R.stats.wall_seconds, 1e3 * stats.prof_launch, 1e3 * stats.prof_wait, 1e3 * stats.prof_reduce, stats.n_launch); stats.prof_launch = stats.prof_wait = stats.prof_reduce = 0; }
+    if (host_profile) {
+      std::fprintf(stderr, "[host profile] wall %.3f ms; in run_newton: launch %.3f ms, wait %.3f ms, events+reduce %.3f ms; launches %ld; split [ms]:", 1e3 * R.stats.wall_seconds, 1e3 * stats.prof_launch, 1e3 * stats.prof_wait, 1e3 * stats.prof_reduce, stats.n_launch);
+      for (int q = 0; q < HP_COUNT; ++q) std::fprintf(stderr, " %s %.3f%s", HostSplit::name(q), 1e3 * hsplit.s[q], q + 1 < HP_COUNT ? "," : "");
+      std::fprintf(stderr, "; blocking waits %ld\n", hsplit.waits);
+      stats.prof_launch = stats.prof_wait = stats.prof_reduce = 0; hsplit = HostSplit();
+    }
     stats.fill(R.stats);
     R.stats.n_kernel_launches = stats.n_launch + stats.persist_launches;
     R.stats.n_step_attempts += stats.persist_attempts; R.stats.barrier_seconds = stats.persist_barrier_s;
diff --git a/cedarsim.jl_amd/csrc/ch_engine_persist.hpp b/cedarsim.jl_amd/csrc/ch_engine_persist.hpp
--- a/cedarsim.jl_amd/csrc/ch_engine_persist.hpp
+++ b/cedarsim.jl_amd/csrc/ch_engine_persist.hpp
@@ -143,9 +143,10 @@
   return va_arena;
 }
 
-inline int ch_circuit::persist_collect(ch_result& R, const TranCtl& cs, bool own_steps, bool single_batch, const std::vector<double>& htimes,
+inline int ch_circuit::persist_collect(ch_result& R, const TranCtl& cs, bool own_steps, bool single_batch, size_t nr, const std::vector<double>& htimes,
                                        const std::vector<double>& hpts, const std::vector<double>& hrows, int status, hclock::time_point tstart) {
   hipStream_t st = ctx->stream;
+  PhaseClock pc(host_profile ? &hsplit : nullptr);
   const int n_obs = R.n_obs;
   stats.persist_attempts = cs.n_attempts;
   stats.persist_barrier_s = (double)cs.t_cycles_barrier * 1e-8;
@@ -159,39 +160,70 @@
   const long long arr_iters = (own_steps && tab.S == 1) ? cs.max_iters : cs.sum_iters;
   R.stats.n_block_iters += cs.sum_block_iters; R.stats.nnonliniter += arr_iters; R.stats.nf += arr_iters; R.stats.njacs += arr_iters;
   R.stats.nfactors += arr_iters; R.stats.nsolve += arr_iters;
-  const size_t nt = htimes.size();
-  R.times = htimes;
+  if (!single_batch) {
+    const size_t nt = htimes.size();
+    R.times = htimes;
+    R.pts.assign(nt, 0);
+    if (own_steps == false) for (size_t r = 0; r < nt; ++r) R.pts[r] = (int32_t)hpts[r];
+    R.values.assign((size_t)n_obs * nt * tab.S, 0.0);
+    rows_to_obs_major(hrows.data(), nt, 0, nt, n_obs, tab.S, R.values.data());
+    pc.to(HP_COLLECT);
+    return finish_tran(R, 0, cs.t, status, tstart);
+  }
+  const size_t nt = nr, n = (size_t)n_obs * nt * tab.S, nx = (size_t)tab.S * desc.A.n_unk;
+  const bool pinned_values = n * sizeof(double) <= ((size_t)8 << 20);
+  R.values.assign(n, 0.0);
+  if (n > 0) HIPCHK(ps.d_ptrans.alloc(n));
+  const size_t head = persist_ret_head(), need = head + (2 * nt + nx + (pinned_values ? n : 0)) * sizeof(double);
+  if (need > ps.h_ret_bytes) { HIPCHK(ps.h_ret.alloc(need + need / 2)); ps.h_ret_bytes = need + need / 2; }
+  double* const ht = (double*)(ps.h_ret.p + head); double* const hp = ht + nt; double* const hx = hp + nt; double* const hv = hx + nx;
+  hipError_t ce = hipSuccess;
+  auto q = [&](hipError_t e) { if (ce == hipSuccess) ce = e; };
+  if (nt > 0) {
+    q(hipMemcpyAsync(ht, ps.d_ptimes.p, nt * sizeof(double), hipMemcpyDeviceToHost, st));
+    q(hipMemcpyAsync(hp, ps.d_ptimes.p + ps.prep.max_rows, nt * sizeof(double), hipMemcpyDeviceToHost, st));
+  }
+  if (n > 0) {
+    hipLaunchKernelGGL(transpose_rows_kernel, dim3((unsigned)std::min<size_t>(65535, (n + 255) / 256)), dim3(256), 0, st, (const double*)ps.d_prows.p, ps.d_ptrans.p, (long)nt, (long)n_obs, tab.S);
+    q(hipGetLastError());
+    q(hipMemcpyAsync(pinned_values ? hv : R.values.data(), ps.d_ptrans.p, n * sizeof(double), hipMemcpyDeviceToHost, st));
+  }
+  if (nx > 0) q(hipMemcpyAsync(hx, nwt.d_X.p, nx * sizeof(double), hipMemcpyDeviceToHost, st));
+  { const hipError_t se = sync_wait();
+    if (ce != hipSuccess || se != hipSuccess) { set_err(std::string("device-resident stepper: collecting the result: ") + hipGetErrorString(ce != hipSuccess ? ce : se)); return CH_ERR_DEVICE; } }
+  R.times.assign(ht, ht + nt);
   R.pts.assign(nt, 0);
-  if (own_steps == false) for (size_t r = 0; r < nt; ++r) R.pts[r] = (int32_t)hpts[r];
-  R.values.assign((size_t)n_obs * nt * tab.S, 0.0);
-  if (single_batch) {
-    const size_t n = (size_t)n_obs * nt * tab.S;
-    if (n > 0) {
-      HIPCHK(ps.d_ptrans.alloc(n));
-      hipLaunchKernelGGL(transpose_rows_kernel, dim3((unsigned)std::min<size_t>(65535, (n + 255) / 256)), dim3(256), 0, st, (const double*)ps.d_prows.p, ps.d_ptrans.p, (long)nt, (long)n_obs, tab.S);
-      HIPCHK(hipGetLastError());
-      HIPCHK(hipMemcpyAsync(R.values.data(), ps.d_ptrans.p, n * sizeof(double), hipMemcpyDeviceToHost, st));
-      HIPCHK(hipStreamSynchronize(st));
-      bool plain = true;
-      for (int ob = 0; ob < n_obs && plain; ++ob) {
-        if (stru.obs_primary[ob] != ob) plain = false;
-        else if (desc.obs_kind[ob] == 0 && desc.A.node_unknown[desc.obs_index[ob]] < 0) plain = false;
-        else if (desc.obs_kind[ob] == 1) { const int br = desc.dev[desc.obs_index[ob]].branch; if (br < 0 || desc.A.branch_unknown[br] < 0) plain = false; }
-      }
-      if (plain) { R.dev_values = ps.d_ptrans.p; R.dev_n = (int64_t)n; }
-    }
-  } else
-  rows_to_obs_major(hrows.data(), nt, 0, nt, n_obs, tab.S, R.values.data());
-  return finish_tran(R, 0, cs.t, status, tstart);
-}
-
-inline int ch_circuit::tran_persistent(double t0, double t1, const ch_tran_opts& o, ch_result& R, const std::vector<double>& bps, int kmax, double dtmin, double dtmax,
-                                       int max_steps, int nmaxit, hclock::time_point tstart, bool& used, const ch_dc_opts* dcm, long long* dc_iters,
-                                       const std::vector<double>* bpc) {
-  used = false;
+  if (own_steps == false) for (size_t r = 0; r < nt; ++r) R.pts[r] = (int32_t)hp[r];
+  if (pinned_values && n > 0) std::memcpy(R.values.data(), hv, n * sizeof(double));
+  if (n > 0) {
+    bool plain = true;
+    for (int ob = 0; ob < n_obs && plain; ++ob) {
+      if (stru.obs_primary[ob] != ob) plain = false;
+      else if (desc.obs_kind[ob] == 0 && desc.A.node_unknown[desc.obs_index[ob]] < 0) plain = false;
+      else if (desc.obs_kind[ob] == 1) { const int br = desc.dev[desc.obs_index[ob]].branch; if (br < 0 || desc.A.branch_unknown[br] < 0) plain = false; }
+    }
+    if (plain) { R.dev_values = ps.d_ptrans.p; R.dev_n = (int64_t)n; }
+  }
+  pc.to(HP_COLLECT);
+  return finish_tran(R, 0, cs.t, status, tstart, hx);
+}
+
+inline size_t ch_circuit::persist_ret_head() const { return StageLayout::pad(2 * sizeof(TranCtl) + sizeof(unsigned)); }
+
+inline int ch_circuit::persist_zero(const PersistPrep& P) {
   hipStream_t st = ctx->stream;
-  g_arena = &arena;
-  const int n_obs = R.n_obs;
+  HIPCHK(hipMemsetAsync(ps.d_zero.p, 0, P.zero_bytes, st));
+  HIPCHK(hipMemsetAsync(ps.d_ptimes.p + P.max_rows, 0, (size_t)P.max_rows * sizeof(double), st));
+  if (P.pa.indep) HIPCHK(hipMemsetAsync(ps.d_prows.p, 0xff, (size_t)P.max_rows * P.row_d * sizeof(double), st));
+  return CH_OK;
+}
+
+inline int ch_circuit::persist_prepare(double t0, double t1, const ch_tran_opts& o, int n_obs, const std::vector<double>& bps, const std::vector<double>* bpc, int kmax,
+                                       double dtmin, double dtmax, int max_steps, int nmaxit, const ch_dc_opts* dcm) {
+  PersistPrep& P = ps.prep;
+  P.ready = false;
+  hipStream_t st = ctx->stream;
+  PhaseClock pcl(host_profile ? &hsplit : nullptr);
   const int nblk = desc.A.n_comp * tab.S, bpw = persist_bpw(nblk), n_wg = (nblk + bpw - 1) / bpw;
   const bool own_steps = persist_own_steps(o);
   const bool wg_consts = own_steps && tab.S == 1 && desc.A.n_comp > 1;
@@ -205,43 +237,69 @@
   const bool pair = desc.A.wide ? stru.wide_split
                            : (desc.A.classes.size() == 1 && stru.h_cms[0].nslots <= 32 && !env_on(Env::PERSIST_NOPAIR));
   if (lds > 150 * 1024) { set_err("device-resident stepper: the workgroup's LDS footprint exceeds 150 KB"); return CH_OK; }
+  if (dcm && (desc.A.nb == 0 || wg_consts)) { set_err("internal: operating point on the device stepper is for the bordered form"); return CH_ERR_INTERNAL; }
+  const void* fn = persist_kernel(desc.A.wide, desc.A.wide ? (own_steps ? PM_OWN : PM_LOCKSTEP) : desc.A.nb > 0 ? PM_BORDER : (own_steps ? PM_OWN : PM_LOCKSTEP),
+                                  (desc.A.wide || desc.A.nb > 0 || stru.lu_variant > 12) ? 16 : 12, pair);
+  if (!fn) { set_err("internal: no device-stepper kernel for this form"); return CH_ERR_INTERNAL; }
+  if (ps.attr_fn != fn) {
+    hipFuncAttributes fa;
+    HIPCHK(hipFuncGetAttributes(&fa, fn));
+    HIPCHK(hipFuncSetAttribute(fn, hipFuncAttributeMaxDynamicSharedMemorySize, (int)((160 * 1024 - (int)fa.sharedSizeBytes) & ~255)));
+    ps.attr_fn = fn; ps.attr_static_lds = fa.sharedSizeBytes;
+  }
+  if (lds + ps.attr_static_lds > 160 * 1024) { set_err("device-resident stepper: LDS footprint"); return CH_OK; }
   const size_t row_d = std::max<size_t>(1, (size_t)n_obs * tab.S);
   long long max_rows;
   if (o.n_saveat > 0) max_rows = (long long)o.n_saveat + 1;
   else max_rows = std::min<long long>((long long)max_steps + 2, std::max<long long>(1024, std::min<long long>(1 << 20, (long long)((256u << 20) / (row_d * sizeof(double))))));
   if (o.n_saveat == 0 && env_on(Env::PERSIST_MAXROWS)) max_rows = std::max(2L, env_long(Env::PERSIST_MAXROWS, 0));
   if (dcm) max_rows = 2;
-  HIPCHK(ps.d_pci.upload(pc.ci, st)); HIPCHK(ps.d_pcd.upload(pc.cd, st)); {
-    std::vector<double> bpu = wg_consts ? pc.bps_all : bps;
-    if (!wg_consts) for (size_t b = 0; b < bps.size(); ++b) bpu.push_back(bpc ? (*bpc)[b] : -1.0);
-    HIPCHK(ps.d_pbps.upload(bpu, st));
-  }
-  if (wg_consts) { HIPCHK(ps.d_pwgc.upload(pc.wgc, st)); HIPCHK(ps.d_pwgk.upload(pc.wgk, st)); }
-  { std::vector<double> sv(o.saveat, o.saveat + std::max(0, o.n_saveat)); if (sv.empty()) sv.push_back(0.0); HIPCHK(ps.d_psave.upload(sv, st)); }
+  pcl.to(HP_BP_BLOB);
+  const size_t n_sv = (size_t)std::max(1, o.n_saveat), n_ent = dcm ? (size_t)nk + nds : 0;
+  ps.lay.plan(pc.ci.size(), pc.cd.size(), wg_consts ? pc.bps_all.size() : 2 * bps.size(), n_sv, sizeof(TranCtl), wg_consts ? pc.wgc.size() : 0, wg_consts ? pc.wgk.size() : 0, n_ent);
+  if (ps.h_stage.n < ps.lay.capacity) HIPCHK(ps.h_stage.alloc(ps.lay.capacity));
+  if (ps.d_stage.n < ps.lay.capacity || !ps.d_stage.p) HIPCHK(ps.d_stage.alloc(ps.lay.capacity));
+  const size_t head = persist_ret_head();
+  if (ps.h_ret_bytes < head) { HIPCHK(ps.h_ret.alloc(head)); ps.h_ret_bytes = head; }
+  const StagePointers hs(ps.lay, ps.h_stage.p), ds(ps.lay, ps.d_stage.p);
+  if (!pc.ci.empty()) std::memcpy(hs.ci, pc.ci.data(), pc.ci.size() * sizeof(int));
+  if (!pc.cd.empty()) std::memcpy(hs.cd, pc.cd.data(), pc.cd.size() * sizeof(double));
+  if (wg_consts) {
+    if (!pc.bps_all.empty()) std::memcpy(hs.bps, pc.bps_all.data(), pc.bps_all.size() * sizeof(double));
+    std::memcpy(hs.wgc, pc.wgc.data(), pc.wgc.size() * sizeof(int)); std::memcpy(hs.wgk, pc.wgk.data(), pc.wgk.size() * sizeof(int));
+  } else {
+    std::memcpy(hs.bps, bps.data(), bps.size() * sizeof(double));
+    for (size_t b = 0; b < bps.size(); ++b) hs.bps[bps.size() + b] = bpc ? (*bpc)[b] : -1.0;
+  }
+  hs.saveat[0] = 0.0;
+  for (int i = 0; i < o.n_saveat; ++i) hs.saveat[i] = o.saveat[i];
+  if (dcm) {
+    std::vector<double> sv, kv;
+    eval_sources(0.0, dcm->tran_mode ? 2 : 0, sv, kv);
+    std::copy(kv.begin(), kv.begin() + nk, hs.dcent); std::copy(sv.begin(), sv.begin() + nds, hs.dcent + nk);
+  }
+  TranCtl& cs = P.cs; std::memset(&cs, 0, sizeof(cs));
+  cs.t = t0; cs.h = start_step(o.dt0, t0, t1, dtmin, dtmax, bps[0]); cs.k = 1; cs.nhist = 1; cs.reset_rate = 1; cs.tslot[0] = t0;
+  std::memcpy(hs.ctl, &cs, sizeof(cs)); std::memcpy((char*)hs.ctl + sizeof(cs), &cs, sizeof(cs));
+  const ZeroLayout zl(n_wg);
   HIPCHK(ps.d_ptimes.alloc((size_t)2 * max_rows));  HIPCHK(ps.d_prows.alloc((size_t)max_rows * row_d));
-  HIPCHK(ps.d_wgrec.alloc((size_t)2 * n_wg * 16)); HIPCHK(ps.d_grprec.alloc(2 * 8 * 16));  HIPCHK(ps.d_pcnt.alloc(10 * 32)); HIPCHK(ps.d_pctl.alloc(2));
-  PersistArgs pa; std::memset(&pa, 0, sizeof(pa));
+  HIPCHK(ps.d_zero.alloc(zl.total));
+  PersistArgs& pa = P.pa; std::memset(&pa, 0, sizeof(pa));
   pa.a = nwt.base;
   pa.a.mode = MODE_TRAN; pa.a.maxit = nmaxit; pa.a.abstol = o.abstol; pa.a.reltol = o.reltol; pa.a.newton_tol = 0.1; pa.a.active = nullptr; pa.a.gshunt = 0.0;
   pa.bpw = bpw; pa.wide_l = stru.wide_l; pa.wide_other = stru.wide_other; pa.va_arena = (int)va_arena;
   pa.nblk = nblk; pa.n_wg = n_wg; pa.red_max = (tab.S > 1 || own_steps) ? 1 : 0; pa.wave_doubles = (int)wave_d;
   pa.t1 = t1; pa.dtmin = dtmin; pa.dtmax = dtmax; pa.first_frac = FIRST_STEP_FRAC; pa.kmax = kmax; pa.max_steps = max_steps;
-  pa.bps = ps.d_pbps.p; pa.nbp = (int)bps.size(); pa.saveat = ps.d_psave.p; pa.n_saveat = o.n_saveat;
-  pa.ci = ps.d_pci.p; pa.cd = ps.d_pcd.p; pa.n_ci = (int)max_ci; pa.n_cd = (int)max_cd;
-  pa.wgc = wg_consts ? ps.d_pwgc.p : nullptr; pa.wgk = wg_consts ? ps.d_pwgk.p : nullptr;
+  pa.bps = ds.bps; pa.nbp = (int)bps.size(); pa.saveat = ds.saveat; pa.n_saveat = o.n_saveat;
+  pa.ci = ds.ci; pa.cd = ds.cd; pa.n_ci = (int)max_ci; pa.n_cd = (int)max_cd;
+  pa.wgc = wg_consts ? ds.wgc : nullptr; pa.wgk = wg_consts ? ds.wgk : nullptr;
   pa.out_times = ps.d_ptimes.p; pa.out_rows = ps.d_prows.p; pa.max_rows = max_rows; pa.n_obs = n_obs;
-  pa.ctl = ps.d_pctl.p; pa.wg_rec = ps.d_wgrec.p; pa.grp_rec = ps.d_grprec.p; pa.counters = ps.d_pcnt.p;
+  pa.ctl = (TranCtl*)ds.ctl; pa.wg_rec = (double*)(ps.d_zero.p + zl.off_wgrec); pa.grp_rec = (double*)(ps.d_zero.p + zl.off_grprec); pa.counters = (unsigned*)(ps.d_zero.p + zl.off_cnt);
   pa.spin_ticks = 200000000LL;
   if (env_on(Env::SPIN_TICKS)) pa.spin_ticks = std::max(1L, env_long(Env::SPIN_TICKS, 0));
   pa.indep = own_steps ? 1 : 0;
-  ps.mode = desc.A.nb > 0 ? CH_MODE_BORDERED : (own_steps ? CH_MODE_OWN_STEPS : CH_MODE_LOCKSTEP);
   if (dcm) {
-    if (desc.A.nb == 0 || wg_consts) { set_err("internal: operating point on the device stepper is for the bordered form"); return CH_ERR_INTERNAL; }
-    std::vector<double> sv, kv, ent;
-    eval_sources(0.0, dcm->tran_mode ? 2 : 0, sv, kv);
-    ent.assign(kv.begin(), kv.begin() + nk); ent.insert(ent.end(), sv.begin(), sv.begin() + nds);
-    HIPCHK(ps.d_pdcent.upload(ent, st));
-    pa.dc_mode = 1; pa.dc_maxit = std::max(1, dcm->maxiters); pa.dc_abstol = dcm->abstol; pa.dc_entries = ps.d_pdcent.p;
+    pa.dc_mode = 1; pa.dc_maxit = std::max(1, dcm->maxiters); pa.dc_abstol = dcm->abstol; pa.dc_entries = ds.dcent;
     pa.dv_max = (!desc.A.mos_hdev.empty() || desc.A.wide) ? dcm->dv_max : 0.0;
   }
   pa.nb = desc.A.nb; pa.n_glob = desc.A.n_glob; pa.n_bdev = (int)desc.A.border_dev.size();
@@ -250,59 +308,84 @@
     pa.bd_kind[q] = bd.kind; pa.bd_ta[q] = bd.ta; pa.bd_tb[q] = bd.tb;
     pa.bd_val[q] = bd.kind == K_R ? torn.h_dmult0[bd.hdev] / torn.h_dpar0[bd.hdev] : torn.h_dmult0[bd.hdev] * torn.h_dpar0[bd.hdev];
   }
-  const bool coop = !pa.indep;
   pa.pair_dbg = (int)env_long(Env::PAIR_DBG, 0);
-  TranCtl cs; std::memset(&cs, 0, sizeof(cs));
-  cs.t = t0; cs.h = start_step(o.dt0, t0, t1, dtmin, dtmax, bps[0]); cs.k = 1; cs.nhist = 1; cs.reset_rate = 1; cs.tslot[0] = t0;
-  const void* fn = persist_kernel(desc.A.wide, desc.A.wide ? (own_steps ? PM_OWN : PM_LOCKSTEP) : desc.A.nb > 0 ? PM_BORDER : (own_steps ? PM_OWN : PM_LOCKSTEP),
-                                  (desc.A.wide || desc.A.nb > 0 || stru.lu_variant > 12) ? 16 : 12, pair);
-  if (!fn) { set_err("internal: no device-stepper kernel for this form"); return CH_ERR_INTERNAL; }
-  {
-    hipFuncAttributes fa;
-    HIPCHK(hipFuncGetAttributes(&fa, fn));
-    if (lds + fa.sharedSizeBytes > 160 * 1024) { set_err("device-resident stepper: LDS footprint"); return CH_OK; }
-    HIPCHK(hipFuncSetAttribute(fn, hipFuncAttributeMaxDynamicSharedMemorySize, (int)((160 * 1024 - (int)fa.sharedSizeBytes) & ~255)));
-  }
+  P.coop = !pa.indep; P.fn = fn; P.lds = lds; P.row_d = row_d; P.zero_bytes = zl.total; P.max_rows = max_rows; P.n_wg = n_wg; P.own_steps = own_steps;
+  HIPCHK(hipMemcpyAsync(ps.d_stage.p, ps.h_stage.p, ps.lay.total, hipMemcpyHostToDevice, st));
+  { const int zrc = persist_zero(P); if (zrc != CH_OK) return zrc; }
+  pcl.to(HP_UPLOADS);
+  P.ready = true;
+  return CH_OK;
+}
+
+inline int ch_circuit::tran_persistent(double t0, double t1, const ch_tran_opts& o, ch_result& R, const std::vector<double>& bps, int kmax, double dtmin, double dtmax,
+                                       int max_steps, int nmaxit, hclock::time_point tstart, bool& used, const ch_dc_opts* dcm, long long* dc_iters,
+                                       const std::vector<double>* bpc) {
+  used = false;
+  hipStream_t st = ctx->stream;
+  g_arena = &arena;
+  if (!ps.prep.ready) {
+    const int prc = persist_prepare(t0, t1, o, R.n_obs, bps, bpc, kmax, dtmin, dtmax, max_steps, nmaxit, dcm);
+    if (prc != CH_OK) { (void)sync_wait(); return prc; }
+    if (!ps.prep.ready) return CH_OK;
+  }
+  PersistPrep& P = ps.prep;
+  P.ready = false;
+  PhaseClock pcl(host_profile ? &hsplit : nullptr);
+  PersistArgs& pa = P.pa;
+  TranCtl cs = P.cs;
+  const bool own_steps = P.own_steps;
+  const size_t row_d = P.row_d; const long long max_rows = P.max_rows;
+  const StagePointers hs(ps.lay, ps.h_stage.p), ds(ps.lay, ps.d_stage.p);
+  const ZeroLayout zl(P.n_wg);
+  const size_t head = persist_ret_head();
+  ps.mode = desc.A.nb > 0 ? CH_MODE_BORDERED : (own_steps ? CH_MODE_OWN_STEPS : CH_MODE_LOCKSTEP);
   std::vector<double> hrows, htimes, hpts;
   bool single_batch = false;
-  std::vector<std::vector<double>> row_store;
+  size_t nr = 0;
   int resume = 0, status = CH_OK;
   for (;;) {
-    HIPCHK(hipMemcpyAsync(ps.d_pctl.p, &cs, sizeof(cs), hipMemcpyHostToDevice, st));
-    HIPCHK(hipMemcpyAsync(ps.d_pctl.p + 1, &cs, sizeof(cs), hipMemcpyHostToDevice, st));
-    HIPCHK(hipMemsetAsync(ps.d_pcnt.p, 0, 10 * 32 * sizeof(unsigned), st));
-    HIPCHK(hipMemsetAsync(ps.d_ptimes.p + max_rows, 0, (size_t)max_rows * sizeof(double), st));
-    if (pa.indep) HIPCHK(hipMemsetAsync(ps.d_prows.p, 0xff, (size_t)max_rows * row_d * sizeof(double), st));
-    HIPCHK(hipMemsetAsync(ps.d_wgrec.p, 0, (size_t)2 * n_wg * 16 * sizeof(double), st)); HIPCHK(hipMemsetAsync(ps.d_grprec.p, 0, 2 * 8 * 16 * sizeof(double), st));
+    if (resume) {
+      std::memcpy(hs.ctl, &cs, sizeof(cs)); std::memcpy((char*)hs.ctl + sizeof(cs), &cs, sizeof(cs));
+      hipError_t ue = hipMemcpyAsync(ds.ctl, hs.ctl, 2 * sizeof(cs), hipMemcpyHostToDevice, st);
+      const int zrc = ue == hipSuccess ? persist_zero(P) : CH_ERR_DEVICE;
+      if (zrc != CH_OK) { if (ue != hipSuccess) set_err(std::string("device-resident stepper: relaunch: ") + hipGetErrorString(ue)); (void)sync_wait(); used = true; return zrc; }
+    }
     pa.resume = resume;
     void* kargs[] = {(void*)&pa};
-    HIPCHK(hipEventRecord(nwt.ev0, st));
-    const hipError_t le = coop ? hipLaunchCooperativeKernel(fn, dim3(n_wg), dim3(PW * 64), kargs, (unsigned)lds, st)
-                               : hipLaunchKernel(fn, dim3(n_wg), dim3(PW * 64), kargs, lds, st);
+    hipError_t le = hipEventRecord(nwt.ev0, st);
+    if (le == hipSuccess) le = P.coop ? hipLaunchCooperativeKernel(P.fn, dim3(P.n_wg), dim3(PW * 64), kargs, (unsigned)P.lds, st)
+                                      : hipLaunchKernel(P.fn, dim3(P.n_wg), dim3(PW * 64), kargs, P.lds, st);
     if (le != hipSuccess) {
       (void)hipGetLastError();
+      (void)sync_wait();
       if (resume == 0) { set_err(std::string("cooperative launch refused: ") + hipGetErrorString(le)); return CH_OK; }
       set_err(std::string("device-resident stepper: relaunch failed: ") + hipGetErrorString(le)); used = true; return CH_ERR_DEVICE;
     }
-    HIPCHK(hipEventRecord(nwt.ev1, st));
     used = true;
-    { const hipError_t se = hipStreamSynchronize(st); if (se != hipSuccess) { set_err(std::string("device-resident stepper: ") + hipGetErrorString(se)); return CH_ERR_DEVICE; } }
+    hipError_t ce = hipEventRecord(nwt.ev1, st);
+    if (ce == hipSuccess) ce = hipMemcpyAsync(ps.h_ret.p, ds.ctl, 2 * sizeof(cs), hipMemcpyDeviceToHost, st);
+    if (ce == hipSuccess) ce = hipMemcpyAsync(ps.h_ret.p + 2 * sizeof(cs), ps.d_zero.p + zl.off_cnt + 9 * 32 * sizeof(unsigned), sizeof(unsigned), hipMemcpyDeviceToHost, st);
+    pcl.to(HP_LAUNCH);
+    { const hipError_t se = sync_wait();
+      if (se != hipSuccess || ce != hipSuccess) { set_err(std::string("device-resident stepper: ") + hipGetErrorString(se != hipSuccess ? se : ce)); return CH_ERR_DEVICE; } }
+    pcl.to(HP_KERNEL_WAIT);
     { float ms = 0; HIPCHK(hipEventElapsedTime(&ms, nwt.ev0, nwt.ev1)); stats.persist_ms += ms; stats.persist_launches += 1; }
-    HIPCHK(hipMemcpy(&cs, ps.d_pctl.p + (pa.indep ? 1 : 0), sizeof(cs), hipMemcpyDeviceToHost));
-    const size_t nr = (size_t)cs.nsaved;
+    std::memcpy(&cs, ps.h_ret.p + (pa.indep ? sizeof(cs) : 0), sizeof(cs));
+    nr = (size_t)cs.nsaved;
     const size_t base_t = htimes.size();
     single_batch = resume == 0 && cs.exit_reason != PX_ROWS_FULL && !dcm;
-    htimes.resize(base_t + nr); hpts.resize(base_t + nr);
-    if (!single_batch) hrows.resize((base_t + nr) * row_d);
-    if (nr > 0) {
-      HIPCHK(hipMemcpy(htimes.data() + base_t, ps.d_ptimes.p, nr * sizeof(double), hipMemcpyDeviceToHost));
-      HIPCHK(hipMemcpy(hpts.data() + base_t, ps.d_ptimes.p + max_rows, nr * sizeof(double), hipMemcpyDeviceToHost));
-      if (!single_batch) HIPCHK(hipMemcpy(hrows.data() + base_t * row_d, ps.d_prows.p, nr * row_d * sizeof(double), hipMemcpyDeviceToHost));
+    if (!single_batch && !dcm) {
+      htimes.resize(base_t + nr); hpts.resize(base_t + nr); hrows.resize((base_t + nr) * row_d);
+      if (nr > 0) {
+        HIPCHK(copy_wait(htimes.data() + base_t, ps.d_ptimes.p, nr * sizeof(double), hipMemcpyDeviceToHost));
+        HIPCHK(copy_wait(hpts.data() + base_t, ps.d_ptimes.p + max_rows, nr * sizeof(double), hipMemcpyDeviceToHost));
+        HIPCHK(copy_wait(hrows.data() + base_t * row_d, ps.d_prows.p, nr * row_d * sizeof(double), hipMemcpyDeviceToHost));
+      }
     }
     if (cs.exit_reason == PX_ROWS_FULL) { cs.nsaved = 0; resume = 1; continue; }
     if (cs.exit_reason == PX_ABORT) {
       ps.aborted = true;
-      unsigned code = 0; (void)hipMemcpy(&code, ps.d_pcnt.p + 9 * 32, sizeof(code), hipMemcpyDeviceToHost);
+      unsigned code = 0; std::memcpy(&code, ps.h_ret.p + 2 * sizeof(cs), sizeof(code));
       set_err("device-resident stepper: a wait exceeded its bound (site " + std::to_string(code & 255u) + ", sequence " + std::to_string(code >> 8) +
               ", attempts " + std::to_string((long long)cs.n_attempts) + "; workgroups not co-resident?)");
       status = CH_ERR_DEVICE;
@@ -310,12 +393,13 @@
     else status = cs.status;
     break;
   }
+  pcl.to(HP_COLLECT);
   if (dcm) {
     if (dc_iters) *dc_iters = cs.sum_iters;
     if (cs.exit_reason == PX_ABORT && status == CH_OK) status = CH_ERR_DEVICE;
     return status;
   }
-  return persist_collect(R, cs, own_steps, single_batch, htimes, hpts, hrows, status, tstart);
+  return persist_collect(R, cs, own_steps, single_batch, nr, htimes, hpts, hrows, status, tstart);
 }
 
 inline int ch_circuit::dc_border(const ch_dc_opts& o, long long* iters) {
diff --git a/cedarsim.jl_amd/csrc/ch_stepper_host.hpp b/cedarsim.jl_amd/csrc/ch_stepper_host.hpp
--- a/cedarsim.jl_amd/csrc/ch_stepper_host.hpp
+++ b/cedarsim.jl_amd/csrc/ch_stepper_host.hpp
@@ -1,7 +1,9 @@
 #pragma once
 
 #include <algorithm>
+#include <chrono>
 #include <cmath>
+#include <cstdint>
 #include <cstring>
 #include <utility>
 #include <vector>
@@ -127,6 +129,79 @@
   for (size_t r = 0; r < rows; ++r) for (int ob = 0; ob < n_obs; ++ob)
     std::copy(rows_in + (r * n_obs + ob) * S, rows_in + (r * n_obs + ob + 1) * S, values + ((size_t)ob * nt + row0 + r) * S);
 }
+
+struct Rng {
+  uint64_t s;
+  explicit Rng(uint64_t seed) : s(seed) {}
+  uint64_t next() { uint64_t z = (s += 0x9E3779B97F4A7C15ull); z = (z ^ (z >> 30)) * 0xBF58476D1CE4E5B9ull; z = (z ^ (z >> 27)) * 0x94D049BB133111EBull; return z ^ (z >> 31); }
+  double uniform() { return ((next() >> 11) + 0.5) * (1.0 / 9007199254740992.0); }
+  double normal() { double u1 = uniform(), u2 = uniform(); return std::sqrt(-2.0 * std::log(u1)) * std::cos(6.283185307179586 * u2); }
+};
+
+struct StartVectorCache {
+  uint64_t seed = 0; int n = 0, S = 0; bool valid = false;
+  std::vector<double> x;
+  std::vector<Rng> after;
+  bool lookup(uint64_t seed_, int n_, int S_) {
+    if (valid && seed == seed_ && n == n_ && S == S_) return true;
+    seed = seed_; n = n_; S = S_; valid = true;
+    x.resize((size_t)std::max(0, S) * std::max(0, n)); after.clear();
+    for (int s = 0; s < S; ++s) {
+      Rng r(seed + (uint64_t)s);
+      for (int i = 0; i < n; ++i) x[(size_t)s * n + i] = 1e-7 * r.normal();
+      after.push_back(r);
+    }
+    return false;
+  }
+};
+
+struct StageLayout {
+  enum Region { CI, CD, BPS, SAVEAT, CTL, WGC, WGK, DCENT, N_REGIONS };
+  static constexpr size_t ALIGN = 16;
+  size_t off[N_REGIONS] = {0}, bytes[N_REGIONS] = {0};
+  size_t total = 0, capacity = 0;
+  static size_t pad(size_t b) { return (b + ALIGN - 1) & ~(ALIGN - 1); }
+  bool plan(size_t n_ci, size_t n_cd, size_t n_bps, size_t n_saveat, size_t ctl_bytes, size_t n_wgc, size_t n_wgk, size_t n_dcent) {
+    const size_t want[N_REGIONS] = {n_ci * sizeof(int), n_cd * sizeof(double), n_bps * sizeof(double), n_saveat * sizeof(double),
+                                    2 * ctl_bytes, n_wgc * sizeof(int), n_wgk * sizeof(int), n_dcent * sizeof(double)};
+    size_t at = 0;
+    for (int r = 0; r < N_REGIONS; ++r) { off[r] = at; bytes[r] = want[r]; at += pad(want[r]); }
+    total = at;
+    if (total <= capacity) return false;
+    capacity = std::max(total, capacity + capacity / 2);
+    return true;
+  }
+};
+struct StagePointers {
+  int* ci; double* cd; double* bps; double* saveat; void* ctl; int* wgc; int* wgk; double* dcent;
+  StagePointers(const StageLayout& L, void* base) {
+    char* b = (char*)base;
+    ci = (int*)(b + L.off[StageLayout::CI]); cd = (double*)(b + L.off[StageLayout::CD]); bps = (double*)(b + L.off[StageLayout::BPS]);
+    saveat = (double*)(b + L.off[StageLayout::SAVEAT]); ctl = (void*)(b + L.off[StageLayout::CTL]); wgc = (int*)(b + L.off[StageLayout::WGC]);
+    wgk = (int*)(b + L.off[StageLayout::WGK]); dcent = (double*)(b + L.off[StageLayout::DCENT]);
+  }
+};
+struct ZeroLayout {
+  size_t off_wgrec = 0, off_grprec = 0, off_cnt = 0, total = 0;
+  explicit ZeroLayout(int n_wg) {
+    auto up = [](size_t b) { return (b + 255) & ~size_t(255); };
+    off_wgrec = 0; off_grprec = up((size_t)2 * n_wg * 16 * sizeof(double)); off_cnt = off_grprec + up(2 * 8 * 16 * sizeof(double));
+    total = off_cnt + up(10 * 32 * sizeof(unsigned));
+  }
+};
+
+enum HostPhase { HP_DC_START, HP_DC_COPIES, HP_DC_WAIT, HP_T0_EVAL, HP_BP_BLOB, HP_UPLOADS, HP_LAUNCH, HP_KERNEL_WAIT, HP_COLLECT, HP_FINAL_STATE, HP_COUNT };
+struct HostSplit {
+  double s[HP_COUNT] = {0}; long waits = 0;
+  static const char* name(int p) { static const char* nm[HP_COUNT] = {"dc start vector", "dc copies", "dc kernel wait", "t0 evaluation", "break points+blob", "uploads+memsets", "launch", "kernel wait", "collection", "final state"}; return nm[p]; }
+};
+struct PhaseClock {
+  using clock = std::chrono::steady_clock;
+  HostSplit* sp; clock::time_point last;
+  explicit PhaseClock(HostSplit* sp_) : sp(sp_) { if (sp) last = clock::now(); }
+  void skip() { if (sp) last = clock::now(); }
+  void to(int phase) { if (!sp) return; const auto now = clock::now(); sp->s[phase] += std::chrono::duration<double>(now - last).count(); last = now; }
+};
 
 struct LaunchStats {
   double device_ms = 0; long n_launch = 0, n_timed = 0;
```

Result: faster. 53500, median of 6 (+2.2%).
